# ysymyth/3D-SDN

Measured on AMD Instinct MI355X. Metric: rendered-objects/sec (FFD decode + transform + silhouette/normal/depth @384, fwd+bwd), higher is better.
Workload: dtype f32

## Files before the change

### 3d-sdn_amd/csrc/raster_bwd.hip

```cpp
#include "raster_math.h"
#include "sdn_common.h"

namespace sdn {

#ifndef SDN_EDGE_CHUNK
#define SDN_EDGE_CHUNK 8
#endif
constexpr int CHUNK = SDN_EDGE_CHUNK;
static_assert(CHUNK == 4 || CHUNK == 8, "k_edge_scan_sil / k_chunk_sum are written for 4 or 8");

struct BwdParams {
    const float* faces;
    const float* textures;
    const float* face_inv;
    const int32_t* face_index_map;
    const float* weight_map;
    const float* depth_map;
    const float* rgb_map;
    const float* g_rgb_out;
    const float* g_alpha_out;
    const float* g_depth_out;
    float* grad_faces;
    float* grad_textures;
    uint32_t* visible;
// ... 102 lines not shown
    w.pi0 = pi[0];
    w.pi1 = pi[1];
    if (axis == 0)
        w.direction = (w.p[0][0] < w.p[1][0]) ? -1 : 1;
    else
        w.direction = (w.p[0][0] < w.p[1][0]) ? 1 : -1;
    w.d0_from = cvt_i32(fmaxf(ceilf(fminf(w.p[0][0], w.p[1][0])), 0.0f));
    w.d0_to = cvt_i32(fminf(fmaxf(w.p[0][0], w.p[1][0]), is_f - 1.0f));
    return w;
}

__device__ __forceinline__ void edge_pixel(const BwdParams& P, const MapReader& M, const EdgeWalk& w, int fn, int axis,
                                           int d0, bool use_alpha, bool use_rgb, int lane, int nlanes, float& acc0,
                                           float& acc1)
{
    const int S = P.S;
    const float is_f = (float)S;
    const float fd0 = (float)d0;
    float d1_cross = (w.p[1][1] - w.p[0][1]) / (w.p[1][0] - w.p[0][0]);
    d1_cross = d1_cross * (fd0 - w.p[0][0]);
    d1_cross = d1_cross + w.p[0][1];
    const int d1_in = (0 < w.direction) ? cvt_i32(floorf(d1_cross)) : cvt_i32(ceilf(d1_cross));
    const int d1_out = d1_in + w.direction;
    if (d1_in < 0 || S <= d1_in) return;
    if (d1_out < 0 || S <= d1_out) return;

    const int xin = axis == 0 ? d0 : d1_in, yin = axis == 0 ? d1_in : d0;
    const int xout = axis == 0 ? d0 : d1_out, yout = axis == 0 ? d1_out : d0;
    float alpha_in = 0.f, alpha_out = 0.f, rgb_in[3] = {0, 0, 0}, rgb_out[3] = {0, 0, 0};
    const int f_in = M.fidx(xin, yin);
    if (use_alpha) {
        alpha_in = f_in >= 0 ? 1.0f : 0.0f;
        alpha_out = M.alpha(xout, yout);
    }
    if (use_rgb) {
#pragma unroll
        for (int k = 0; k < 3; k++) {
            rgb_in[k] = M.rgb(xin, yin, k);
            rgb_out[k] = M.rgb(xout, yout, k);
        }
    }
    const bool nz1 = w.p[1][0] != fd0, nz0 = w.p[0][0] != fd0;
    const float den1 = w.p[1][0] - fd0, den0 = fd0 - w.p[0][0];
    const bool sparse_rows = P.nz_cnt && use_alpha && !use_rgb;

    if (f_in == fn && sparse_rows) {
        const int d1_limit = (0 < w.direction) ? S - 1 : 0;
        const int d1_from = max(min(d1_out, d1_limit), 0);
        const int d1_to = min(max(d1_out, d1_limit), S - 1);
        const size_t row = (size_t)(axis == 0 ? P.bs : 0) * S + (size_t)M.b * S + d0;
        const uint16_t* cnt = P.nz_cnt + row * (S + 1);
        const int k1 = cnt[d1_to + 1];
        for (int k = cnt[d1_from] + lane; k < k1; k += nlanes) {
            const int d1 = P.nz_pos[row * S + k];
            const float diff_grad = P.nz_val[row * S + k];
            if (nz1) acc0 -= diff_grad / edge_dist(w.p[0][0], w.p[1][0], den1, d1, d1_cross, is_f, P.eps);
            if (nz0) acc1 -= diff_grad / edge_dist(w.p[0][0], w.p[1][0], den0, d1, d1_cross, is_f, P.eps);
        }
    } else if (f_in == fn) {
        const int d1_limit = (0 < w.direction) ? S - 1 : 0;
        const int d1_from = max(min(d1_out, d1_limit), 0);
        const int d1_to = min(max(d1_out, d1_limit), S - 1);
        for (int d1 = d1_from + lane; d1 <= d1_to; d1 += nlanes) {
            const int x = axis == 0 ? d0 : d1, y = axis == 0 ? d1 : d0;
            float diff_grad = 0.0f;
            if (use_alpha) diff_grad = diff_grad + (M.alpha(x, y) - alpha_in) * M.g_alpha(x, y);
            if (use_rgb) {
#pragma unroll
                for (int k = 0; k < 3; k++) diff_grad = diff_grad + (M.rgb(x, y, k) - rgb_in[k]) * M.g_rgb(x, y, k);
            }
            if (diff_grad <= 0) continue;
            if (nz1) acc0 -= diff_grad / edge_dist(w.p[0][0], w.p[1][0], den1, d1, d1_cross, is_f, P.eps);
            if (nz0) acc1 -= diff_grad / edge_dist(w.p[0][0], w.p[1][0], den0, d1, d1_cross, is_f, P.eps);
        }
    }
    {
        float d0_cross2;
        if ((fd0 - w.p[0][0]) * (fd0 - w.p[2][0]) < 0) {
            d0_cross2 = (w.p[2][1] - w.p[0][1]) / (w.p[2][0] - w.p[0][0]);
            d0_cross2 = d0_cross2 * (fd0 - w.p[0][0]);
            d0_cross2 = d0_cross2 + w.p[0][1];
        } else {
            d0_cross2 = (w.p[1][1] - w.p[2][1]) / (w.p[1][0] - w.p[2][0]);
            d0_cross2 = d0_cross2 * (fd0 - w.p[2][0]);
            d0_cross2 = d0_cross2 + w.p[2][1];
        }
        const int d1_limit = (0 < w.direction) ? cvt_i32(ceilf(d0_cross2)) : cvt_i32(floorf(d0_cross2));
        const int d1_from = max(min(d1_in, d1_limit), 0);
        const int d1_to = min(max(d1_in, d1_limit), S - 1);
        for (int d1 = d1_from + lane; d1 <= d1_to; d1 += nlanes) {
            const int x = axis == 0 ? d0 : d1, y = axis == 0 ? d1 : d0;
            if (M.fidx(x, y) != fn) continue;
            float diff_grad = 0.0f;
            if (use_alpha) diff_grad = diff_grad + (1.0f - alpha_out) * M.g_alpha(x, y);
            if (use_rgb) {
#pragma unroll
                for (int k = 0; k < 3; k++) diff_grad = diff_grad + (M.rgb(x, y, k) - rgb_out[k]) * M.g_rgb(x, y, k);
            }
            if (diff_grad <= 0) continue;
            if (nz1) acc0 -= diff_grad / edge_dist(w.p[0][0], w.p[1][0], den1, d1, d1_cross, is_f, P.eps);
            if (nz0) acc1 -= diff_grad / edge_dist(w.p[0][0], w.p[1][0], den0, d1, d1_cross, is_f, P.eps);
        }
    }
}

__global__ __launch_bounds__(256) void k_mark_visible(const int32_t* __restrict__ face_index_map, long npx, int S,
                                                       int nf, uint32_t* __restrict__ visible)
{
    const long i = (long)blockIdx.x * 256 + threadIdx.x;
    if (i >= npx) return;
    const int fn = face_index_map[i];
    if (fn >= 0) visible[(i / ((long)S * S)) * nf + fn] = 1u;
}

__global__ __launch_bounds__(256) void k_cover_bits(const BwdParams P, uint32_t* __restrict__ cov, uint32_t* __restrict__ covT,
                                                    float* __restrict__ gT)
{
    __shared__ uint32_t flag[32][33];
    __shared__ float gt[32][33];
    const int S = P.S, b = blockIdx.z, W = (S + 31) >> 5;
    const bool aa = (P.flags & SDN_AA) != 0;
    const int R = aa ? S / 2 : S, n = aa ? 16 : 32;
    const int lx = threadIdx.x & 31, l8 = threadIdx.x >> 5;
    const unsigned half = threadIdx.x & 32;
    const int x = blockIdx.x * 32 + lx;
    int fn[4];
    float gv[4];
#pragma unroll
    for (int r = 0; r < 4; r++) {
        const int ly = l8 + 8 * r, y = blockIdx.y * 32 + ly;
        const int xo = blockIdx.x * n + lx, yo = blockIdx.y * n + ly;
        fn[r] = (x < S && y < S) ? P.face_index_map[((size_t)b * S + y) * S + x] : -1;
        gv[r] = (lx < n && ly < n && xo < R && yo < R) ? P.g_alpha_out[((size_t)b * R + yo) * R + xo] : 0.0f;
    }
#pragma unroll
    for (int r = 0; r < 4; r++) {
        const int ly = l8 + 8 * r, y = blockIdx.y * 32 + ly;
        const bool covered = fn[r] >= 0;
        const int left = __shfl_up(fn[r], 1);
        if (covered && ((threadIdx.x & 63) == 0 || left != fn[r])) P.visible[(size_t)b * P.nf + fn[r]] = 1u;
        flag[ly][lx] = covered ? 1u : 0u;
        gt[ly][lx] = gv[r];
        const unsigned long long m = __ballot(covered);
        if (lx == 0 && y < S) cov[((size_t)b * S + y) * W + blockIdx.x] = (uint32_t)(m >> half);
    }
    __syncthreads();
#pragma unroll
    for (int r = 0; r < 4; r++) {
        const int lc = l8 + 8 * r, xt = blockIdx.x * 32 + lc;
        const unsigned long long m = __ballot(flag[lx][lc] != 0u);
        if (lx == 0 && xt < S) covT[((size_t)b * S + xt) * W + blockIdx.y] = (uint32_t)(m >> half);
        const int xo = blockIdx.x * n + lc, yo = blockIdx.y * n + lx;
        if (lx < n && lc < n && xo < R && yo < R) gT[((size_t)b * R + xo) * R + yo] = gt[lx][lc];
    }
}

constexpr int CR = 6;
template <bool AA>
__global__ __launch_bounds__(256) void k_compact_rows(const BwdParams P, const uint32_t* __restrict__ cov,
                                                      const uint32_t* __restrict__ covT, const float* __restrict__ gT,
                                                      size_t rows_per_map, int S, uint16_t* __restrict__ cnt,
                                                      uint16_t* __restrict__ pos, float* __restrict__ val)
{
    const int lane = threadIdx.x & 63;
    const size_t row = (size_t)blockIdx.x * 4 + (threadIdx.x >> 6);
    if (row >= 2 * rows_per_map) return;
    const bool image_row = row < rows_per_map;
    const size_t line = image_row ? row : row - rows_per_map;
    const int b = (int)(line / (size_t)S), d0 = (int)(line % (size_t)S);
    const int R = AA ? S / 2 : S, W = (S + 31) >> 5;
    const uint32_t* cw = (image_row ? cov : covT) + line * W;
    const float* gl = image_row ? P.g_alpha_out + ((size_t)b * R + (R - 1 - (AA ? d0 >> 1 : d0))) * R
                                : gT + ((size_t)b * R + (AA ? d0 >> 1 : d0)) * R;
    uint16_t* c = cnt + row * (S + 1);
    const bool odd = ((row * (size_t)(S + 1)) & 1) != 0;
    const unsigned long long below = (1ull << lane) - 1ull;
    int base = 0;
    if (AA && odd && lane == 0) c[0] = 0;
    for (int e0 = 0; e0 < R; e0 += 64 * CR) {
        float g[CR];
        uint32_t w[CR];
#pragma unroll
        for (int j = 0; j < CR; j++) {
            const int e = e0 + 64 * j + lane;
            g[j] = 0.0f;
            w[j] = 0u;
            if (e < R) {
                g[j] = gl[image_row ? e : R - 1 - e];
                w[j] = cw[AA ? e >> 4 : e >> 5];
            }
        }
#pragma unroll
        for (int j = 0; j < CR; j++) {
            const int e = e0 + 64 * j + lane;
            if (e0 + 64 * j >= R) break;
            const float t = (0.0f - 1.0f) * (AA ? g[j] * 0.25f : g[j]);
            const float h = t > 0.0f ? t : 0.0f;
            const bool in = e < R && h > 0.0f;
            if (AA) {
                const uint32_t two = w[j] >> (2 * (e & 15));
                const bool nz0 = in && !(two & 1u), nz1 = in && !(two & 2u);
                const unsigned long long m0 = __ballot(nz0), m1 = __ballot(nz1);
                const int i0 = base + __popcll(m0 & below) + __popcll(m1 & below);
                const int i1 = i0 + (nz0 ? 1 : 0), i2 = i1 + (nz1 ? 1 : 0);
                if (e < R) {
                    const int x = 2 * e;
                    if (odd)
                        *reinterpret_cast<uint32_t*>(c + x + 1) = (uint32_t)i1 | (uint32_t)i2 << 16;
                    else
                        *reinterpret_cast<uint32_t*>(c + x) = (uint32_t)i0 | (uint32_t)i1 << 16;
                    if (nz0) {
                        pos[row * S + i0] = (uint16_t)x;
                        val[row * S + i0] = h;
                    }
                    if (nz1) {
                        pos[row * S + i1] = (uint16_t)(x + 1);
                        val[row * S + i1] = h;
                    }
                }
                base += __popcll(m0) + __popcll(m1);
            } else {
                const bool nz = in && !((w[j] >> (e & 31)) & 1u);
                const unsigned long long m = __ballot(nz);
                const int i0 = base + __popcll(m & below);
                if (e < R) {
                    c[e] = (uint16_t)i0;
                    if (nz) {
                        pos[row * S + i0] = (uint16_t)e;
                        val[row * S + i0] = h;
                    }
                }
                base += __popcll(m);
            }
        }
    }
    if (lane == 0 && !(AA && odd)) c[S] = (uint16_t)base;
}

constexpr int PLAN_THREADS = 1024;
__global__ __launch_bounds__(PLAN_THREADS) void k_edge_plan(const BwdParams P)
{
    const long i = (long)blockIdx.x * PLAN_THREADS + threadIdx.x;
    const long total = (long)P.bs * P.nf;
    if (P.sink.grad_verts) {
        const long n = (long)P.bs * P.sink.nv * 3;
        for (long k = i; k < n; k += (long)gridDim.x * PLAN_THREADS) P.sink.grad_verts[k] = 0.0f;
    }
    const int lane = threadIdx.x & 63;
    int from[6], cnt[6];
    uint32_t nchunks = 0;
    bool contributes = false;
    if (i < total) {
        const bool active = (P.flags & (SDN_ALPHA | SDN_RGB)) != 0;
        if (active && P.visible[i] != 0u) {
            float face[9];
#pragma unroll
            for (int k = 0; k < 9; k++) face[k] = P.faces[i * 9 + k];
            if (!is_backface(face)) {
                const float is_f = (float)P.S;
#pragma unroll
                for (int e = 0; e < 6; e++) {
                    const EdgeWalk w = edge_walk(face, e >> 1, e & 1, is_f);
                    from[e] = w.d0_from;
                    cnt[e] = max(w.d0_to - w.d0_from + 1, 0);
                    nchunks += (uint32_t)((cnt[e] + CHUNK - 1) / CHUNK);
                }
                contributes = nchunks != 0;
            }
        }
    }
    __shared__ uint32_t wave_sum[PLAN_THREADS / 64];
    __shared__ uint32_t block_base;
    uint32_t incl = nchunks;
#pragma unroll
    for (int d = 1; d < 64; d <<= 1) {
        const uint32_t o = __shfl_up(incl, d, 64);
        if (lane >= d) incl += o;
    }
    const int wave = threadIdx.x >> 6;
    if (lane == 63) wave_sum[wave] = incl;
    __syncthreads();
    if (threadIdx.x == 0) {
        uint32_t tot = 0;
        for (int w = 0; w < PLAN_THREADS / 64; w++) tot += wave_sum[w];
        block_base = tot ? atomicAdd(P.counter, tot) : 0u;
    }
    __syncthreads();
    uint32_t wave_base = block_base;
    for (int w = 0; w < wave; w++) wave_base += wave_sum[w];
    if (i >= total) return;
    const bool per_face = !segment_path(P);
    if (!contributes) {
        if (per_face) P.chunk_base[i] = -2;
        return;
    }
    const uint32_t base = wave_base + incl - nchunks;
    if (base + nchunks > P.cap) {
        if (per_face)
            P.chunk_base[i] = -1;
        else
            P.chunk_base[atomicAdd(P.counter + 1, 1u)] = (int32_t)i;
        for (uint32_t c = base; c < P.cap; c++) P.chunk_desc[c] = make_uint4(0xffffffffu, 0xffffffffu, 0u, 0u);
        return;
    }
    if (per_face) P.chunk_base[i] = (int32_t)base;
    uint32_t c = base;
// ... 495 lines not shown
    const bool head = valid && (px != d.x || py != d.y);
    const unsigned long long bounds = __ballot(head || !valid);
    const unsigned long long above = lane == 63 ? 0ull : bounds >> (lane + 1);
    const int len = head ? (above ? __ffsll((long long)above) : 64 - lane) : 0;
    float a0 = 0.f, a1 = 0.f;
    for (int k = 0; __ballot(k < len) != 0ull; k++) {
        const float tx = __shfl(v.x, lane + k, 64), ty = __shfl(v.y, lane + k, 64);
        if (k < len) {
            a0 += tx;
            a1 += ty;
        }
    }
    const unsigned long long runs_on = __ballot(head && !above && after.x == d.x && after.y == d.y);
    if (runs_on) {
        const int hl = __ffsll((long long)runs_on) - 1;
        const uint32_t kx = (uint32_t)__builtin_amdgcn_readlane((int)d.x, hl), ky = (uint32_t)__builtin_amdgcn_readlane((int)d.y, hl);
        for (uint32_t s0 = c_wave + 64u; s0 < nchunks; s0 += 64u) {
            const uint32_t s = s0 + (uint32_t)lane;
            uint2 ds = make_uint2(0xffffffffu, 0xffffffffu);
            float2 vs = make_float2(0.f, 0.f);
            uint32_t ms = 0u;
            if (s < nchunks) {
                ds = key_at(s);
                vs = P.chunk_out[s];
                ms = P.chunk_mask[s];
            }
            const bool mine = ds.x == kx && ds.y == ky;
            if (mine && ms) vs = chunk_add_owners(P, s, ms, vs);
            const unsigned long long others = ~__ballot(mine);
            const int n = others ? __ffsll((long long)others) - 1 : 64;
            for (int k = 0; k < n; k++) {
                const float tx = __shfl(vs.x, k, 64), ty = __shfl(vs.y, k, 64);
                if (lane == hl) {
                    a0 += tx;
                    a1 += ty;
                }
            }
            if (n < 64) break;
        }
    }
    if (!head) return;
    segment_add(P, (long)d.x, (int)d.y, a0, a1);
}

__global__ __launch_bounds__(256) void k_bwd_pixels(const BwdParams P)
{
    const long i = (long)blockIdx.x * 256 + threadIdx.x;
    const long npx = (long)P.bs * P.S * P.S;
    if (i >= npx) return;
    const int fn = P.face_index_map[i];
    if (fn < 0) return;
    const int S = P.S;
    const int bn = (int)(i / ((long)S * S));
    const int pn = (int)(i % ((long)S * S));
    const int yi = pn / S, xi = pn % S;
    const MapReader M(P, bn);
    const size_t fidx = (size_t)bn * P.nf + fn;
    float face[9];
#pragma unroll
    for (int k = 0; k < 9; k++) face[k] = P.faces[fidx * 9 + k];
    const float depth = P.depth_map[i];
    const float w[3] = {P.weight_map[i * 3 + 0], P.weight_map[i * 3 + 1], P.weight_map[i * 3 + 2]};

    if ((P.flags & SDN_DEPTH) && P.g_depth_out) {
        float inv[9];
#pragma unroll
        for (int k = 0; k < 9; k++) inv[k] = P.face_inv[fidx * 9 + k];
        const float g = M.g_depth(xi, yi);
        const float depth2 = depth * depth;
        float* gf = P.grad_faces + fidx * 9;
#pragma unroll
        for (int k = 0; k < 3; k++) {
            const float zk = face[3 * k + 2];
            float t = g * w[k];
            t = t * depth2;
            t = t / (zk * zk);
            unsafeAtomicAdd(&gf[3 * k + 2], t);
        }
        float tmp[2] = {0.f, 0.f};
#pragma unroll
        for (int k = 0; k < 2; k++)
#pragma unroll
            for (int l = 0; l < 3; l++) tmp[k] = tmp[k] + (-inv[3 * l + k] / face[3 * l + 2]);
#pragma unroll
        for (int k = 0; k < 3; k++)
#pragma unroll
            for (int l = 0; l < 2; l++) {
                float t = -g * tmp[l];
                t = t * w[k];
                t = t * depth2;
                t = t * (float)S;
                t = t / 2.0f;
                unsafeAtomicAdd(&gf[3 * k + l], t);
            }
    }
    if ((P.flags & SDN_RGB) && P.g_rgb_out && P.grad_textures) {
        const bool face_color = (P.flags & SDN_FACE_COLOR) != 0;
        const int ts = face_color ? 2 : P.ts;
        const TexCoord tc = texture_coord(w, depth, face[2], face[5], face[8], ts, P.eps);
        const float g[3] = {M.g_rgb(xi, yi, 0), M.g_rgb(xi, yi, 1), M.g_rgb(xi, yi, 2)};
        if (face_color) {
            float acc[3] = {0.f, 0.f, 0.f};
#pragma unroll
            for (int c = 0; c < 8; c++) {
                int isc;
                float wgt;
                texture_corner(tc, c, ts, isc, wgt);
#pragma unroll
                for (int k = 0; k < 3; k++) acc[k] = acc[k] + wgt * g[k];
            }
#pragma unroll
            for (int k = 0; k < 3; k++) unsafeAtomicAdd(&P.grad_textures[fidx * 3 + k], acc[k]);
        } else {
            float* gt = P.grad_textures + fidx * (size_t)ts * ts * ts * 3;
#pragma unroll
            for (int c = 0; c < 8; c++) {
                int isc;
                float wgt;
                texture_corner(tc, c, ts, isc, wgt);
#pragma unroll
                for (int k = 0; k < 3; k++) unsafeAtomicAdd(&gt[(long)isc * 3 + k], wgt * g[k]);
            }
        }
    }
}

}

using namespace sdn;

static size_t align256(size_t n) { return (n + 255) & ~(size_t)255; }

static void bwd_layout(int bs, int nf, int S, size_t off[14], uint32_t& cap, size_t& total)
{
    const size_t n = (size_t)bs * nf;
    cap = (uint32_t)(4 * n + 65536);
    off[0] = 0;
    off[1] = 256;
    off[10] = off[1] + align256(n * sizeof(uint32_t));
    off[2] = off[10] + align256((size_t)4 * bs * S * sizeof(uint32_t));
    off[3] = off[2] + align256(n * sizeof(int32_t));
    off[4] = off[3] + align256((size_t)cap * sizeof(uint4));
    off[5] = off[4] + align256((size_t)cap * sizeof(float2));
    off[6] = off[5];
    off[7] = off[6] + align256((size_t)bs * S * S * sizeof(float));
    off[8] = off[7] + align256((size_t)2 * bs * S * (S + 1) * sizeof(uint16_t));
    off[9] = off[8] + align256((size_t)2 * bs * S * S * sizeof(uint16_t));
    off[11] = off[9] + align256((size_t)2 * bs * S * S * sizeof(float));
    off[12] = off[11] + align256((size_t)2 * bs * S * 3 * S * sizeof(OwnerRec));
    off[13] = off[12] + align256((size_t)cap * 8 * sizeof(float2));
    total = off[13] + align256((size_t)cap);
}

namespace sdn {
const uint32_t* raster_bwd_visible_flags(const void* workspace) { return (const uint32_t*)((const char*)workspace + 256); }
}

SDN_API int sdn_raster_bwd_workspace_bytes(int bs, int nf, int S, size_t* out)
{
    if (bs <= 0 || nf <= 0 || S <= 0 || !out) return fail(SDN_EINVAL, "sdn_raster_bwd_workspace_bytes: bad sizes");
    size_t off[14], total;
    uint32_t cap;
    bwd_layout(bs, nf, S, off, cap, total);
    *out = total;
    return SDN_OK;
}

SDN_API int sdn_rasterize_bwd(const float* faces, const float* textures, int ts, int bs, int nf, int S, double eps,
                              int flags, const float* face_inv, const int32_t* face_index_map,
                              const float* weight_map, const float* depth_map, const float* rgb_map,
                              const float* g_rgb_out, const float* g_alpha_out, const float* g_depth_out,
                              float* grad_faces, float* grad_textures, void* workspace, size_t workspace_bytes,
                              sdnStream stream)
{
    return rasterize_bwd_core(nullptr, faces, textures, ts, bs, nf, S, eps, flags, face_inv, face_index_map, weight_map, depth_map,
                              rgb_map, g_rgb_out, g_alpha_out, g_depth_out, grad_faces, grad_textures, workspace, workspace_bytes,
                              stream);
}

int sdn::rasterize_bwd_core(const VertexSink* sink, const float* faces, const float* textures, int ts, int bs, int nf, int S,
                            double eps, int flags, const float* face_inv, const int32_t* face_index_map, const float* weight_map,
                            const float* depth_map, const float* rgb_map, const float* g_rgb_out, const float* g_alpha_out,
                            const float* g_depth_out, float* grad_faces, float* grad_textures, void* workspace,
                            size_t workspace_bytes, sdnStream stream)
{
    if (!faces || !face_inv || !face_index_map || !weight_map || !depth_map || (!grad_faces && !sink) || bs <= 0 || nf <= 0 ||
        S <= 0)
        return fail(SDN_EINVAL, "sdn_rasterize_bwd: missing state (was the forward run with SDN_SAVE_MAPS?)");
    if (sink && ((flags & (SDN_RGB | SDN_DEPTH | SDN_ACCUMULATE)) || !(flags & SDN_ALPHA) || !g_alpha_out || !sink->faces_idx ||
                 !sink->grad_verts || nf != (sink->fill_back ? 2 : 1) * sink->nf0))
        return fail(SDN_EINVAL, "rasterize_bwd_core: the vertex sink takes a silhouette-only pass");
    if ((flags & SDN_RGB) && (!rgb_map || !textures))
        return fail(SDN_EINVAL, "sdn_rasterize_bwd: rgb gradients need rgb_map and textures");
    if ((flags & SDN_AA) && (S & 1)) return fail(SDN_EINVAL, "sdn_rasterize_bwd: SDN_AA needs an even internal size");
    size_t off[14], need;
    uint32_t cap;
    bwd_layout(bs, nf, S, off, cap, need);
    if (!workspace || workspace_bytes < need)
        return fail(SDN_ENOMEM, "sdn_rasterize_bwd: workspace %zu < %zu bytes", workspace_bytes, need);
    hipStream_t st = (hipStream_t)stream;
    BwdParams P;
    P.faces = faces;
    P.textures = textures;
    P.face_inv = face_inv;
    P.face_index_map = face_index_map;
    P.weight_map = weight_map;
    P.depth_map = depth_map;
    P.rgb_map = rgb_map;
    P.g_rgb_out = (flags & SDN_RGB) ? g_rgb_out : nullptr;
    P.g_alpha_out = (flags & SDN_ALPHA) ? g_alpha_out : nullptr;
    P.g_depth_out = (flags & SDN_DEPTH) ? g_depth_out : nullptr;
    P.grad_faces = grad_faces;
    P.grad_textures = grad_textures;
    char* ws = (char*)workspace;
    P.counter = (uint32_t*)(ws + off[0]);
    P.visible = (uint32_t*)(ws + off[1]);
    P.chunk_base = (int32_t*)(ws + off[2]);
    P.chunk_desc = (uint4*)(ws + off[3]);
    P.chunk_out = (float2*)(ws + off[4]);
    P.nz_cnt = nullptr;
    P.nz_pos = nullptr;
    P.nz_val = nullptr;
    P.row_cnt = nullptr;
    P.own_rec = nullptr;
    P.own_out = nullptr;
    P.chunk_mask = nullptr;
    P.cap = (flags & SDN_SERIAL_EDGES) ? 0u : cap;
    P.eps = eps;
    P.ts = ts;
    P.bs = bs;
    P.nf = nf;
    P.S = S;
    P.flags = flags;
    P.sink = sink ? *sink : VertexSink{nullptr, 0, 0, 0, 0, nullptr};
    if (!P.g_rgb_out) P.flags &= ~SDN_RGB;
    if (!P.g_alpha_out) P.flags &= ~SDN_ALPHA;
    const long total = (long)bs * nf;
    const long npx = (long)bs * S * S;
    const bool edges = (P.flags & (SDN_ALPHA | SDN_RGB)) != 0;
    if (!edges) P.flags &= ~SDN_SPARSE_GRAD;
    int rc;
    if (edges) {
        hipError_t e = hipMemsetAsync(ws, 0, off[2], st);
        if (e != hipSuccess) return fail(SDN_ELAUNCH, "hipMemsetAsync(plan): %s", hipGetErrorString(e));
        const size_t cov_words = (size_t)(S + 31) / 32;
        const bool setup_fits = 2 * (size_t)bs * S * cov_words * sizeof(uint32_t) <= off[7] - off[6] &&
                                (size_t)bs * S * S * sizeof(float) <= off[12] - off[11];
        const bool sil_path = (P.flags & SDN_ALPHA) && !(P.flags & SDN_RGB) && !(flags & SDN_SERIAL_EDGES) && setup_fits;
        if (!sil_path) {
            hipLaunchKernelGGL(k_mark_visible, dim3(cdiv(npx, 256)), dim3(256), 0, st, face_index_map, npx, S, nf,
                               P.visible);
            if ((rc = check_launch("k_mark_visible"))) return rc;
        }
        if (sil_path) {
            if (S > 65535) return fail(SDN_EINVAL, "sdn_rasterize_bwd: internal size %d exceeds the 16-bit row index", S);
            const bool aa = (P.flags & SDN_AA) != 0;
            const size_t rows = (size_t)bs * S;
            uint32_t* cov = (uint32_t*)(ws + off[6]);
            uint32_t* covT = cov + rows * cov_words;
            float* gT = (float*)(ws + off[11]);
            uint16_t* cnt = (uint16_t*)(ws + off[7]);
            uint16_t* pos = (uint16_t*)(ws + off[8]);
            float* val = (float*)(ws + off[9]);
            hipLaunchKernelGGL(k_cover_bits, dim3(cdiv(S, 32), cdiv(S, 32), bs), dim3(256), 0, st, P, cov, covT, gT);
            if ((rc = check_launch("k_cover_bits"))) return rc;
            const dim3 grid((unsigned)cdiv((long)(2 * rows), 4));
            if (aa)
                hipLaunchKernelGGL(k_compact_rows<true>, grid, dim3(256), 0, st, P, cov, covT, gT, rows, S, cnt, pos, val);
            else
                hipLaunchKernelGGL(k_compact_rows<false>, grid, dim3(256), 0, st, P, cov, covT, gT, rows, S, cnt, pos, val);
            if ((rc = check_launch("k_compact_rows"))) return rc;
            P.nz_cnt = cnt;
            P.nz_pos = pos;
            P.nz_val = val;
            if ((size_t)cap * 8 >= (1u << 30)) return fail(SDN_EINVAL, "sdn_rasterize_bwd: %u chunks exceed the 30-bit slot index", cap);
            P.row_cnt = (uint32_t*)(ws + off[10]);
            P.own_rec = (OwnerRec*)(ws + off[11]);
            P.own_out = (float2*)(ws + off[12]);
            P.chunk_mask = (uint8_t*)(ws + off[13]);
        }
    }
    hipLaunchKernelGGL(k_edge_plan, dim3(cdiv(total, PLAN_THREADS)), dim3(PLAN_THREADS), 0, st, P);
    if ((rc = check_launch("k_edge_plan"))) return rc;
    if (edges) {
        {
            TimedLaunch timed(TIME_EDGE_SCAN, st, 0.0);
            if (P.nz_cnt) {
                hipLaunchKernelGGL(k_edge_scan_sil, dim3(256 * 8), dim3(256), 0, st, P);
                const int nrows = 2 * bs * S;
                hipLaunchKernelGGL(k_edge_rows, dim3((unsigned)nrows), dim3(256), (size_t)S * sizeof(float2), st, P, nrows);
                if (!segment_path(P)) hipLaunchKernelGGL(k_chunk_sum, dim3(cdiv((long)cap, 256)), dim3(256), 0, st, P);
            } else
                hipLaunchKernelGGL(k_edge_scan, dim3(256 * 8), dim3(256), 0, st, P);
        }
        if ((rc = check_launch("k_edge_scan"))) return rc;
    }
    if (segment_path(P)) {
        hipLaunchKernelGGL(k_edge_segments, dim3((unsigned)(cdiv((long)cap, 256) + SEG_SERIAL_BLOCKS)), dim3(256), 0, st, P);
        if ((rc = check_launch("k_edge_segments"))) return rc;
    } else {
        hipLaunchKernelGGL(k_edge_reduce, dim3(cdiv(total, 256)), dim3(256), 0, st, P);
        if ((rc = check_launch("k_edge_reduce"))) return rc;
    }

    const bool need_tex = (P.flags & SDN_RGB) && grad_textures;
    if (need_tex && !(flags & SDN_ACCUMULATE)) {
        const size_t n = (flags & SDN_FACE_COLOR) ? (size_t)total * 3 : (size_t)total * ts * ts * ts * 3;
        hipError_t e = hipMemsetAsync(grad_textures, 0, n * sizeof(float), st);
        if (e != hipSuccess) return fail(SDN_ELAUNCH, "hipMemsetAsync(grad_textures): %s", hipGetErrorString(e));
    }
    if (((P.flags & SDN_DEPTH) && P.g_depth_out) || need_tex) {
        hipLaunchKernelGGL(k_bwd_pixels, dim3(cdiv(npx, 256)), dim3(256), 0, st, P);
        if ((rc = check_launch("k_bwd_pixels"))) return rc;
    }
    return SDN_OK;
}
```

### 3d-sdn_amd/csrc/raster_fwd.hip

```cpp
#include <mutex>
#include <type_traits>
#include <vector>

#include "camera_math.h"
#include "raster_math.h"
#include "sdn_common.h"

namespace sdn {

constexpr int TS = 32;
constexpr int NTHR = (TS / 2) * (TS / 2);
constexpr int NWAVE = NTHR / 64;
static_assert(NTHR % 64 == 0 && NTHR >= 2 * TS && TS <= 32, "tile / workgroup geometry (hit queue packs px, py in 5 bits)");
constexpr int QCAP = 512;
constexpr int FREC = 13;
#ifndef SDN_LAB_FLAT_MAX
#define SDN_LAB_FLAT_MAX 256
#endif
constexpr int FLAT_MAX = SDN_LAB_FLAT_MAX;
static_assert(FLAT_MAX >= 1 && FLAT_MAX <= 256, "a batch's stream holds at most 64 * 256 candidates: 14 bits of start, at most 256 passes (the marks are u16, 0xffff = none)");
#ifndef SDN_LAB_HIZ_MIN_LIST
#define SDN_LAB_HIZ_MIN_LIST 257
#endif
constexpr int HIZ_MIN_LIST = SDN_LAB_HIZ_MIN_LIST;
#ifndef SDN_K1_HIZ
#define SDN_K1_HIZ 1
#endif
constexpr uint32_t TB_CULLED = 0x000000FFu;

struct FwdParams {
    const float* faces;
    const float* textures;
    const float* bg;
    float* face_inv;
    int32_t* face_index_map;
    float* weight_map;
    float* depth_map;
    float* rgb_map;
    float* rgb_out;
    float* alpha_out;
    float* depth_out;
    const uint32_t* tilebox;
    const uint4* pixbox;
    const uint32_t* tile_off;
    const uint32_t* tile_list;
    const uint32_t* overflow;
    const uint32_t* tile_order;
    const uint32_t* thin_count;
    const float4* thin_list;
    unsigned long long* counters;
    uint32_t list_cap;
    double eps;
    int ts, bs, nf, S, ntx, flags, bg_per_batch;
    int hiz;
    float near_le, far_f;
};

constexpr float THIN_MARGIN = 4.0f;

__device__ __forceinline__ float face_margin_px(const float f[9], int S)
{
    const float ex0 = f[3] - f[0], ey0 = f[4] - f[1];
    const float ex1 = f[6] - f[0], ey1 = f[7] - f[1];
    const float ex2 = f[6] - f[3], ey2 = f[7] - f[4];
    const float l0 = sqrtf(ex0 * ex0 + ey0 * ey0);
    const float l1 = sqrtf(ex1 * ex1 + ey1 * ey1);
    const float l2 = sqrtf(ex2 * ex2 + ey2 * ey2);
    const float lmax = fmaxf(l0, fmaxf(l1, l2));
    const float perim = l0 + l1 + l2;
    float cmax = fmaxf(fmaxf(fabsf(f[0]), fabsf(f[1])), fmaxf(fabsf(f[3]), fabsf(f[4])));
    cmax = fmaxf(cmax, fmaxf(fabsf(f[6]), fabsf(f[7])));
    const float area2 = fabsf(ex0 * ey1 - ex1 * ey0) - 9.5367432e-7f * lmax * lmax;
    if (!(area2 > 0.0f)) return -1.0f;
    const float delta = 9.5367432e-7f * (1.0f + cmax);
    const float base = 0.004f * fmaxf(1.0f, (float)S * (1.0f / 1024.0f)) + 0.5f * (float)S * delta;
    const float m = base + 0.5f * (float)S * (delta * perim * lmax / area2);
    if (!(m < (float)S)) return -1.0f;
    return m;
}

constexpr int HIST_MAX = 4096;

template <bool K1, bool GATHER>
__global__ __launch_bounds__(256) void k_face_setup(const float* __restrict__ faces, int nf, int S, int ntx,
                                                     float* __restrict__ face_inv, uint32_t* __restrict__ tilebox,
                                                     uint4* __restrict__ pixbox, uint32_t* __restrict__ tile_count,
                                                     uint32_t* __restrict__ thin_count, float4* __restrict__ thin_list,
                                                     const FaceSource G)
{
    __shared__ uint32_t hist[HIST_MAX];
    const int ntiles = ntx * ntx;
    const bool use_lds = ntiles <= HIST_MAX;
    if (use_lds)
        for (int t = threadIdx.x; t < ntiles; t += 256) hist[t] = 0u;
    __syncthreads();
    const int b = blockIdx.y;
    const int t_local = blockIdx.x * 256 + threadIdx.x;
    uint32_t* gcount = tile_count + (size_t)b * ntiles;
    const bool pairs = GATHER && G.fill_back != 0;
    const int nthr = pairs ? G.nf0 : nf;
    float v[3][3], pf[9];
    if constexpr (GATHER) {
        if (t_local < nthr) {
            const int32_t* idx = G.faces_idx + (size_t)b * G.fstride + (size_t)t_local * 3;
#pragma unroll
            for (int k = 0; k < 3; k++) {
                const float* p = G.verts + ((size_t)b * G.nv + idx[k]) * 3;
                v[k][0] = G.flip_x ? p[0] * -1.0f : p[0];
                v[k][1] = p[1];
                v[k][2] = p[2];
            }
            Basis B;
            if (G.mode != 0) B = camera_basis(G.mode, G.eye, G.dir, G.up, b);
            const float wv = G.width ? G.width[b] : 1.0f;
#pragma unroll
            for (int k = 0; k < 3; k++) {
                float o[3];
                project_vertex(v[k], G.mode, B, G.width != nullptr, wv, o);
                pf[3 * k + 0] = o[0];
                pf[3 * k + 1] = o[1];
                pf[3 * k + 2] = o[2];
            }
        }
    }
    if (t_local < nthr)
    for (int rep = 0; rep < (pairs ? 2 : 1); rep++) {
    const int fn_local = t_local + (rep ? G.nf0 : 0);
    const long i = (long)b * nf + fn_local;
    float f[9];
    float nrm[3] = {0.f, 0.f, 0.f};
    if constexpr (GATHER) {
        if (G.normals_out) {
            if (rep)
                face_normal(v[2], v[1], v[0], G.sx, nrm);
            else
                face_normal(v[0], v[1], v[2], G.sx, nrm);
        }
#pragma unroll
        for (int k = 0; k < 3; k++)
#pragma unroll
            for (int d = 0; d < 3; d++) f[3 * k + d] = rep ? pf[3 * (2 - k) + d] : pf[3 * k + d];
    } else {
#pragma unroll
        for (int k = 0; k < 9; k++) f[k] = faces[i * 9 + k];
    }
    float inv[9] = {0, 0, 0, 0, 0, 0, 0, 0, 0};
    uint32_t tb = TB_CULLED;
    uint4 pb = make_uint4(0, 0, 0, 0);
    bool thin = false;
    if constexpr (K1) {
      if (!is_backface(f)) {
        bool finite = true;
#pragma unroll
        for (int k = 0; k < 9; k++) finite = finite && (f[k] - f[k] == 0.0f);
        const K1Face K = k1_setup(f, S);
        if (finite && !K.dead && K.xi_min <= K.xi_max) {
            float inv_s[9];
            face_inverse(K.px, K.py, inv_s);
#pragma unroll
            for (int l = 0; l < 3; l++)
#pragma unroll
                for (int k = 0; k < 3; k++) {
                    const float v = inv_s[3 * l + k];
                    if (K.pi[l] == 0) inv[k] = v;
                    if (K.pi[l] == 1) inv[3 + k] = v;
                    if (K.pi[l] == 2) inv[6 + k] = v;
                }
            const float ymin = fminf(K.py[0], fminf(K.py[1], K.py[2])), ymax = fmaxf(K.py[0], fmaxf(K.py[1], K.py[2]));
            int y0 = 0, y1 = S - 1;
            if (!(K.px[2] < 0.0f)) {
                y0 = (int)fmaxf(floorf(ymin) - 1.0f, 0.0f);
                y1 = (int)fminf(ceilf(ymax) + 1.0f, (float)(S - 1));
            }
            if (y0 <= y1 && ymax + 1.0f >= 0.0f && ymin - 1.0f <= (float)(S - 1)) {
                const int x0 = K.xi_min, x1 = K.xi_max;
                tb = (uint32_t)(x0 / TS) | ((uint32_t)(x1 / TS) << 8) | ((uint32_t)(y0 / TS) << 16) | ((uint32_t)(y1 / TS) << 24);
                pb = make_uint4((uint32_t)x0 | ((uint32_t)x1 << 16), (uint32_t)y0 | ((uint32_t)y1 << 16), 0u, 0u);
                for (int ty = y0 / TS; ty <= y1 / TS; ty++)
                    for (int tx = x0 / TS; tx <= x1 / TS; tx++) {
                        if (use_lds)
                            atomicAdd(&hist[ty * ntx + tx], 1u);
                        else
                            atomicAdd(&gcount[ty * ntx + tx], 1u);
                    }
            }
        }
      }
    } else if (!is_backface(f)) {
        const float is_f = (float)S;
        float px[3], py[3];
#pragma unroll
        for (int k = 0; k < 3; k++) {
            px[k] = ndc_to_pixel(f[3 * k + 0], is_f);
            py[k] = ndc_to_pixel(f[3 * k + 1], is_f);
        }
        face_inverse(px, py, inv);
        int x0 = 0, x1 = S - 1, y0 = 0, y1 = S - 1;
        const float m = face_margin_px(f, S);
        const float xmin = fminf(px[0], fminf(px[1], px[2])), xmax = fmaxf(px[0], fmaxf(px[1], px[2]));
        const float ymin = fminf(py[0], fminf(py[1], py[2])), ymax = fmaxf(py[0], fmaxf(py[1], py[2]));
        const bool finite = (xmin - xmin == 0.0f) && (xmax - xmax == 0.0f) && (ymin - ymin == 0.0f) &&
                            (ymax - ymax == 0.0f) && (px[0] == px[0]) && (px[1] == px[1]) && (px[2] == px[2]) &&
                            (py[0] == py[0]) && (py[1] == py[1]) && (py[2] == py[2]);
        bool visible = true;
        if (!finite) {
            visible = false;
        } else if (!(m > 0.0f) || m > THIN_MARGIN) {
            visible = false;
            int ia = 0, ib = 1;
            float l2 = (px[1] - px[0]) * (px[1] - px[0]) + (py[1] - py[0]) * (py[1] - py[0]);
            const float l2b = (px[2] - px[0]) * (px[2] - px[0]) + (py[2] - py[0]) * (py[2] - py[0]);
            const float l2c = (px[2] - px[1]) * (px[2] - px[1]) + (py[2] - py[1]) * (py[2] - py[1]);
            if (l2b > l2) { l2 = l2b; ia = 0; ib = 2; }
            if (l2c > l2) { l2 = l2c; ia = 1; ib = 2; }
            if (l2 > 0.0f) {
                const float L = sqrtf(l2);
                const float nx = -(py[ib] - py[ia]) / L, ny = (px[ib] - px[ia]) / L;
                const int ic = 3 - ia - ib;
                const float h = fabsf((px[ic] - px[ia]) * nx + (py[ic] - py[ia]) * ny);
                const float pmax = fmaxf(fmaxf(fabsf(xmin), fabsf(xmax)), fmaxf(fabsf(ymin), fabsf(ymax)));
                float cmax = fmaxf(fmaxf(fabsf(f[0]), fabsf(f[1])), fmaxf(fabsf(f[3]), fabsf(f[4])));
                cmax = fmaxf(cmax, fmaxf(fabsf(f[6]), fabsf(f[7])));
                const float delta_px = 9.5367432e-7f * (1.0f + cmax) * 0.5f * (float)S;
                const float band = h + 0.05f + 2.5f * delta_px + 4e-6f * (pmax + (float)S);
                const bool repeated = (__float_as_uint(f[0]) == __float_as_uint(f[3]) && __float_as_uint(f[1]) == __float_as_uint(f[4])) ||
                                      (__float_as_uint(f[0]) == __float_as_uint(f[6]) && __float_as_uint(f[1]) == __float_as_uint(f[7])) ||
                                      (__float_as_uint(f[3]) == __float_as_uint(f[6]) && __float_as_uint(f[4]) == __float_as_uint(f[7]));
                int bx0 = 0, bx1 = S - 1, by0 = 0, by1 = S - 1;
                bool boxed_out = false;
                if (m > 0.0f) {
                    const float fx0 = ceilf(xmin - m), fx1 = floorf(xmax + m);
                    const float fy0 = ceilf(ymin - m), fy1 = floorf(ymax + m);
                    if (fx1 < 0.0f || fy1 < 0.0f || fx0 > (float)(S - 1) || fy0 > (float)(S - 1) || fx0 > fx1 || fy0 > fy1) {
                        boxed_out = true;
                    } else {
                        bx0 = (int)fmaxf(fx0, 0.0f);
                        by0 = (int)fmaxf(fy0, 0.0f);
                        bx1 = (int)fminf(fx1, (float)(S - 1));
                        by1 = (int)fminf(fy1, (float)(S - 1));
                    }
                }
                if (!(repeated && band < 0.5f) && !boxed_out) {
                    const uint32_t trange = (uint32_t)(bx0 / TS) | ((uint32_t)(bx1 / TS) << 8) | ((uint32_t)(by0 / TS) << 16) |
                                            ((uint32_t)(by1 / TS) << 24);
                    pb = make_uint4((uint32_t)bx0 | ((uint32_t)bx1 << 16), (uint32_t)by0 | ((uint32_t)by1 << 16), __float_as_uint(m), 0u);
                    const uint32_t slot = atomicAdd(&thin_count[b], 1u);
                    float4* e = thin_list + (size_t)b * nf * 2;
                    e[slot] = make_float4(nx, ny, px[ia] * nx + py[ia] * ny, band);
                    e[nf + slot] = make_float4(px[ia], py[ia], __uint_as_float((uint32_t)fn_local), __uint_as_float(trange));
                    thin = true;
                }
            }
        } else {
            const float fx0 = ceilf(xmin - m), fx1 = floorf(xmax + m);
            const float fy0 = ceilf(ymin - m), fy1 = floorf(ymax + m);
            if (fx1 < 0.0f || fy1 < 0.0f || fx0 > (float)(S - 1) || fy0 > (float)(S - 1) || fx0 > fx1 || fy0 > fy1) {
                visible = false;
            } else {
                x0 = (int)fmaxf(fx0, 0.0f);
                y0 = (int)fmaxf(fy0, 0.0f);
                x1 = (int)fminf(fx1, (float)(S - 1));
                y1 = (int)fminf(fy1, (float)(S - 1));
            }
        }
        if (visible) {
            tb = (uint32_t)(x0 / TS) | ((uint32_t)(x1 / TS) << 8) | ((uint32_t)(y0 / TS) << 16) |
                 ((uint32_t)(y1 / TS) << 24);
            pb = make_uint4((uint32_t)x0 | ((uint32_t)x1 << 16), (uint32_t)y0 | ((uint32_t)y1 << 16), __float_as_uint(m), 0u);
            for (int ty = y0 / TS; ty <= y1 / TS; ty++)
                for (int tx = x0 / TS; tx <= x1 / TS; tx++) {
                    if (use_lds)
                        atomicAdd(&hist[ty * ntx + tx], 1u);
                    else
                        atomicAdd(&gcount[ty * ntx + tx], 1u);
                }
        }
    }
    tilebox[i] = tb;
    if (!GATHER || tb != TB_CULLED || thin) {
#pragma unroll
        for (int k = 0; k < 9; k++) face_inv[i * 9 + k] = inv[k];
        pixbox[i] = pb;
        if constexpr (GATHER) {
            float* fo = G.faces_out + i * 9;
#pragma unroll
            for (int k = 0; k < 9; k++) fo[k] = f[k];
            if (G.normals_out) {
                float* o = G.normals_out + i * 3;
                o[0] = nrm[0];
                o[1] = nrm[1];
                o[2] = nrm[2];
            }
        }
    }
    }
    __syncthreads();
    if (use_lds)
        for (int t = threadIdx.x; t < ntiles; t += 256) {
            const uint32_t c = hist[t];
            if (c) atomicAdd(&gcount[t], c);
        }
}

constexpr int ORDER_CLASSES = 64;
__device__ __forceinline__ int order_class(uint32_t entries, bool streams_all_faces)
{
    if (streams_all_faces) return 0;
    const int c = (int)(4.0f * __log2f((float)entries + 1.0f));
    return ORDER_CLASSES - 1 - min(ORDER_CLASSES - 1, c);
}

__global__ __launch_bounds__(256) void k_tile_offsets(const uint32_t* __restrict__ tile_count, int ntiles,
                                                       uint32_t list_cap, uint32_t* __restrict__ tile_off,
                                                       uint32_t* __restrict__ overflow, uint32_t* __restrict__ order_hist)
{
    __shared__ uint32_t wave_tot[4];
    __shared__ uint32_t carry_s;
    __shared__ uint32_t hist[ORDER_CLASSES];
    const int b = blockIdx.x, tid = threadIdx.x;
    if (tid < ORDER_CLASSES) hist[tid] = 0u;
    const uint32_t* cnt = tile_count + (size_t)b * ntiles;
    uint32_t* off = tile_off + (size_t)b * (ntiles + 1);
    if (tid == 0) carry_s = 0u;
    __syncthreads();
    for (int base = 0; base < ntiles; base += 256) {
        const int t = base + tid;
        const uint32_t v = t < ntiles ? cnt[t] : 0u;
        uint32_t incl = v;
#pragma unroll
        for (int d = 1; d < 64; d <<= 1) {
            const uint32_t o = __shfl_up(incl, d, 64);
            if ((tid & 63) >= d) incl += o;
        }
        if ((tid & 63) == 63) wave_tot[tid >> 6] = incl;
        __syncthreads();
        uint32_t wave_off = 0, total = 0;
#pragma unroll
        for (int w = 0; w < 4; w++) {
            const uint32_t x = wave_tot[w];
            if (w < (tid >> 6)) wave_off += x;
            total += x;
        }
        const uint32_t carry = carry_s;
        if (t < ntiles) off[t] = carry + wave_off + incl - v;
        __syncthreads();
        if (tid == 0) carry_s = carry + total;
        __syncthreads();
    }
    if (tid == 0) {
        off[ntiles] = carry_s;
        overflow[b] = carry_s > list_cap ? 1u : 0u;
    }
    const bool streams = carry_s > list_cap;
    for (int t = tid; t < ntiles; t += 256) atomicAdd(&hist[order_class(cnt[t], streams)], 1u);
    __syncthreads();
    if (tid < ORDER_CLASSES && hist[tid]) atomicAdd(&order_hist[tid], hist[tid]);
}

__global__ __launch_bounds__(256) void k_tile_order(const uint32_t* __restrict__ tile_count, int ntiles, int total,
                                                     const uint32_t* __restrict__ overflow,
                                                     const uint32_t* __restrict__ order_hist,
                                                     uint32_t* __restrict__ order_cursor, uint32_t* __restrict__ tile_order)
{
    __shared__ uint32_t base[ORDER_CLASSES];
    const int tid = threadIdx.x;
    if (tid < 64) {
        const uint32_t v = order_hist[tid];
        uint32_t incl = v;
#pragma unroll
        for (int d = 1; d < 64; d <<= 1) {
            const uint32_t o = __shfl_up(incl, d, 64);
            if (tid >= d) incl += o;
        }
        base[tid] = incl - v;
    }
    __shared__ uint32_t lcnt[ORDER_CLASSES], lbase[ORDER_CLASSES];
    if (tid < ORDER_CLASSES) lcnt[tid] = 0u;
    __syncthreads();
    const int g = blockIdx.x * 256 + tid;
    int c = 0;
    uint32_t local = 0;
    if (g < total) {
        c = order_class(tile_count[g], overflow[g / ntiles] != 0u);
        local = atomicAdd(&lcnt[c], 1u);
    }
    __syncthreads();
    if (tid < ORDER_CLASSES && lcnt[tid]) lbase[tid] = base[tid] + atomicAdd(&order_cursor[tid], lcnt[tid]);
    __syncthreads();
    if (g < total) tile_order[lbase[c] + local] = (uint32_t)g;
}

__global__ __launch_bounds__(256) void k_tile_fill(const uint32_t* __restrict__ tilebox, int nf, int ntx,
                                                    const uint32_t* __restrict__ tile_off,
                                                    const uint32_t* __restrict__ overflow, uint32_t list_cap,
                                                    uint32_t* __restrict__ tile_cursor, uint32_t* __restrict__ tile_list)
{
    __shared__ uint32_t cnt[HIST_MAX];
    __shared__ uint32_t base[HIST_MAX];
    const int b = blockIdx.y;
    if (overflow[b]) return;
    const int fn = blockIdx.x * 256 + threadIdx.x;
    const uint32_t v = fn < nf ? tilebox[(size_t)b * nf + fn] : TB_CULLED;
    const int tx0 = (int)(v & 255u), tx1 = (int)((v >> 8) & 255u), ty0 = (int)((v >> 16) & 255u), ty1 = (int)(v >> 24);
    const bool active = tx0 <= tx1;
    const int ntiles = ntx * ntx;
    const uint32_t* off = tile_off + (size_t)b * (ntiles + 1);
    uint32_t* cur = tile_cursor + (size_t)b * ntiles;
    uint32_t* lst = tile_list + (size_t)b * list_cap;
    if (ntiles > HIST_MAX) {
        if (active)
            for (int ty = ty0; ty <= ty1; ty++)
                for (int tx = tx0; tx <= tx1; tx++) {
                    const int tt = ty * ntx + tx;
                    lst[off[tt] + atomicAdd(&cur[tt], 1u)] = (uint32_t)fn;
                }
        return;
    }
    for (int t = threadIdx.x; t < ntiles; t += 256) cnt[t] = 0u;
    __syncthreads();
    if (active)
        for (int ty = ty0; ty <= ty1; ty++)
            for (int tx = tx0; tx <= tx1; tx++) atomicAdd(&cnt[ty * ntx + tx], 1u);
    __syncthreads();
    for (int t = threadIdx.x; t < ntiles; t += 256) {
        const uint32_t c = cnt[t];
        if (c) {
            base[t] = off[t] + atomicAdd(&cur[t], c);
            cnt[t] = 0u;
        }
    }
    __syncthreads();
    if (active)
        for (int ty = ty0; ty <= ty1; ty++)
            for (int tx = tx0; tx <= tx1; tx++) {
                const int tt = ty * ntx + tx;
                lst[base[tt] + atomicAdd(&cnt[tt], 1u)] = (uint32_t)fn;
            }
}

struct PixelResult {
    int fn;
    float w[3];
    float zp;
    float rgb[3];
    float alpha;
};

__device__ __forceinline__ PixelResult shade_pixel(const FwdParams& P, int b, unsigned long long key, int gx, int gy)
{
    PixelResult r;
    const bool want_rgb = (P.flags & SDN_RGB) != 0;
    float bgc[3] = {0.f, 0.f, 0.f};
    if (want_rgb) {
        const float* c = P.bg + (P.bg_per_batch ? 3 * b : 0);
        bgc[0] = c[0];
        bgc[1] = c[1];
        bgc[2] = c[2];
    }
    if (key == ~0ull) {
        r.fn = -1;
        r.w[0] = r.w[1] = r.w[2] = 0.0f;
        r.zp = P.far_f;
        r.alpha = 0.0f;
#pragma unroll
        for (int k = 0; k < 3; k++) r.rgb[k] = 0.0f * 0.0f + (1.0f - 0.0f) * bgc[k];
        return r;
    }
    const int fn = (int)(uint32_t)(key & 0xffffffffull);
    const size_t fidx = (size_t)b * P.nf + fn;
    float inv[9], f[9];
#pragma unroll
    for (int k = 0; k < 9; k++) inv[k] = P.face_inv[fidx * 9 + k];
#pragma unroll
    for (int k = 0; k < 9; k++) f[k] = P.faces[fidx * 9 + k];
    r.fn = fn;
    if (P.flags & SDN_K1_COVERAGE) {
        int pi[3];
        k1_order(f, pi);
        float inv_s[9], ws[3];
#pragma unroll
        for (int l = 0; l < 3; l++)
#pragma unroll
            for (int k = 0; k < 3; k++) inv_s[3 * l + k] = pi[l] == 0 ? inv[k] : (pi[l] == 1 ? inv[3 + k] : inv[6 + k]);
        bary_weights(inv_s, gx, gy, ws);
#pragma unroll
        for (int l = 0; l < 3; l++) {
            if (pi[l] == 0) r.w[0] = ws[l];
            if (pi[l] == 1) r.w[1] = ws[l];
            if (pi[l] == 2) r.w[2] = ws[l];
        }
    } else {
        bary_weights(inv, gx, gy, r.w);
    }
    r.zp = ord_unbits((uint32_t)(key >> 32));
    r.alpha = 1.0f;
    r.rgb[0] = r.rgb[1] = r.rgb[2] = 0.0f;
    if (want_rgb) {
        const bool face_color = (P.flags & SDN_FACE_COLOR) != 0;
        const int ts = face_color ? 2 : P.ts;
        const TexCoord tc = texture_coord(r.w, r.zp, f[2], f[5], f[8], ts, P.eps);
        const float* tex = face_color ? (P.textures + fidx * 3) : (P.textures + fidx * (size_t)ts * ts * ts * 3);
        float acc[3] = {0.f, 0.f, 0.f};
#pragma unroll
        for (int pn = 0; pn < 8; pn++) {
            int isc;
            float wgt;
            texture_corner(tc, pn, ts, isc, wgt);
            const float* t = face_color ? tex : (tex + (long)isc * 3);
#pragma unroll
            for (int k = 0; k < 3; k++) acc[k] = acc[k] + wgt * t[k];
        }
#pragma unroll
        for (int k = 0; k < 3; k++) r.rgb[k] = acc[k] * 1.0f + (1.0f - 1.0f) * bgc[k];
    }
    return r;
}

__device__ __forceinline__ void tile_epilogue(const FwdParams& P, const int b, const int X0, const int Y0,
                                              const unsigned long long* zbuf, const int tid)
{
    const int S = P.S;
    const bool aa = (P.flags & SDN_AA) != 0;
    const bool save = (P.flags & SDN_SAVE_MAPS) != 0;
    const bool lazy = (P.flags & SDN_LAZY_MAPS) != 0;
    const bool want_rgb = (P.flags & SDN_RGB) != 0;
    const bool want_alpha = (P.flags & SDN_ALPHA) != 0;
    const bool want_depth = (P.flags & SDN_DEPTH) != 0;
    const int qx = tid % (TS / 2), qy = tid / (TS / 2);
    const int R = aa ? S / 2 : S;
    float s_alpha = 0.f, s_depth = 0.f, s_rgb[3] = {0.f, 0.f, 0.f};
    bool any_valid = false;
#pragma unroll
    for (int dyi = 0; dyi < 2; dyi++) {
#pragma unroll
        for (int dx = 0; dx < 2; dx++) {
            const int dy = 1 - dyi;
            const int px = 2 * qx + dx, py = 2 * qy + dy;
            const int gx = X0 + px, gy = Y0 + py;
            if (gx >= S || gy >= S) continue;
            any_valid = true;
            const PixelResult r = shade_pixel(P, b, zbuf[py * TS + px], gx, gy);
            const size_t q = ((size_t)b * S + gy) * S + gx;
            if (save) {
                P.face_index_map[q] = r.fn;
                P.depth_map[q] = r.zp;
            }
            if (save && !lazy) {
                P.weight_map[q * 3 + 0] = r.w[0];
                P.weight_map[q * 3 + 1] = r.w[1];
                P.weight_map[q * 3 + 2] = r.w[2];
                if (want_rgb) {
                    P.rgb_map[q * 3 + 0] = r.rgb[0];
                    P.rgb_map[q * 3 + 1] = r.rgb[1];
                    P.rgb_map[q * 3 + 2] = r.rgb[2];
                }
            }
            if (aa) {
                s_alpha = s_alpha + r.alpha;
                s_depth = s_depth + r.zp;
#pragma unroll
                for (int k = 0; k < 3; k++) s_rgb[k] = s_rgb[k] + r.rgb[k];
            } else {
                const size_t o = ((size_t)b * S + (S - 1 - gy)) * S + gx;
                if (want_alpha) P.alpha_out[o] = r.alpha;
                if (want_depth) P.depth_out[o] = r.zp;
                if (want_rgb) {
#pragma unroll
                    for (int k = 0; k < 3; k++)
                        P.rgb_out[(((size_t)b * 3 + k) * S + (S - 1 - gy)) * S + gx] = r.rgb[k];
                }
            }
        }
    }
    if (aa && any_valid) {
        const int oc = X0 / 2 + qx;
        const int orow = R - 1 - (Y0 / 2 + qy);
        const size_t o = ((size_t)b * R + orow) * R + oc;
        if (want_alpha) P.alpha_out[o] = s_alpha * 0.25f;
        if (want_depth) P.depth_out[o] = s_depth * 0.25f;
        if (want_rgb) {
#pragma unroll
            for (int k = 0; k < 3; k++) P.rgb_out[(((size_t)b * 3 + k) * R + orow) * R + oc] = s_rgb[k] * 0.25f;
        }
    }
}

__device__ __forceinline__ void hiz_refresh(const uint32_t* zhi, uint32_t* blockmax, const int lane)
{
    uint32_t m[4] = {0u, 0u, 0u, 0u};
#pragma unroll
    for (int i = 0; i < 16; i++) m[i >> 2] = max(m[i >> 2], zhi[2 * (i * 64 + lane) + 1]);
#pragma unroll
    for (int rb = 0; rb < 4; rb++) {
        uint32_t v = m[rb];
        v = max(v, (uint32_t)__shfl_xor((int)v, 1, 64));
        v = max(v, (uint32_t)__shfl_xor((int)v, 2, 64));
        v = max(v, (uint32_t)__shfl_xor((int)v, 4, 64));
        v = max(v, (uint32_t)__shfl_xor((int)v, 32, 64));
        m[rb] = v;
    }
    if ((lane & 39) == 0) {
#pragma unroll
        for (int rb = 0; rb < 4; rb++) blockmax[rb * 4 + (lane >> 3)] = m[rb];
    }
    __builtin_amdgcn_wave_barrier();
}
__device__ __forceinline__ bool hiz_hidden(const uint32_t* blockmax, const uint32_t zc, const int x0, const int x1, const int y0,
                                           const int y1)
{
    uint32_t zb = 0u;
    for (int by = y0 >> 3; by <= (y1 >> 3); by++)
        for (int bx = x0 >> 3; bx <= (x1 >> 3); bx++) zb = max(zb, blockmax[by * (TS / 8) + bx]);
    return zc > zb;
}

template <bool COUNT, int HIZ>
__global__ __launch_bounds__(NTHR, 6) void k_raster_tiles(const FwdParams P)
{
    unsigned n_cand = 0, n_in = 0, n_key = 0;
    unsigned long long c_fetch = 0, c_small = 0, c_large = 0, c_thin = 0, c_epi = 0, t_mark = 0, t_begin = 0;
    auto tick = [&](unsigned long long& acc) {
        if constexpr (COUNT) {
            const unsigned long long now = wall_clock64();
            acc += now - t_mark;
            t_mark = now;
        }
    };
    if constexpr (COUNT) t_begin = t_mark = wall_clock64();
    __shared__ unsigned long long zbuf[TS * TS];
    __shared__ uint32_t q_fn[QCAP];
    __shared__ float xtab[TS], ytab[TS];
    __shared__ uint32_t q_count, next_batch, next_thin;
    __shared__ uint32_t hit_queue[NWAVE][128];
    __shared__ float face_rec[NWAVE][64 * FREC];
    __shared__ uint32_t blockmax[(TS / 8) * (TS / 8)];
    __shared__ uint32_t own_strip[NWAVE][32];
    static_assert(TS == 32, "the hi-z refresh maps 64 lanes x 16 reads onto a 32 x 32 tile");

    const int tid = threadIdx.x;
    const int lane = tid & 63, wave = tid >> 6;
    const int ntiles_all = P.ntx * P.ntx;
    const uint32_t gid = P.tile_order[blockIdx.x];
    const int b = (int)(gid / (uint32_t)ntiles_all), tile = (int)(gid % (uint32_t)ntiles_all);
    const int tx = tile % P.ntx, ty = tile / P.ntx;
    const int X0 = tx * TS, Y0 = ty * TS;
    const int S = P.S, nf = P.nf;

    for (int i = tid; i < TS * TS; i += NTHR) zbuf[i] = ~0ull;
    if (tid < TS)
        xtab[tid] = pixel_to_ndc(X0 + tid, S);
    else if (tid < 2 * TS)
        ytab[tid - TS] = pixel_to_ndc(Y0 + tid - TS, S);
    if (tid == 0) q_count = next_batch = next_thin = 0;
    if (tid < (TS / 8) * (TS / 8)) blockmax[tid] = 0xffffffffu;
    __syncthreads();

    const float4* thin_cull = P.thin_list + (size_t)b * nf * 2;
    const uint32_t n_thin = P.thin_count[b];
    const float4 thin_c0 = thin_cull[min(tid, 2 * nf - 1)];
    const uint32_t thin_r0 = reinterpret_cast<const uint32_t*>(thin_cull + nf + min(tid, nf - 1))[3];
    const uint32_t* tb = P.tilebox + (size_t)b * nf;
    const uint4* pbx = P.pixbox + (size_t)b * nf;
    const float* faces_b = P.faces + (size_t)b * nf * 9;
    const float* finv_b = P.face_inv + (size_t)b * nf * 9;

    auto shade_hit = [&](const float z0, const float z1, const float z2, const float (&inv)[9], const uint32_t qf,
                         const int px, const int py) {
        float bw[3];
        bary_weights(inv, X0 + px, Y0 + py, bw);
        const float zp = persp_depth(bw, z0, z1, z2);
        if (zp > P.near_le && zp < P.far_f) {
            if constexpr (COUNT) n_key++;
            const unsigned long long key = ((unsigned long long)ord_bits(zp) << 32) | qf;
            atomicMin(&zbuf[py * TS + px], key);
        }
    };
    uint32_t* hq = hit_queue[wave];
    float* frec = face_rec[wave];
    int hq_n = 0;
    auto drain = [&](const int count) {
        if (lane < count) {
            const uint32_t e = hq[lane];
            const int slot = (int)(e & 63u), px = (int)((e >> 6) & 31u), py = (int)((e >> 11) & 31u);
            const float* r = frec + slot * FREC;
            float inv[9];
#pragma unroll
            for (int k = 0; k < 9; k++) inv[k] = r[3 + k];
            shade_hit(r[0], r[1], r[2], inv, __float_as_uint(r[12]), px, py);
        }
    };
    const uint32_t* zhi = reinterpret_cast<const uint32_t*>(zbuf);
    auto behind = [&](const uint32_t zc, const int px, const int py) -> bool { return zc > zhi[2 * (py * TS + px) + 1]; };
    bool hiz_on = false;
    auto refresh_hiz = [&]() { hiz_refresh(zhi, blockmax, lane); };
    auto push_hits = [&](const bool hit, const uint32_t entry) {
        const unsigned long long hm = __ballot(hit);
        if (hm) {
            if (hit) hq[hq_n + (int)__popcll(hm & ((1ull << lane) - 1ull))] = entry;
            hq_n += (int)__popcll(hm);
            __builtin_amdgcn_wave_barrier();
            if (hq_n >= 64) {
                drain(64);
                __builtin_amdgcn_wave_barrier();
                const uint32_t rest = (lane < hq_n - 64) ? hq[64 + lane] : 0u;
                __builtin_amdgcn_wave_barrier();
                hq[lane] = rest;
                hq_n -= 64;
                __builtin_amdgcn_wave_barrier();
            }
        }
    };
    auto raster_batch = [&](const uint32_t* ids, const int n) {
        if constexpr (HIZ > 0) {
            if (HIZ == 1 || hiz_on) refresh_hiz();
        }
        const bool mine = lane < n;
        const uint32_t qf_l = mine ? ids[lane] : 0u;
        uint4 pb_l = make_uint4(0u, 0u, 0u, 0u);
        float f_l[9], inv_l[9];
#pragma unroll
        for (int kk = 0; kk < 9; kk++) f_l[kk] = inv_l[kk] = 0.0f;
        if (mine) {
            pb_l = pbx[qf_l];
#pragma unroll
            for (int kk = 0; kk < 9; kk++) f_l[kk] = faces_b[(size_t)qf_l * 9 + kk];
#pragma unroll
            for (int kk = 0; kk < 9; kk++) inv_l[kk] = finv_b[(size_t)qf_l * 9 + kk];
        }
        const int lx0 = max((int)(pb_l.x & 0xffffu), X0), lx1 = min((int)(pb_l.x >> 16), X0 + TS - 1);
        const int ly0 = max((int)(pb_l.y & 0xffffu), Y0), ly1 = min((int)(pb_l.y >> 16), Y0 + TS - 1);
        const int lw = lx1 - lx0 + 1, lh = ly1 - ly0 + 1;
        int area_l = (mine && lw > 0 && lh > 0) ? lw * lh : 0;
        const float zmin_l = fminf(f_l[2], fminf(f_l[5], f_l[8]));
        const uint32_t zc_l = (zmin_l > 0.0f) ? ord_bits(zmin_l * 0.99999f) : 0u;
        if constexpr (HIZ > 0) {
            if ((HIZ == 1 || hiz_on) && area_l > 0 && zc_l != 0u && hiz_hidden(blockmax, zc_l, lx0 - X0, lx1 - X0, ly0 - Y0, ly1 - Y0))
// ... 119 lines not shown
                    hit = inside_ndc(f, xtab[px], yp);
                    if constexpr (COUNT) n_in += hit ? 1u : 0u;
                    if (hit) hit = !behind(zc, px, py);
                }
                push_hits(hit, slot | ((uint32_t)px << 6) | ((uint32_t)py << 11));
            }
        }
        if (hq_n) {
            drain(hq_n);
            hq_n = 0;
            __builtin_amdgcn_wave_barrier();
        }
        tick(c_large);
    };

    const float4* thin_recs = thin_cull + nf;
    auto thin_cull_pass = [&]() {
        const float cx = (float)X0 + 0.5f * (float)(TS - 1), cy = (float)Y0 + 0.5f * (float)(TS - 1);
        const float reach = 0.7072f * (float)TS + 0.4f;
#ifndef SDN_LAB_NO_THIN_CULL
        for (uint32_t t = tid; t < n_thin; t += NTHR) {
            const float4 c = t < (uint32_t)NTHR ? thin_c0 : thin_cull[t];
            if (fabsf(cx * c.x + cy * c.y - c.z) > c.w + reach) continue;
            const uint32_t v = t < (uint32_t)NTHR ? thin_r0 : reinterpret_cast<const uint32_t*>(thin_recs + t)[3];
            if ((uint32_t)tx < (v & 255u) || (uint32_t)tx > ((v >> 8) & 255u) || (uint32_t)ty < ((v >> 16) & 255u) || (uint32_t)ty > (v >> 24)) continue;
            const uint32_t slot = atomicAdd(&q_count, 1u);
            if (slot < (uint32_t)QCAP) q_fn[slot] = t;
        }
#endif
    };
    auto thin_items = [&]() {
#ifndef SDN_LAB_NO_THIN
        const uint32_t queued = q_count;
        const bool all = queued > (uint32_t)QCAP;
        const uint32_t n_loop = all ? n_thin : queued;
        constexpr int ROWS_PER_ITEM = 8, GROUPS = TS / ROWS_PER_ITEM;
        for (;;) {
            uint32_t first = 0;
            if (lane == 0) first = atomicAdd(&next_thin, 64u);
            first = (uint32_t)__builtin_amdgcn_readfirstlane((int)first);
            if (first >= n_loop * GROUPS) break;
            const uint32_t item = first + (uint32_t)lane;
            if (item >= n_loop * GROUPS) continue;
            const uint32_t c = item / GROUPS;
            const int g = (int)(item % GROUPS);
            const uint32_t t = all ? c : q_fn[c];
            const float4 e0 = thin_cull[t], e1 = thin_recs[t];
            const float nx = e0.x, ny = e0.y, band = e0.w, ax = e1.x, ay = e1.y;
            const uint32_t qf = __float_as_uint(e1.z);
            const uint4 pbq = pbx[qf];
            const int cx0 = max((int)(pbq.x & 0xffffu) - X0, 0), cx1 = min((int)(pbq.x >> 16) - X0, TS - 1);
            const int cy0 = max((int)(pbq.y & 0xffffu) - Y0, g * ROWS_PER_ITEM), cy1 = min((int)(pbq.y >> 16) - Y0, (g + 1) * ROWS_PER_ITEM - 1);
            if (cx0 > cx1) continue;
            float f[9];
            bool loaded = false;
            for (int py = cy0; py <= cy1; py++) {
                const float off = ((float)(Y0 + py) - ay) * ny;
                int lo = cx0, hi = cx1;
                if (fabsf(nx) > 1e-3f) {
                    const float r = 1.0f / nx;
                    const float xa = ax + (-band - off) * r, xb = ax + (band - off) * r;
                    const float x_lo = fminf(xa, xb) - (float)X0 - 1.0f, x_hi = fmaxf(xa, xb) - (float)X0 + 1.0f;
                    if (!(x_lo <= (float)(TS - 1)) || !(x_hi >= 0.0f)) continue;
                    lo = max(cx0, (int)fmaxf(x_lo, 0.0f));
                    hi = min(cx1, (int)fminf(x_hi, (float)(TS - 1)));
                } else if (fabsf(off + ((float)X0 + 0.5f * (float)(TS - 1) - ax) * nx) > band + 0.5f * (float)TS * fabsf(nx) + 1.0f) {
                    continue;
                }
                for (int px = lo; px <= hi; px++) {
                    const float dist = fabsf(((float)(X0 + px) - ax) * nx + ((float)(Y0 + py) - ay) * ny);
                    if (!(dist <= band)) continue;
                    if (!loaded) {
#pragma unroll
                        for (int k = 0; k < 9; k++) f[k] = faces_b[(size_t)qf * 9 + k];
                        loaded = true;
                    }
                    if (inside_ndc(f, xtab[px], ytab[py])) {
                        float inv[9];
#pragma unroll
                        for (int k = 0; k < 9; k++) inv[k] = finv_b[(size_t)qf * 9 + k];
                        float w[3];
                        bary_weights(inv, X0 + px, Y0 + py, w);
                        const float zp = persp_depth(w, f[2], f[5], f[8]);
                        if (zp > P.near_le && zp < P.far_f) {
                            const unsigned long long key = ((unsigned long long)ord_bits(zp) << 32) | qf;
                            atomicMin(&zbuf[py * TS + px], key);
                        }
                    }
                }
            }
        }
#endif
    };

    if (P.overflow[b] == 0u) {
        const int ntiles = P.ntx * P.ntx;
        const uint32_t* off = P.tile_off + (size_t)b * (ntiles + 1);
        const uint32_t lo = off[tile], hi = off[tile + 1];
        tick(c_fetch);
        thin_cull_pass();
        __syncthreads();
        tick(c_thin);
        const uint32_t* lst = P.tile_list + (size_t)b * P.list_cap + lo;
        const int n_list = (int)(hi - lo);
        hiz_on = n_list >= HIZ_MIN_LIST;
        if (n_list <= 64 * NWAVE) {
            const int per_wave = (n_list + NWAVE - 1) / NWAVE;
            const int run_lo = wave * per_wave, run_hi = min(n_list, run_lo + per_wave);
            if (run_lo < run_hi) raster_batch(lst + run_lo, run_hi - run_lo);
        } else {
            for (;;) {
                int base = 0;
                if (lane == 0) base = (int)atomicAdd(&next_batch, 64u);
                base = __builtin_amdgcn_readfirstlane(base);
                if (base >= n_list) break;
                raster_batch(lst + base, min(64, n_list - base));
            }
        }
        thin_items();
        tick(c_thin);
    } else {
        for (int base = 0; base < nf; base += NTHR) {
            const int fn = base + tid;
            if (fn < nf) {
                const uint32_t v = tb[fn];
                const bool hit = (uint32_t)tx >= (v & 255u) && (uint32_t)tx <= ((v >> 8) & 255u) &&
                                 (uint32_t)ty >= ((v >> 16) & 255u) && (uint32_t)ty <= (v >> 24);
                if (hit) {
                    const uint32_t slot = atomicAdd(&q_count, 1u);
                    q_fn[slot] = (uint32_t)fn;
                }
            }
            __syncthreads();
            const int cnt = (int)q_count;
            __syncthreads();
            const bool last = base + NTHR >= nf;
            if (cnt >= NTHR || (last && cnt > 0)) {
                const int per_wave = (cnt + NWAVE - 1) / NWAVE;
                const int run_lo = wave * per_wave, run_hi = min(cnt, run_lo + per_wave);
                for (int qb = run_lo; qb < run_hi; qb += 64) raster_batch(q_fn + qb, min(64, run_hi - qb));
                __syncthreads();
                if (tid == 0) q_count = 0;
                __syncthreads();
            }
        }
        thin_cull_pass();
        __syncthreads();
        thin_items();
    }
    __syncthreads();
    tick(c_fetch);


    tile_epilogue(P, b, X0, Y0, zbuf, tid);
    if constexpr (COUNT) {
        tick(c_epi);
        __shared__ unsigned long long cnt[3];
        if (tid < 3) cnt[tid] = 0ull;
        __syncthreads();
        unsigned long long c[3] = {n_cand, n_in, n_key};
#pragma unroll
        for (int k = 0; k < 3; k++) {
#pragma unroll
            for (int o = 32; o > 0; o >>= 1) c[k] += __shfl_xor(c[k], o, 64);
            if (lane == 0 && c[k]) atomicAdd(&cnt[k], c[k]);
        }
        __syncthreads();
        if (tid < 3 && cnt[tid]) atomicAdd(P.counters + tid, cnt[tid]);
        if (lane == 0 && (gid & 15u) == 0u) {
            atomicAdd(P.counters + 3, c_fetch);
            atomicAdd(P.counters + 4, c_small);
            atomicAdd(P.counters + 5, c_large);
            atomicAdd(P.counters + 6, c_thin);
            atomicAdd(P.counters + 7, c_epi);
            atomicAdd(P.counters + 8, t_mark - t_begin);
            atomicMax(P.counters + 9, t_mark - t_begin);
            atomicAdd(P.counters + 10, 1ull);
        }
    }
}

__global__ __launch_bounds__(NTHR) void k_raster_tiles_k1(const FwdParams P)
{
    __shared__ unsigned long long zbuf[TS * TS];
    __shared__ uint32_t next_batch;
    __shared__ uint32_t hit_queue[NWAVE][128];
    __shared__ float face_rec[NWAVE][64 * FREC];
    __shared__ uint32_t blockmax[(TS / 8) * (TS / 8)];
    bool hiz_on = false;
    const int tid = threadIdx.x;
    const int lane = tid & 63, wave = tid >> 6;
    const int ntiles = P.ntx * P.ntx;
    const uint32_t gid = P.tile_order[blockIdx.x];
    const int b = (int)(gid / (uint32_t)ntiles), tile = (int)(gid % (uint32_t)ntiles);
    const int tx = tile % P.ntx, ty = tile / P.ntx;
    const int X0 = tx * TS, Y0 = ty * TS;
    const int S = P.S, nf = P.nf;
    for (int i = tid; i < TS * TS; i += NTHR) zbuf[i] = ~0ull;
    if (tid == 0) next_batch = 0;
    if (tid < (TS / 8) * (TS / 8)) blockmax[tid] = 0xffffffffu;
    __syncthreads();
    const uint4* pbx = P.pixbox + (size_t)b * nf;
    const uint32_t* tb = P.tilebox + (size_t)b * nf;
    const float* faces_b = P.faces + (size_t)b * nf * 9;
    const float* finv_b = P.face_inv + (size_t)b * nf * 9;
    const uint32_t* zhi = reinterpret_cast<const uint32_t*>(zbuf);
    uint32_t* hq = hit_queue[wave];
    float* frec = face_rec[wave];
    int hq_n = 0;
    auto drain = [&](const int count) {
        if (lane < count) {
            const uint32_t e = hq[lane];
            const int slot = (int)(e & 63u), px = (int)((e >> 6) & 31u), py = (int)((e >> 11) & 31u);
            const float* r = frec + slot * FREC;
            float inv_s[9], w[3];
#pragma unroll
            for (int k = 0; k < 9; k++) inv_s[k] = r[3 + k];
            bary_weights(inv_s, X0 + px, Y0 + py, w);
            const float zp = persp_depth(w, r[0], r[1], r[2]);
            if (zp > P.near_le && zp < P.far_f) {
                const unsigned long long key = ((unsigned long long)ord_bits(zp) << 32) | __float_as_uint(r[12]);
                atomicMin(&zbuf[py * TS + px], key);
            }
        }
    };
    auto behind = [&](const uint32_t zc, const int px, const int py) -> bool { return zc > zhi[2 * (py * TS + px) + 1]; };
    auto push_hits = [&](const bool hit, const uint32_t entry) {
        const unsigned long long hm = __ballot(hit);
        if (hm) {
            if (hit) hq[hq_n + (int)__popcll(hm & ((1ull << lane) - 1ull))] = entry;
            hq_n += (int)__popcll(hm);
            __builtin_amdgcn_wave_barrier();
            if (hq_n >= 64) {
                drain(64);
                __builtin_amdgcn_wave_barrier();
                const uint32_t rest = (lane < hq_n - 64) ? hq[64 + lane] : 0u;
                __builtin_amdgcn_wave_barrier();
                hq[lane] = rest;
                hq_n -= 64;
                __builtin_amdgcn_wave_barrier();
            }
        }
    };
    constexpr int K1_SMALL = 32;
    auto raster_batch = [&](const bool have, const uint32_t fn) {
        if (hiz_on && SDN_K1_HIZ) hiz_refresh(zhi, blockmax, lane);
        float f[9], inv[9];
#pragma unroll
        for (int k = 0; k < 9; k++) f[k] = inv[k] = 0.0f;
        uint4 pb = make_uint4(0u, 0u, 0u, 0u);
        if (have) {
#pragma unroll
            for (int k = 0; k < 9; k++) f[k] = faces_b[(size_t)fn * 9 + k];
#pragma unroll
            for (int k = 0; k < 9; k++) inv[k] = finv_b[(size_t)fn * 9 + k];
            pb = pbx[fn];
        }
        const int lx0 = max((int)(pb.x & 0xffffu), X0), lx1 = min((int)(pb.x >> 16), X0 + TS - 1);
        const int ly0 = max((int)(pb.y & 0xffffu), Y0), ly1 = min((int)(pb.y >> 16), Y0 + TS - 1);
        const int lw = lx1 - lx0 + 1, lh = ly1 - ly0 + 1;
        int area = (have && lw > 0 && lh > 0) ? lw * lh : 0;
        const K1Face K = k1_setup(f, S);
        const float zmin = fminf(f[2], fminf(f[5], f[8]));
        const uint32_t zc_l = (zmin > 0.0f) ? ord_bits(zmin * 0.99999f) : 0u;
        if (hiz_on && SDN_K1_HIZ && area > 0 && zc_l != 0u && hiz_hidden(blockmax, zc_l, lx0 - X0, lx1 - X0, ly0 - Y0, ly1 - Y0)) area = 0;
        if (area > 0) {
            float* r = frec + lane * FREC;
#pragma unroll
            for (int l = 0; l < 3; l++) {
                const int k = K.pi[l];
                r[l] = k == 0 ? f[2] : (k == 1 ? f[5] : f[8]);
#pragma unroll
                for (int c = 0; c < 3; c++) r[3 + 3 * l + c] = k == 0 ? inv[c] : (k == 1 ? inv[3 + c] : inv[6 + c]);
            }
            r[12] = __uint_as_float(fn);
        }
        __builtin_amdgcn_wave_barrier();
        {
            bool act = area > 0 && area <= K1_SMALL;
            int xi = lx0 - 1, yi = 0, ye = -1;
            while (__ballot(act) != 0ull) {
                bool hit = false;
                uint32_t entry = 0u;
                if (act) {
                    if (yi > ye) {
                        xi++;
                        if (xi > lx1) {
                            act = false;
                        } else {
                            int ya, yb;
                            k1_column(K, xi, S, ya, yb);
                            yi = max(ya, ly0);
                            ye = min(yb, ly1);
                        }
                    }
                    if (act && yi <= ye) {
                        const int px = xi - X0, py = yi - Y0;
                        hit = !behind(zc_l, px, py);
                        entry = (uint32_t)lane | ((uint32_t)px << 6) | ((uint32_t)py << 11);
                        yi++;
                    }
                }
                push_hits(hit, entry);
            }
        }
        unsigned long long big = __ballot(area > K1_SMALL);
        while (big) {
            const int j = __builtin_amdgcn_readfirstlane(__ffsll((long long)big) - 1);
            big &= big - 1ull;
            const int x0 = __builtin_amdgcn_readlane(lx0, j), y0 = __builtin_amdgcn_readlane(ly0, j);
            const int w = __builtin_amdgcn_readlane(lw, j), h = __builtin_amdgcn_readlane(lh, j);
            const uint32_t zc = (uint32_t)__builtin_amdgcn_readlane((int)zc_l, j);
            K1Face Kj;
#pragma unroll
            for (int l = 0; l < 3; l++) {
                Kj.px[l] = __int_as_float(__builtin_amdgcn_readlane(__float_as_int(K.px[l]), j));
                Kj.py[l] = __int_as_float(__builtin_amdgcn_readlane(__float_as_int(K.py[l]), j));
                Kj.pi[l] = 0;
            }
            Kj.sa = __int_as_float(__builtin_amdgcn_readlane(__float_as_int(K.sa), j));
            Kj.sb = __int_as_float(__builtin_amdgcn_readlane(__float_as_int(K.sb), j));
            Kj.sc = __int_as_float(__builtin_amdgcn_readlane(__float_as_int(K.sc), j));
            Kj.xi_min = __builtin_amdgcn_readlane(K.xi_min, j);
            Kj.xi_max = __builtin_amdgcn_readlane(K.xi_max, j);
            Kj.a_ok = __builtin_amdgcn_readlane((int)K.a_ok, j) != 0;
            Kj.b_ok = __builtin_amdgcn_readlane((int)K.b_ok, j) != 0;
            Kj.dead = false;
            const int col = lane >> 1;
            int ya = 0, yb = -1;
            if (col < w) {
                k1_column(Kj, x0 + col, S, ya, yb);
                ya = max(ya, y0);
                yb = min(yb, y0 + h - 1);
            }
            const int px = x0 + col - X0;
            for (int yi = ya + (lane & 1); __ballot(yi <= yb) != 0ull; yi += 2) {
                const bool in = yi <= yb;
                const int py = in ? yi - Y0 : 0;
                const bool hit = in && !behind(zc, in ? px : 0, py);
                push_hits(hit, (uint32_t)j | ((uint32_t)px << 6) | ((uint32_t)py << 11));
            }
        }
        if (hq_n) {
            drain(hq_n);
            hq_n = 0;
            __builtin_amdgcn_wave_barrier();
        }
    };
    if (P.overflow[b] == 0u) {
        const uint32_t* off = P.tile_off + (size_t)b * (ntiles + 1);
        const uint32_t lo = off[tile], hi = off[tile + 1];
        const uint32_t* lst = P.tile_list + (size_t)b * P.list_cap + lo;
        const int n_list = (int)(hi - lo);
        hiz_on = P.hiz != 0 && n_list >= HIZ_MIN_LIST;
        for (;;) {
            int base = 0;
            if (lane == 0) base = (int)atomicAdd(&next_batch, 64u);
            base = __builtin_amdgcn_readfirstlane(base);
            if (base >= n_list) break;
            const bool have = base + lane < n_list;
            raster_batch(have, have ? lst[base + lane] : 0u);
        }
    } else {
        for (int base = 0; base < nf; base += NTHR) {
            const int fn = base + tid;
            bool have = false;
            if (fn < nf) {
                const uint32_t v = tb[fn];
                have = (uint32_t)tx >= (v & 255u) && (uint32_t)tx <= ((v >> 8) & 255u) && (uint32_t)ty >= ((v >> 16) & 255u) &&
                       (uint32_t)ty <= (v >> 24);
            }
            raster_batch(have, (uint32_t)fn);
        }
    }
    __syncthreads();
    tile_epilogue(P, b, X0, Y0, zbuf, tid);
}

__global__ __launch_bounds__(NTHR) void k_raster_tiles_k1_plain(const FwdParams P)
{
    __shared__ unsigned long long zbuf[TS * TS];
    __shared__ uint32_t next_batch;
    const int tid = threadIdx.x;
    const int lane = tid & 63;
    const int ntiles = P.ntx * P.ntx;
    const uint32_t gid = P.tile_order[blockIdx.x];
    const int b = (int)(gid / (uint32_t)ntiles), tile = (int)(gid % (uint32_t)ntiles);
    const int tx = tile % P.ntx, ty = tile / P.ntx;
    const int X0 = tx * TS, Y0 = ty * TS;
    const int S = P.S, nf = P.nf;
    for (int i = tid; i < TS * TS; i += NTHR) zbuf[i] = ~0ull;
    if (tid == 0) next_batch = 0;
    __syncthreads();
    const uint4* pbx = P.pixbox + (size_t)b * nf;
    const uint32_t* tb = P.tilebox + (size_t)b * nf;
    const float* faces_b = P.faces + (size_t)b * nf * 9;
    const float* finv_b = P.face_inv + (size_t)b * nf * 9;
    const uint32_t* zhi = reinterpret_cast<const uint32_t*>(zbuf);
    auto k1_pixel = [&](const float (&inv_s)[9], const float (&zs)[3], const uint32_t fn, const int xi, const int yi) {
        const float zmin = fminf(zs[0], fminf(zs[1], zs[2]));
        if (zmin > 0.0f && ord_bits(zmin * 0.99999f) > zhi[2 * ((yi - Y0) * TS + (xi - X0)) + 1]) return;
        float w[3];
        bary_weights(inv_s, xi, yi, w);
        const float zp = persp_depth(w, zs[0], zs[1], zs[2]);
        if (zp > P.near_le && zp < P.far_f) {
            const unsigned long long key = ((unsigned long long)ord_bits(zp) << 32) | fn;
            atomicMin(&zbuf[(yi - Y0) * TS + (xi - X0)], key);
        }
    };
    auto sorted_rows = [&](const K1Face& K, const float (&f)[9], const float (&inv)[9], float (&inv_s)[9], float (&zs)[3]) {
#pragma unroll
        for (int l = 0; l < 3; l++) {
            const int k = K.pi[l];
            zs[l] = k == 0 ? f[2] : (k == 1 ? f[5] : f[8]);
#pragma unroll
            for (int c = 0; c < 3; c++) inv_s[3 * l + c] = k == 0 ? inv[c] : (k == 1 ? inv[3 + c] : inv[6 + c]);
        }
    };
    constexpr int K1_SMALL = 32;
    auto raster_batch = [&](const bool have, const uint32_t fn) {
        float f[9], inv[9];
#pragma unroll
        for (int k = 0; k < 9; k++) f[k] = inv[k] = 0.0f;
        uint4 pb = make_uint4(0u, 0u, 0u, 0u);
        if (have) {
#pragma unroll
            for (int k = 0; k < 9; k++) f[k] = faces_b[(size_t)fn * 9 + k];
#pragma unroll
            for (int k = 0; k < 9; k++) inv[k] = finv_b[(size_t)fn * 9 + k];
            pb = pbx[fn];
        }
        const int lx0 = max((int)(pb.x & 0xffffu), X0), lx1 = min((int)(pb.x >> 16), X0 + TS - 1);
        const int ly0 = max((int)(pb.y & 0xffffu), Y0), ly1 = min((int)(pb.y >> 16), Y0 + TS - 1);
        const int lw = lx1 - lx0 + 1, lh = ly1 - ly0 + 1;
        const int area = (have && lw > 0 && lh > 0) ? lw * lh : 0;
        if (area > 0 && area <= K1_SMALL) {
            const K1Face K = k1_setup(f, S);
            float inv_s[9], zs[3];
            sorted_rows(K, f, inv, inv_s, zs);
            for (int xi = lx0; xi <= lx1; xi++) {
                int ya, yb;
                k1_column(K, xi, S, ya, yb);
                for (int yi = max(ya, ly0); yi <= min(yb, ly1); yi++) k1_pixel(inv_s, zs, fn, xi, yi);
            }
        }
        unsigned long long big = __ballot(area > K1_SMALL);
        while (big) {
            const int j = __builtin_amdgcn_readfirstlane(__ffsll((long long)big) - 1);
            big &= big - 1ull;
            float g[9], ginv[9];
#pragma unroll
            for (int k = 0; k < 9; k++) {
                g[k] = __int_as_float(__builtin_amdgcn_readlane(__float_as_int(f[k]), j));
                ginv[k] = __int_as_float(__builtin_amdgcn_readlane(__float_as_int(inv[k]), j));
            }
            const int x0 = __builtin_amdgcn_readlane(lx0, j), y0 = __builtin_amdgcn_readlane(ly0, j);
            const int w = __builtin_amdgcn_readlane(lw, j), h = __builtin_amdgcn_readlane(lh, j);
            const uint32_t gfn = (uint32_t)__builtin_amdgcn_readlane((int)fn, j);
            const K1Face K = k1_setup(g, S);
            float inv_s[9], zs[3];
            sorted_rows(K, g, ginv, inv_s, zs);
            const int col = lane >> 1;
            if (col < w) {
                int ya, yb;
                k1_column(K, x0 + col, S, ya, yb);
                ya = max(ya, y0);
                yb = min(yb, y0 + h - 1);
                for (int yi = ya + (lane & 1); yi <= yb; yi += 2) k1_pixel(inv_s, zs, gfn, x0 + col, yi);
            }
        }
    };
    if (P.overflow[b] == 0u) {
        const uint32_t* off = P.tile_off + (size_t)b * (ntiles + 1);
        const uint32_t lo = off[tile], hi = off[tile + 1];
        const uint32_t* lst = P.tile_list + (size_t)b * P.list_cap + lo;
        const int n_list = (int)(hi - lo);
        for (;;) {
            int base = 0;
            if (lane == 0) base = (int)atomicAdd(&next_batch, 64u);
            base = __builtin_amdgcn_readfirstlane(base);
            if (base >= n_list) break;
            const bool have = base + lane < n_list;
            raster_batch(have, have ? lst[base + lane] : 0u);
        }
    } else {
        for (int base = 0; base < nf; base += NTHR) {
            const int fn = base + tid;
            bool have = false;
            if (fn < nf) {
                const uint32_t v = tb[fn];
                have = (uint32_t)tx >= (v & 255u) && (uint32_t)tx <= ((v >> 8) & 255u) && (uint32_t)ty >= ((v >> 16) & 255u) &&
                       (uint32_t)ty <= (v >> 24);
            }
            raster_batch(have, (uint32_t)fn);
        }
    }
    __syncthreads();
    tile_epilogue(P, b, X0, Y0, zbuf, tid);
}

}

using namespace sdn;

struct FwdWorkspace {
    size_t tilebox, pixbox, zeroed, tile_count, tile_cursor, overflow, thin_count, counters, order_hist, zeroed_bytes,
        tile_order, tile_off, tile_list, thin_list, total;
    uint32_t list_cap;
    int ntx, ntiles;
};

static size_t align256(size_t n) { return (n + 255) & ~(size_t)255; }

static FwdWorkspace workspace_layout(int bs, int nf, int S)
{
    FwdWorkspace w;
    const size_t n = (size_t)bs * nf;
    w.ntx = (S + TS - 1) / TS;
    w.ntiles = w.ntx * w.ntx;
    w.list_cap = (uint32_t)(8 * (size_t)nf + 4 * (size_t)w.ntiles);
    size_t o = 0;
    w.tilebox = o;
    o += align256(n * sizeof(uint32_t));
    w.pixbox = o;
    o += align256(n * sizeof(uint4));
    w.zeroed = o;
    w.tile_count = o;
    o += align256((size_t)bs * w.ntiles * sizeof(uint32_t));
    w.tile_cursor = o;
    o += align256((size_t)bs * w.ntiles * sizeof(uint32_t));
    w.overflow = o;
    o += align256((size_t)bs * sizeof(uint32_t));
    w.thin_count = o;
    o += align256((size_t)bs * sizeof(uint32_t));
    w.counters = o;
    o += align256(16 * sizeof(unsigned long long));
    w.order_hist = o;
    o += align256(2 * ORDER_CLASSES * sizeof(uint32_t));
    w.zeroed_bytes = o - w.zeroed;
    w.tile_order = o;
    o += align256((size_t)bs * w.ntiles * sizeof(uint32_t));
    w.tile_off = o;
    o += align256((size_t)bs * (w.ntiles + 1) * sizeof(uint32_t));
    w.tile_list = o;
    o += align256((size_t)bs * w.list_cap * sizeof(uint32_t));
    w.thin_list = o;
    o += align256(n * 2 * sizeof(float4));
    w.total = o;
    return w;
}

SDN_API int sdn_raster_workspace_bytes(int bs, int nf, int S, size_t* out)
{
    if (bs <= 0 || nf <= 0 || S <= 0 || !out) return fail(SDN_EINVAL, "sdn_raster_workspace_bytes: bad sizes");
    *out = workspace_layout(bs, nf, S).total;
    return SDN_OK;
}

namespace sdn {
int rasterize_fwd_core(const FaceSource* src, const float* faces, const float* textures, int ts, int bs, int nf, int S, double near,
                       double far, double eps, const float* bg, int bg_per_batch, int flags, float* face_inv,
                       int32_t* face_index_map, float* weight_map, float* depth_map, float* rgb_map,
                       float* rgb_out, float* alpha_out, float* depth_out, void* workspace,
                       size_t workspace_bytes, sdnStream stream)
{
    if (!(flags & (SDN_RGB | SDN_ALPHA | SDN_DEPTH)))
        return fail(SDN_EINVAL, "sdn_rasterize_fwd: nothing to draw (rasterize.py:25-27)");
    if (!faces || !face_inv || bs <= 0 || nf <= 0 || S <= 0) return fail(SDN_EINVAL, "sdn_rasterize_fwd: bad faces/sizes");
    if (S > TS * 256) return fail(SDN_EINVAL, "sdn_rasterize_fwd: internal size %d > %d", S, TS * 256);
    if ((flags & SDN_AA) && (S & 1)) return fail(SDN_EINVAL, "sdn_rasterize_fwd: SDN_AA needs an even internal size");
    if (flags & SDN_RGB) {
        if (!textures || !bg || !rgb_out) return fail(SDN_EINVAL, "sdn_rasterize_fwd: rgb needs textures, bg, rgb_out");
        if (!(flags & SDN_FACE_COLOR) && ts < 2) return fail(SDN_EINVAL, "sdn_rasterize_fwd: texture size < 2");
    }
    if ((flags & SDN_ALPHA) && !alpha_out) return fail(SDN_EINVAL, "sdn_rasterize_fwd: alpha_out is NULL");
    if ((flags & SDN_DEPTH) && !depth_out) return fail(SDN_EINVAL, "sdn_rasterize_fwd: depth_out is NULL");
    if ((flags & SDN_SAVE_MAPS) && (!face_index_map || !depth_map))
        return fail(SDN_EINVAL, "sdn_rasterize_fwd: SDN_SAVE_MAPS needs the state maps");
    if ((flags & SDN_SAVE_MAPS) && !(flags & SDN_LAZY_MAPS) && (!weight_map || ((flags & SDN_RGB) && !rgb_map)))
        return fail(SDN_EINVAL, "sdn_rasterize_fwd: SDN_SAVE_MAPS needs the state maps");
    const FwdWorkspace W = workspace_layout(bs, nf, S);
    if (!workspace || workspace_bytes < W.total)
        return fail(SDN_ENOMEM, "sdn_rasterize_fwd: workspace %zu < %zu bytes", workspace_bytes, W.total);

    hipStream_t st = (hipStream_t)stream;
    char* ws = (char*)workspace;
    uint32_t* tilebox = (uint32_t*)(ws + W.tilebox);
    uint4* pixbox = (uint4*)(ws + W.pixbox);
    uint32_t* tile_count = (uint32_t*)(ws + W.tile_count);
    uint32_t* tile_cursor = (uint32_t*)(ws + W.tile_cursor);
    uint32_t* overflow = (uint32_t*)(ws + W.overflow);
    uint32_t* tile_off = (uint32_t*)(ws + W.tile_off);
    uint32_t* tile_list = (uint32_t*)(ws + W.tile_list);
    uint32_t* thin_count = (uint32_t*)(ws + W.thin_count);
    float4* thin_list = (float4*)(ws + W.thin_list);
    const int ntx = W.ntx;
    hipError_t me = hipMemsetAsync(ws + W.zeroed, 0, W.zeroed_bytes, st);
    if (me != hipSuccess) return fail(SDN_ELAUNCH, "hipMemsetAsync(tile counters): %s", hipGetErrorString(me));
    const dim3 face_grid(cdiv(nf, 256), bs);
    if (src && nf != (src->fill_back ? 2 : 1) * src->nf0) return fail(SDN_EINVAL, "rasterize_fwd_core: nf %d does not match the face source (%d faces, fill_back %d)", nf, src->nf0, src->fill_back);
    const dim3 setup_grid(cdiv((src && src->fill_back) ? src->nf0 : nf, 256), bs);
    const int k1 = (flags & SDN_K1_COVERAGE) ? 1 : 0;
    FaceSource G = FaceSource();
    if (src) G = *src;
#define SDN_FACE_SETUP(K1_, GATHER_)                                                                                          \
    hipLaunchKernelGGL((k_face_setup<K1_, GATHER_>), setup_grid, dim3(256), 0, st, faces, nf, S, ntx, face_inv, tilebox, pixbox, \
                       tile_count, thin_count, thin_list, G)
    if (k1 && src) SDN_FACE_SETUP(true, true);
    else if (k1) SDN_FACE_SETUP(true, false);
    else if (src) SDN_FACE_SETUP(false, true);
    else SDN_FACE_SETUP(false, false);
#undef SDN_FACE_SETUP
    int rc = check_launch("k_face_setup");
    if (rc) return rc;
    const uint32_t list_cap = (flags & SDN_STREAM_FACES) ? 0u : W.list_cap;
    uint32_t* order_hist = (uint32_t*)(ws + W.order_hist);
    uint32_t* tile_order = (uint32_t*)(ws + W.tile_order);
    hipLaunchKernelGGL(k_tile_offsets, dim3(bs), dim3(256), 0, st, tile_count, W.ntiles, list_cap, tile_off, overflow,
                       order_hist);
    if ((rc = check_launch("k_tile_offsets"))) return rc;
    hipLaunchKernelGGL(k_tile_order, dim3(cdiv(bs * W.ntiles, 256)), dim3(256), 0, st, tile_count, W.ntiles, bs * W.ntiles,
                       overflow, order_hist, order_hist + ORDER_CLASSES, tile_order);
    if ((rc = check_launch("k_tile_order"))) return rc;
    hipLaunchKernelGGL(k_tile_fill, face_grid, dim3(256), 0, st, tilebox, nf, ntx, tile_off, overflow, W.list_cap,
                       tile_cursor, tile_list);
    if ((rc = check_launch("k_tile_fill"))) return rc;

    FwdParams P;
    P.faces = faces;
    P.textures = textures;
    P.bg = bg;
    P.face_inv = face_inv;
    P.face_index_map = face_index_map;
    P.weight_map = weight_map;
    P.depth_map = depth_map;
    P.rgb_map = rgb_map;
    P.rgb_out = rgb_out;
    P.alpha_out = alpha_out;
    P.depth_out = depth_out;
    P.tilebox = tilebox;
    P.pixbox = pixbox;
    P.tile_off = tile_off;
    P.tile_list = tile_list;
    P.overflow = overflow;
    P.tile_order = tile_order;
    P.thin_count = thin_count;
    P.thin_list = thin_list;
    P.counters = (unsigned long long*)(ws + W.counters);
    P.list_cap = W.list_cap;
    P.eps = eps;
    P.ts = ts;
    P.bs = bs;
    P.nf = nf;
    P.S = S;
    P.ntx = ntx;
    P.flags = flags;
    P.bg_per_batch = bg_per_batch;
    float near_le = (float)near;
    if ((double)near_le > near) near_le = nextafterf(near_le, -INFINITY);
    P.near_le = near_le;
    P.far_f = (float)far;
    static const int hiz = [] { const char* e = getenv("SDN_RASTER_HIZ"); return e && e[0] >= '0' && e[0] <= '2' ? e[0] - '0' : 2; }();
    P.hiz = hiz;
    if (k1) {
        if (flags & SDN_COUNT_WORK) return fail(SDN_EINVAL, "sdn_rasterize_fwd: SDN_COUNT_WORK is not built for SDN_K1_COVERAGE");
        TimedLaunch timed(TIME_RASTER_TILES_K1, st, 0.0);
        static const bool plain = [] { const char* e = getenv("SDN_K1_PLAIN"); return e && e[0] == '1'; }();
        if (plain)
            hipLaunchKernelGGL(k_raster_tiles_k1_plain, dim3(ntx * ntx * bs), dim3(NTHR), 0, st, P);
        else
            hipLaunchKernelGGL(k_raster_tiles_k1, dim3(ntx * ntx * bs), dim3(NTHR), 0, st, P);
        return check_launch("k_raster_tiles_k1");
    }
    const dim3 grid(ntx * ntx * bs);
    if (flags & SDN_COUNT_WORK) {
        if (hiz == 0)
            hipLaunchKernelGGL((k_raster_tiles<true, 0>), grid, dim3(NTHR), 0, st, P);
        else if (hiz == 1)
            hipLaunchKernelGGL((k_raster_tiles<true, 1>), grid, dim3(NTHR), 0, st, P);
        else
            hipLaunchKernelGGL((k_raster_tiles<true, 2>), grid, dim3(NTHR), 0, st, P);
    } else {
        TimedLaunch timed(TIME_RASTER_TILES, st, 0.0);
        if (hiz == 0)
            hipLaunchKernelGGL((k_raster_tiles<false, 0>), grid, dim3(NTHR), 0, st, P);
        else if (hiz == 1)
            hipLaunchKernelGGL((k_raster_tiles<false, 1>), grid, dim3(NTHR), 0, st, P);
        else
            hipLaunchKernelGGL((k_raster_tiles<false, 2>), grid, dim3(NTHR), 0, st, P);
    }
    return check_launch("k_raster_tiles");
}
}

SDN_API int sdn_rasterize_fwd(const float* faces, const float* textures, int ts, int bs, int nf, int S, double near,
                              double far, double eps, const float* bg, int bg_per_batch, int flags, float* face_inv,
                              int32_t* face_index_map, float* weight_map, float* depth_map, float* rgb_map,
                              float* rgb_out, float* alpha_out, float* depth_out, void* workspace,
                              size_t workspace_bytes, sdnStream stream)
{
    return rasterize_fwd_core(nullptr, faces, textures, ts, bs, nf, S, near, far, eps, bg, bg_per_batch, flags, face_inv,
                              face_index_map, weight_map, depth_map, rgb_map, rgb_out, alpha_out, depth_out, workspace,
                              workspace_bytes, stream);
}

__global__ __launch_bounds__(256) void k_reshade_maps(const FwdParams P, long npx)
{
    const long q = (long)blockIdx.x * 256 + threadIdx.x;
    if (q >= npx) return;
    const int S = P.S;
    const int gx = (int)(q % S), gy = (int)((q / S) % S), b = (int)(q / ((long)S * S));
    const int fn = P.face_index_map[q];
    const unsigned long long key = fn < 0 ? ~0ull : (((unsigned long long)ord_bits(P.depth_map[q]) << 32) | (uint32_t)fn);
    const PixelResult r = shade_pixel(P, b, key, gx, gy);
    P.weight_map[q * 3 + 0] = r.w[0];
    P.weight_map[q * 3 + 1] = r.w[1];
    P.weight_map[q * 3 + 2] = r.w[2];
    if ((P.flags & SDN_RGB) && P.rgb_map) {
        P.rgb_map[q * 3 + 0] = r.rgb[0];
        P.rgb_map[q * 3 + 1] = r.rgb[1];
        P.rgb_map[q * 3 + 2] = r.rgb[2];
    }
}

namespace sdn {
int launch_reshade_maps(const float* faces, const float* textures, int ts, int bs, int nf, int S, double far, double eps,
                        const float* bg, int bg_per_batch, int flags, const float* face_inv, const int32_t* face_index_map,
                        const float* depth_map, float* weight_map, float* rgb_map, hipStream_t st)
{
    if (!faces || !face_inv || !face_index_map || !depth_map || !weight_map) return fail(SDN_EINVAL, "reshade: null pointer");
    if ((flags & SDN_RGB) && (!textures || !bg || !rgb_map)) return fail(SDN_EINVAL, "reshade: colour maps need textures, bg, rgb_map");
    FwdParams P = {};
    P.faces = faces;
    P.textures = textures;
    P.bg = bg;
    P.face_inv = const_cast<float*>(face_inv);
    P.face_index_map = const_cast<int32_t*>(face_index_map);
    P.depth_map = const_cast<float*>(depth_map);
    P.weight_map = weight_map;
    P.rgb_map = rgb_map;
    P.eps = eps;
    P.ts = ts;
    P.bs = bs;
    P.nf = nf;
    P.S = S;
    P.flags = flags;
    P.bg_per_batch = bg_per_batch;
    P.far_f = (float)far;
    const long npx = (long)bs * S * S;
    hipLaunchKernelGGL(k_reshade_maps, dim3(cdiv(npx, 256)), dim3(256), 0, st, P, npx);
    return check_launch("k_reshade_maps");
}
}

SDN_API int sdn_raster_work_counters(const void* workspace, int bs, int nf, int S, unsigned long long* out3, sdnStream stream)
{
    if (!workspace || !out3 || bs <= 0 || nf <= 0 || S <= 0) return fail(SDN_EINVAL, "sdn_raster_work_counters: bad arguments");
    const FwdWorkspace W = workspace_layout(bs, nf, S);
    hipStream_t st = (hipStream_t)stream;
    if (hipMemcpyAsync(out3, (const char*)workspace + W.counters, 3 * sizeof(unsigned long long), hipMemcpyDeviceToHost, st) !=
            hipSuccess ||
        hipStreamSynchronize(st) != hipSuccess)
        return fail(SDN_ELAUNCH, "sdn_raster_work_counters: copy failed");
    return SDN_OK;
}

SDN_API int sdn_raster_phase_clocks(const void* workspace, int bs, int nf, int S, unsigned long long* out8, sdnStream stream)
{
    if (!workspace || !out8 || bs <= 0 || nf <= 0 || S <= 0) return fail(SDN_EINVAL, "sdn_raster_phase_clocks: bad arguments");
    const FwdWorkspace W = workspace_layout(bs, nf, S);
    hipStream_t st = (hipStream_t)stream;
    if (hipMemcpyAsync(out8, (const char*)workspace + W.counters + 3 * sizeof(unsigned long long), 8 * sizeof(unsigned long long),
                       hipMemcpyDeviceToHost, st) != hipSuccess ||
        hipStreamSynchronize(st) != hipSuccess)
        return fail(SDN_ELAUNCH, "sdn_raster_phase_clocks: copy failed");
    return SDN_OK;
}
```

### 3d-sdn_amd/csrc/raster_maps.hip

```cpp
#include <cstdlib>

#include "camera_math.h"
#include "sdn_common.h"

using namespace sdn;

namespace {

size_t a256(size_t n) { return (n + 255) & ~(size_t)255; }

struct MapsLayout {
    size_t pv, faces9, face_inv, faces_n, colors, fim, wmap, dmap, rgbmap, bgcopy, raster_ws, raster_ws_bytes, total;
    size_t b_raster, b_raster_bytes, g_faces9, g_colors, g_pv, g_faces_n, g_v2, b_total;
    int nf, S;
};

int maps_layout(int bs, int nv, int nf0, int fill_back, int image_size, int flags, MapsLayout& L)
{
    if (bs < 1 || nv < 1 || nf0 < 1 || image_size < 1) return fail(SDN_EINVAL, "sdn_render_maps: bad sizes");
    L.nf = fill_back ? 2 * nf0 : nf0;
    L.S = (flags & SDN_AA) ? 2 * image_size : image_size;
    const size_t n = (size_t)bs * L.nf, px = (size_t)bs * L.S * L.S, v = (size_t)bs * nv;
    const bool normal = (flags & SDN_RGB) != 0;
    size_t o = 0;
    auto take = [&](size_t bytes) {
        const size_t at = o;
        o += a256(bytes);
        return at;
    };
    L.pv = take(v * 12);
    L.faces9 = take(n * 36);
    L.face_inv = take(n * 36);
    L.colors = take(normal ? n * 12 : 0);
    L.fim = take(px * 4);
    L.wmap = take(px * 12);
    L.dmap = take(px * 4);
    L.rgbmap = take(normal ? px * 12 : 0);
    L.bgcopy = take(0);
    int rc = sdn_raster_workspace_bytes(bs, L.nf, L.S, &L.raster_ws_bytes);
    if (rc) return rc;
    L.raster_ws = 0;
    L.total = o;
    o = 0;
    rc = sdn_raster_bwd_workspace_bytes(bs, L.nf, L.S, &L.b_raster_bytes);
    if (rc) return rc;
    L.b_raster = take(L.b_raster_bytes);
    L.g_faces9 = take(n * 36);
    L.g_colors = take(normal ? n * 12 : 0);
    L.g_pv = take(v * 12);
    L.g_faces_n = take(normal ? n * 36 : 0);
    L.faces_n = take(normal ? n * 36 : 0);
    L.g_v2 = take(normal ? v * 12 : 0);
    L.b_total = o;
    return SDN_OK;
}

__global__ __launch_bounds__(256) void k_add_inplace(float* __restrict__ a, const float* __restrict__ b, long n)
{
    const long i = (long)blockIdx.x * 256 + threadIdx.x;
    if (i < n) a[i] = a[i] + b[i];
}

bool sink_enabled()
{
    static const bool on = [] { const char* e = getenv("SDN_VERTEX_SINK"); return !(e && e[0] == '0'); }();
    return on;
}

}

SDN_API int sdn_render_maps_bytes(int bs, int nv, int nf0, int fill_back, int image_size, int flags, size_t* state_bytes,
                                  size_t* bwd_bytes, size_t* fwd_scratch_bytes)
{
    MapsLayout L;
    int rc = maps_layout(bs, nv, nf0, fill_back, image_size, flags, L);
    if (rc) return rc;
    if (state_bytes) *state_bytes = L.total;
    if (bwd_bytes) *bwd_bytes = L.b_total;
    if (fwd_scratch_bytes) *fwd_scratch_bytes = L.raster_ws_bytes;
    return SDN_OK;
}

SDN_API int sdn_render_maps_fwd(const float* verts, int bs, int nv, const int32_t* faces_idx, int nf0,
                                long faces_batch_stride, int fill_back, int camera_mode, const float* eye, const float* dir,
                                const float* up, const float* width, int flip_x, int image_size, int flags, double near,
                                double far, double eps, const float* bg, float* alpha_out, float* normal_out,
                                float* depth_out, void* state, size_t state_bytes, void* scratch, size_t scratch_bytes,
                                sdnStream stream)
{
    if (!verts || !faces_idx || !alpha_out || !state || !scratch) return fail(SDN_EINVAL, "sdn_render_maps_fwd: null pointer");
    MapsLayout L;
    int rc = maps_layout(bs, nv, nf0, fill_back, image_size, flags, L);
    if (rc) return rc;
    if (state_bytes < L.total) return fail(SDN_ENOMEM, "sdn_render_maps_fwd: state %zu < %zu bytes", state_bytes, L.total);
    if (scratch_bytes < L.raster_ws_bytes)
        return fail(SDN_ENOMEM, "sdn_render_maps_fwd: scratch %zu < %zu bytes", scratch_bytes, L.raster_ws_bytes);
    const bool normal = (flags & SDN_RGB) != 0;
    if (normal && (!normal_out || !bg)) return fail(SDN_EINVAL, "sdn_render_maps_fwd: the normal map needs normal_out and bg");
    if ((flags & SDN_DEPTH) && !depth_out) return fail(SDN_EINVAL, "sdn_render_maps_fwd: depth_out is NULL");
    hipStream_t st = (hipStream_t)stream;
    char* s = (char*)state;
    float* colors = normal ? (float*)(s + L.colors) : nullptr;
    static const bool fused_setup = [] { const char* e = getenv("SDN_MAPS_FUSED_SETUP"); return !(e && e[0] == '0'); }();
    FaceSource G = FaceSource();
    if (fused_setup) {
        G.verts = verts; G.faces_idx = faces_idx; G.fstride = faces_batch_stride; G.nv = nv; G.nf0 = nf0;
        G.fill_back = fill_back; G.flip_x = flip_x; G.mode = camera_mode; G.eye = eye; G.dir = dir; G.up = up; G.width = width;
        G.faces_out = (float*)(s + L.faces9); G.normals_out = colors; G.sx = flip_x ? -1.0f : 1.0f;
        if (camera_mode < 0 || camera_mode > 2 || (camera_mode != 0 && (!eye || !dir || !up)))
            return fail(SDN_EINVAL, "sdn_render_maps_fwd: camera mode %d needs eye / direction / up", camera_mode);
    } else {
        if (normal) {
            if ((rc = launch_face_normals_gather(verts, faces_idx, bs, nv, nf0, faces_batch_stride, fill_back, flip_x,
                                                 flip_x ? -1.0f : 1.0f, colors, st)))
                return rc;
        }
        if ((rc = sdn_project_vertices(verts, bs, nv, camera_mode, eye, dir, up, width, flip_x, (float*)(s + L.pv), stream)))
            return rc;
        if ((rc = launch_gather_faces((const float*)(s + L.pv), faces_idx, bs, nv, nf0, faces_batch_stride, fill_back, 0,
                                      (float*)(s + L.faces9), st)))
            return rc;
    }
    const int rflags = (flags & (SDN_RGB | SDN_DEPTH | SDN_AA | SDN_SAVE_MAPS | SDN_STREAM_FACES | SDN_COUNT_WORK | SDN_K1_COVERAGE)) | SDN_ALPHA |
                       (normal ? SDN_FACE_COLOR : 0) | SDN_LAZY_MAPS;
    return rasterize_fwd_core(fused_setup ? &G : nullptr, (const float*)(s + L.faces9), colors, normal ? 2 : 0, bs, L.nf, L.S, near,
                              far, eps, bg, 0, rflags, (float*)(s + L.face_inv), (int32_t*)(s + L.fim), (float*)(s + L.wmap),
                              (float*)(s + L.dmap), normal ? (float*)(s + L.rgbmap) : nullptr, normal_out, alpha_out, depth_out,
                              scratch, L.raster_ws_bytes, stream);
}

SDN_API int sdn_render_maps_bwd(const float* verts, int bs, int nv, const int32_t* faces_idx, int nf0,
                                long faces_batch_stride, int fill_back, int camera_mode, const float* eye, const float* dir,
                                const float* up, const float* width, int flip_x, int image_size, int flags, double eps,
                                double eps_alpha, const float* bg, const float* g_alpha, const float* g_normal, const float* g_depth,
                                float* grad_verts, const void* state, size_t state_bytes, void* workspace,
                                size_t workspace_bytes, sdnStream stream)
{
    if (!verts || !faces_idx || !grad_verts || !state || !workspace) return fail(SDN_EINVAL, "sdn_render_maps_bwd: null pointer");
    if (!(flags & SDN_SAVE_MAPS)) return fail(SDN_EINVAL, "sdn_render_maps_bwd: the forward call did not save its maps");
    MapsLayout L;
    int rc = maps_layout(bs, nv, nf0, fill_back, image_size, flags, L);
    if (rc) return rc;
    if (state_bytes < L.total || workspace_bytes < L.b_total)
        return fail(SDN_ENOMEM, "sdn_render_maps_bwd: state %zu / workspace %zu bytes, need %zu / %zu", state_bytes,
                    workspace_bytes, L.total, L.b_total);
    const bool normal = (flags & SDN_RGB) != 0;
    if (!normal) g_normal = nullptr;
    if (!(flags & SDN_DEPTH)) g_depth = nullptr;
    if (normal && (g_normal || g_depth) && !bg)
        return fail(SDN_EINVAL, "sdn_render_maps_bwd: the colour map is re-derived for this gradient: pass the forward call's bg");
    hipStream_t st = (hipStream_t)stream;
    const char* s = (const char*)state;
    char* w = (char*)workspace;
    const float* faces9 = (const float*)(s + L.faces9);
    const float* colors = normal ? (const float*)(s + L.colors) : nullptr;
    float* g_faces9 = (float*)(w + L.g_faces9);
    float* g_colors = g_normal ? (float*)(w + L.g_colors) : nullptr;
    const int base = (flags & (SDN_AA | SDN_SERIAL_EDGES)) | (normal ? SDN_FACE_COLOR : 0) | SDN_SPARSE_GRAD;
    const uint32_t* visible = (g_alpha || g_normal) ? raster_bwd_visible_flags(w + L.b_raster) : nullptr;
    auto raster_bwd = [&](int fl, double e, const float* gr, const float* ga, const float* gd, float* gt) {
        return sdn_rasterize_bwd(faces9, colors, normal ? 2 : 0, bs, L.nf, L.S, e, fl, (const float*)(s + L.face_inv),
                                 (const int32_t*)(s + L.fim), (const float*)(s + L.wmap), (const float*)(s + L.dmap),
                                 normal ? (const float*)(s + L.rgbmap) : nullptr, gr, ga, gd, g_faces9, gt, w + L.b_raster,
                                 L.b_raster_bytes, stream);
    };
    if ((normal && (g_normal || g_depth)) || (!normal && g_depth)) {
        char* sw = const_cast<char*>(s);
        if ((rc = launch_reshade_maps(faces9, colors, normal ? 2 : 0, bs, L.nf, L.S, 0.0, eps,
                                      normal ? bg : nullptr, 0,
                                      (flags & (SDN_AA | SDN_K1_COVERAGE)) | (normal ? (SDN_RGB | SDN_FACE_COLOR) : 0), (const float*)(s + L.face_inv),
                                      (const int32_t*)(s + L.fim), (const float*)(s + L.dmap), (float*)(sw + L.wmap),
                                      normal ? (float*)(sw + L.rgbmap) : nullptr, st)))
            return rc;
    }
    float* g_pv = (float*)(w + L.g_pv);
    if (g_alpha && !g_depth && !g_colors && sink_enabled()) {
        const VertexSink sink = {faces_idx, faces_batch_stride, nv, nf0, fill_back, g_pv};
        if ((rc = rasterize_bwd_core(&sink, faces9, colors, normal ? 2 : 0, bs, L.nf, L.S, eps_alpha, base | SDN_ALPHA,
                                     (const float*)(s + L.face_inv), (const int32_t*)(s + L.fim), (const float*)(s + L.wmap),
                                     (const float*)(s + L.dmap), nullptr, nullptr, g_alpha, nullptr, nullptr, nullptr,
                                     w + L.b_raster, L.b_raster_bytes, stream)))
            return rc;
        return sdn_project_vertices_bwd(verts, bs, nv, camera_mode, eye, dir, up, width, flip_x, g_pv, grad_verts, stream);
    }
    if (!normal) {
        if ((rc = raster_bwd(base | SDN_ALPHA | (g_depth ? SDN_DEPTH : 0), eps_alpha, nullptr, g_alpha, g_depth, nullptr))) return rc;
    } else if ((rc = raster_bwd(base | SDN_ALPHA, eps_alpha, nullptr, g_alpha, nullptr, nullptr))) {
        return rc;
    }
    if (normal && (g_normal || g_depth)) {
        if (g_colors) {
            hipError_t e = hipMemsetAsync(g_colors, 0, (size_t)bs * L.nf * 12, st);
            if (e != hipSuccess) return fail(SDN_ELAUNCH, "sdn_render_maps_bwd: memset: %s", hipGetErrorString(e));
        }
        if ((rc = raster_bwd(base | (g_normal ? SDN_RGB : 0) | (g_depth ? SDN_DEPTH : 0) | SDN_ACCUMULATE, eps, g_normal, nullptr,
                             g_depth, g_colors)))
            return rc;
    }
    if ((rc = launch_gather_faces_bwd(g_faces9, faces_idx, bs, nv, nf0, faces_batch_stride, fill_back, 0, 1, g_pv, st, visible)))
        return rc;
    if ((rc = sdn_project_vertices_bwd(verts, bs, nv, camera_mode, eye, dir, up, width, flip_x, g_pv, grad_verts, stream)))
        return rc;
    if (g_colors) {
        float* g_faces_n = (float*)(w + L.g_faces_n);
        float* g_v2 = (float*)(w + L.g_v2);
        float* faces_n = (float*)(w + L.faces_n);
        if ((rc = launch_gather_faces(verts, faces_idx, bs, nv, nf0, faces_batch_stride, fill_back, flip_x, faces_n, st))) return rc;
        if ((rc = launch_face_normals_bwd(faces_n, g_colors, (long)bs * L.nf, flip_x ? -1.0f : 1.0f,
                                          g_faces_n, st)))
            return rc;
        if ((rc = launch_gather_faces_bwd(g_faces_n, faces_idx, bs, nv, nf0, faces_batch_stride, fill_back, flip_x, 1, g_v2, st, visible)))
            return rc;
        const long n = (long)bs * nv * 3;
        hipLaunchKernelGGL(k_add_inplace, dim3(cdiv(n, 256)), dim3(256), 0, st, grad_verts, (const float*)g_v2, n);
        if ((rc = check_launch("k_add_inplace"))) return rc;
    }
    return SDN_OK;
}
```

### 3d-sdn_amd/csrc/sdn_common.h

```cpp
#pragma once
#include <hip/hip_runtime.h>

#include <cstdarg>
#include <cstdio>
#include <cstdlib>
#include <cstring>

#include "../../include/sdn_hip.h"

#define SDN_API extern "C" __attribute__((visibility("default")))

namespace sdn {

char* error_slot();

inline int fail(int code, const char* fmt, ...)
{
    va_list ap;
    va_start(ap, fmt);
    vsnprintf(error_slot(), 512, fmt, ap);
    va_end(ap);
    return code;
}

inline int check_launch(const char* what)
{
    hipError_t e = hipGetLastError();
    if (e != hipSuccess) return fail(SDN_ELAUNCH, "%s: %s", what, hipGetErrorString(e));
    return SDN_OK;
}

inline unsigned cdiv(long a, long b) { return (unsigned)((a + b - 1) / b); }

inline bool debug_checks()
{
    const char* e = getenv("SDN_DEBUG_CHECKS");
    return e && !strcmp(e, "1");
}

template <class Launch>
inline int debug_count(const char* who, hipStream_t st, int* bad, Launch launch)
{
    int* flag = nullptr;
    if (hipMalloc(&flag, sizeof(int)) != hipSuccess || hipMemsetAsync(flag, 0, sizeof(int), st) != hipSuccess)
        return fail(SDN_ELAUNCH, "%s: no memory for the debug check", who);
    launch(flag);
    hipError_t e = hipMemcpyAsync(bad, flag, sizeof(int), hipMemcpyDeviceToHost, st);
    if (e == hipSuccess) e = hipStreamSynchronize(st);
    (void)hipFree(flag);
    if (e != hipSuccess) return fail(SDN_ELAUNCH, "%s: debug check: %s", who, hipGetErrorString(e));
    return SDN_OK;
}

enum TimingSlot { TIME_RASTER_TILES = 0, TIME_EDGE_SCAN = 1, TIME_CONV_GEMM = 2, TIME_CONV_WGRAD = 3, TIME_CONV_NARROW = 4,
                  TIME_RASTER_TILES_K1 = 5, TIME_SCENE_MASKS = 6, TIME_SLOTS = 7 };
void timing_declare_work(double work);
struct TimedLaunch {
    TimedLaunch(int slot, hipStream_t st, double work);
    ~TimedLaunch();
    int slot_;
    hipStream_t st_;
    double work_;
    hipEvent_t e0_ = nullptr, e1_ = nullptr;
};

int launch_gather_faces(const float* verts, const int32_t* faces_idx, int bs, int nv, int nf0, long fstride, int fill_back,
                        int flip_x, float* faces_out, hipStream_t st);
int launch_gather_faces_bwd(const float* grad_faces, const int32_t* faces_idx, int bs, int nv, int nf0, long fstride,
                            int fill_back, int flip_x, int zero_first, float* grad_verts, hipStream_t st,
                            const uint32_t* visible = nullptr);
const uint32_t* raster_bwd_visible_flags(const void* raster_bwd_workspace);
int launch_face_normals_gather(const float* verts, const int32_t* faces_idx, int bs, int nv, int nf0, long fstride,
                               int fill_back, int flip_x, float sx, float* normals, hipStream_t st);
int launch_face_normals(const float* faces, long total, float sx, float* normals, hipStream_t st);
int launch_reshade_maps(const float* faces, const float* textures, int ts, int bs, int nf, int S, double far, double eps,
                        const float* bg, int bg_per_batch, int flags, const float* face_inv, const int32_t* face_index_map,
                        const float* depth_map, float* weight_map, float* rgb_map, hipStream_t st);
int launch_face_normals_bwd(const float* faces, const float* grad_normals, long total, float sx, float* grad_faces,
                            hipStream_t st);
struct FaceSource;
int rasterize_fwd_core(const FaceSource* src, const float* faces, const float* textures, int ts, int bs, int nf, int S, double near,
                       double far, double eps, const float* bg, int bg_per_batch, int flags, float* face_inv,
                       int32_t* face_index_map, float* weight_map, float* depth_map, float* rgb_map, float* rgb_out,
                       float* alpha_out, float* depth_out, void* workspace, size_t workspace_bytes, sdnStream stream);

struct VertexSink {
    const int32_t* faces_idx;
    long fstride;
    int nv, nf0, fill_back;
    float* grad_verts;
};
int rasterize_bwd_core(const VertexSink* sink, const float* faces, const float* textures, int ts, int bs, int nf, int S, double eps,
                       int flags, const float* face_inv, const int32_t* face_index_map, const float* weight_map,
                       const float* depth_map, const float* rgb_map, const float* g_rgb_out, const float* g_alpha_out,
                       const float* g_depth_out, float* grad_faces, float* grad_textures, void* workspace, size_t workspace_bytes,
                       sdnStream stream);

}
```

### 3d-sdn_amd/sdn_hip/__init__.py

```python
import ctypes
import os
import threading

import torch

_HERE = os.path.dirname(os.path.abspath(__file__))
LIB_PATH = os.path.normpath(os.path.join(_HERE, '..', 'lib', 'libsdn_hip.so'))

RGB, ALPHA, DEPTH, AA, FACE_COLOR, SAVE_MAPS, ACCUMULATE, SERIAL_EDGES, STREAM_FACES, COUNT_WORK = 1, 2, 4, 8, 16, 32, 64, 128, 256, 512
K1_COVERAGE = 4096

ABI_VERSION = 20

_lib = None
_lock = threading.Lock()
_vp = ctypes.c_void_p
_ci = ctypes.c_int
_cl = ctypes.c_long
_cd = ctypes.c_double
_sz = ctypes.c_size_t


class SdnHipError(RuntimeError):
    pass


def _signatures():
    sig = {
        'sdn_project_vertices': [_vp, _ci, _ci, _ci, _vp, _vp, _vp, _vp, _ci, _vp, _vp],
        'sdn_project_vertices_bwd': [_vp, _ci, _ci, _ci, _vp, _vp, _vp, _vp, _ci, _vp, _vp, _vp],
        'sdn_gather_faces': [_vp, _vp, _ci, _ci, _ci, _cl, _ci, _vp, _vp],
        'sdn_gather_faces_bwd': [_vp, _vp, _ci, _ci, _ci, _cl, _ci, _vp, _vp],
        'sdn_face_normals': [_vp, _cl, _vp, _vp],
        'sdn_face_normals_bwd': [_vp, _vp, _cl, _vp, _vp],
        'sdn_raster_workspace_bytes': [_ci, _ci, _ci, ctypes.POINTER(_sz)],
        'sdn_rasterize_fwd': [_vp, _vp, _ci, _ci, _ci, _ci, _cd, _cd, _cd, _vp, _ci, _ci, _vp, _vp, _vp, _vp, _vp,
                              _vp, _vp, _vp, _vp, _sz, _vp],
        'sdn_raster_bwd_workspace_bytes': [_ci, _ci, _ci, ctypes.POINTER(_sz)],
        'sdn_rasterize_bwd': [_vp, _vp, _ci, _ci, _ci, _ci, _cd, _ci, _vp, _vp, _vp, _vp, _vp, _vp, _vp, _vp, _vp,
                              _vp, _vp, _sz, _vp],
    }
    sig['sdn_raster_work_counters'] = [_vp, _ci, _ci, _ci, ctypes.POINTER(ctypes.c_ulonglong), _vp]
    sig['sdn_ffd_decode'] = [_vp, _vp, _vp, _ci, _ci, _ci, _vp, _vp]
    sig['sdn_ffd_decode_bwd'] = [_vp, _vp, _vp, _ci, _ci, _ci, _vp, _vp]
    _i8p = ctypes.POINTER(ctypes.c_int8)
    _cf = ctypes.c_float
    sig['sdn_conv_gemm_workspace_bytes'] = [_ci, _ci, _ci, _ci, ctypes.POINTER(_sz)]
    sig['sdn_conv_gemm'] = [_vp, _ci, _ci, _ci, _ci, _vp, _ci, _ci, _ci, _ci, _ci, _ci, _ci, _ci, _ci, _ci, _i8p, _i8p,
                            _ci, _ci, _vp, _ci, _ci, _vp, _ci, _vp, _ci, _ci, _vp, _sz, _vp]
    _i32p = ctypes.POINTER(ctypes.c_int32)
    sig['sdn_conv_gemm_phases'] = [_vp, _ci, _ci, _ci, _ci, _vp, _ci, _ci, _ci, _ci, _ci, _ci, _i32p, _i32p, _i32p, _i32p, _i32p, _i8p,
                                   _ci, _ci, ctypes.POINTER(_vp), _i32p, _ci, _vp, _ci, _vp, _ci, _ci, _vp]
    sig['sdn_conv_wgrad'] = [_vp, _vp, _vp, _ci, _ci, _ci, _ci, _ci, _ci, _ci, _ci, _ci, _i8p, _i8p, _ci, _ci, _ci, _ci,
                             _ci, _vp, _sz, _vp]
    sig['sdn_conv_wgrad_narrow'] = [_vp, _vp, _vp, _ci, _ci, _ci, _ci, _ci, _ci, _ci, _ci, _ci, _i8p, _i8p, _ci, _ci, _ci,
                                    _vp]
    sig['sdn_conv_wgrad_head_mfma'] = [_vp, _vp, _vp, _ci, _ci, _ci, _ci, _ci, _ci, _ci, _ci, _ci, _i8p, _i8p, _ci, _ci, _ci,
                                    _vp]
    sig['sdn_conv_narrow_fwd'] = [_vp, _ci, _ci, _ci, _ci, _vp, _ci, _ci, _ci, _ci, _vp, _ci, _ci, _ci, _ci, _ci, _ci,
                                  _vp, _ci, _vp]
    sig['sdn_conv_head_steps'] = [_ci, _ci, _ci, ctypes.POINTER(_ci)]
    sig['sdn_conv_head_mfma'] = [_vp, _ci, _ci, _ci, _ci, _vp, _ci, _ci, _ci, _ci, _vp, _ci, _ci, _ci, _ci, _ci, _ci, _vp, _ci, _vp, _vp]
    sig['sdn_in_apply'] = [_vp, _vp, _vp, _vp, _vp, _ci, _ci, _ci, _ci, _cf, _ci, _ci, _cf, _vp, _vp, _vp, _cl, _ci, _vp]
    sig['sdn_in_bwd'] = [_vp, _vp, _vp, _vp, _ci, _ci, _ci, _ci, _vp, _cl, _vp]
    sig['sdn_act_bwd'] = [_vp, _vp, _vp, _cl, _ci, _ci, _vp, _cl, _vp]
    sig['sdn_reflect_fold'] = [_vp, _vp, _ci, _ci, _ci, _ci, _ci, _ci, _vp]
    sig['sdn_conv_pack_weights'] = [_vp, _ci, _ci, _cl, _cl, _vp, _ci, _ci, _ci, _ci, _vp, _vp]
    sig['sdn_conv_unpack_grad'] = [_vp, _ci, _ci, _cl, _cl, _vp, _ci, _ci, _vp, _ci, _vp]
    sig['sdn_split_planes'] = [_vp, _cl, _ci, _vp, _cl, _vp]
    sig['sdn_assemble_nhwc'] = [_vp, _vp, _ci, _ci, _ci, _ci, _ci, _vp, _vp]
    sig['sdn_conv_pack_weights_kmajor'] = [_vp, _ci, _ci, _cl, _cl, _vp, _ci, _ci, _ci, _vp, _vp]
    sig['sdn_conv_tile'] = [_vp, _cl, _ci, _ci, _ci, _ci, _vp, _vp, _cl, _ci, _ci, _ci, _ci, _ci, _ci, _ci, _ci, _ci, _ci, _ci,
                            _i8p, _i8p, _ci, _vp, _ci, _vp, _ci, _vp, _ci, _ci, _vp]
    sig['sdn_conv_halo_blocks'] = [_ci, _ci, _ci, _ci, _ci, _ci, ctypes.POINTER(_ci), ctypes.POINTER(_ci), ctypes.POINTER(_cl)]
    sig['sdn_conv_halo'] = [_vp, _cl, _ci, _ci, _ci, _ci, _vp, _ci, _ci, _ci, _ci, _i8p, _i8p, _ci, _vp, _ci, _vp, _ci, _vp, _ci, _vp]
    sig['sdn_conv_wgrad_tile'] = [_vp, _cl, _vp, _cl, _vp, _ci, _ci, _ci, _ci, _ci, _ci, _ci, _ci, _ci, _i8p, _i8p, _ci, _vp]
    sig['sdn_segment_mean'] = [_vp, _vp, _ci, _ci, _ci, _ci, _vp, _vp, _vp, _vp]
    sig['sdn_l1_loss_fwd'] = [_vp, _vp, _cl, _vp, _vp, _vp]
    sig['sdn_l1_loss_bwd'] = [_vp, _vp, _cl, _vp, _vp, _vp, _vp]
    sig['sdn_silhouette_loss_fwd'] = [_vp, _vp, _vp, _cl, _vp, _cl, _vp, _vp, _vp]
    sig['sdn_silhouette_loss_bwd'] = [_vp, _vp, _vp, _cl, _vp, _cl, _vp, _vp, _vp, _vp, _vp]
    sig['sdn_pose_params'] = [_vp, _vp, _ci, _vp, _vp, _vp]
    sig['sdn_pose_params_bwd'] = [_vp, _vp, _vp, _vp, _ci, _vp, _vp, _vp]
    sig['sdn_pose_algebra'] = [_vp] * 7 + [_ci, _ci, ctypes.c_float, ctypes.c_float] + [_vp] * 9 + [_vp]
    sig['sdn_pose_algebra_bwd'] = [_vp] * 8 + [_ci, _ci] + [_vp] * 8 + [_vp] * 4 + [_vp]
    sig['sdn_composite_frame'] = [_vp, _vp, _vp, _vp, _ci, _ci, _vp, _ci, _vp, _vp, _vp, _ci, _ci, _vp, _vp, _vp, _vp]
    sig['sdn_edit_assemble'] = [_vp, _cl, _vp, _vp, _vp, _vp, _vp, _ci, _ci, _ci, _ci, _ci, _vp, _vp, _vp, _vp, _vp, _vp]
    sig['sdn_scene_cover'] = [_vp, _ci, _ci, _ci, _vp, _vp]
    sig['sdn_scene_crops'] = [_vp] * 8 + [_ci] * 6 + [_cf] * 6 + [_vp] * 4
    sig['sdn_scene_edit'] = [_vp] * 7 + [_ci, _ci, _ci] + [_vp] * 5
    sig['sdn_unmold_masks'] = [_vp, _ci, _ci, _ci, _ci, _vp, _vp, _ci, _vp, _ci, _vp, _ci, _ci, _ci, _vp, _vp, _vp]
    sig['sdn_scene_gt_masks'] = [_vp, _vp, _ci, _ci, _ci, _vp, _vp, _vp, _vp]
    sig['sdn_scene_paint2d'] = [_vp, _vp, _vp, _ci, _ci, _vp, _ci, _vp, _ci, _ci, _ci, _vp, _vp]
    sig['sdn_scene_id_workspace_bytes'] = [ctypes.POINTER(_sz)]
    sig['sdn_scene_id_stats'] = [_vp, _vp, _ci, _ci, _ci, _vp, _vp, _vp]
    sig['sdn_scene_id_planes'] = [_vp, _vp, _vp, _vp, _ci, _ci, _ci, _vp, _vp, _vp, _vp]
    sig['sdn_assemble_planes'] = [_vp] * 5 + [_ci, _vp, _vp, _ci, _vp] + [_ci] * 9 + [_cf, _cf, _ci, _cf, _vp, _vp]
    sig['sdn_assemble_maps'] = [_vp] * 10 + [_ci] * 9 + [_vp] * 4 + [_ci, _ci] + [_vp] * 4
    sig['sdn_train_rois'] = [_vp, _vp, _ci, _ci, _ci, _ci, _vp, _vp]
    sig['sdn_train_crops'] = [_vp, _vp, _ci, _ci, _ci] + [_vp] * 5 + [_ci, _vp, _ci, _vp, _ci, _vp, _ci, _ci, _ci] + [_cf] * 6 + [_vp] * 5
    sig['sdn_train_id_stats_workspace_bytes'] = [_ci, ctypes.POINTER(_sz)]
    sig['sdn_train_id_stats'] = [_vp, _ci, _cl, _vp, _vp, _vp]
    sig['sdn_train_crops_mixed'] = [_vp] * 5 + [_ci, _vp, _ci, _vp, _ci, _vp, _ci, _ci, _ci] + [_vp] * 5
    sig['sdn_segm_fuse'] = [_vp, _ci, _ci, _ci, _ci, _ci, _vp, _vp, _vp]
    sig['sdn_segm_labels_from_colors'] = [_vp, _ci, _ci, _ci, _vp, _vp, _ci, _vp, _vp, _vp]
    sig['sdn_segm_confusion'] = [_vp, _vp, _ci, _ci, _ci, _ci, _vp, _vp]
    sig['sdn_segm_train_batch'] = [_vp, _vp, _ci, _ci, _ci, _vp, _vp, _cl, _ci, _ci, _ci] + [_cf] * 6 + [_vp, _cl, _vp, _vp, _vp, _vp]
    sig['sdn_segm_loss_fwd'] = [_vp, _vp, _vp, _ci, _ci, _ci, _ci, _cf, _vp, _sz, _vp, _vp, _vp, _vp]
    sig['sdn_segm_loss_bwd'] = [_vp, _vp, _vp, _ci, _ci, _ci, _ci, _cf, _vp, _vp, _vp, _vp, _vp, _vp]
    sig['sdn_segm_ppm_pool'] = [_vp, _ci, _ci, _ci, _ci, _vp, _vp, _ci, _vp, _vp, _vp]
    sig['sdn_segm_ppm_fill'] = [_vp, _ci, _ci, _ci, _ci, _vp, _vp, _ci, _vp, _vp]
    sig['sdn_segm_ppm_fill_bwd'] = [_vp, _ci, _ci, _ci, _ci, _vp, _vp, _ci, _vp, _vp]
    sig['sdn_segm_ppm_pool_bwd'] = [_vp, _vp, _ci, _ci, _ci, _ci, _vp, _vp, _ci, _vp, _vp]
    sig['sdn_encode_maps'] = [_vp, _ci, _vp, _ci, _vp, _ci, _ci, _ci, _ci, _ci, _ci, _vp, _vp, _vp, _vp]
    sig['sdn_inst_index_workspace_bytes'] = [ctypes.POINTER(_sz)]
    sig['sdn_inst_index_build'] = [_vp, _ci, _ci, _ci, _ci, _vp, _sz, _vp, _vp, _cl, _vp]
    sig['sdn_inst_index_rank'] = [_vp, _ci, _ci, _ci, _ci, _vp, _sz, _vp, _vp, _vp]
    sig['sdn_mrcnn_loss_workspace_bytes'] = [_ci, _ci, ctypes.POINTER(_sz), ctypes.POINTER(_sz)]
    _mrl_inputs = [_vp, _ci, _vp, _vp, _vp, _ci, _ci, _ci, _vp, _ci, _vp, _vp, _vp, _vp, _vp, _ci, _ci, _ci, _ci]
    sig['sdn_mrcnn_loss_fwd'] = _mrl_inputs + [_vp, _sz, _vp, _sz, _vp, _vp, _vp]
    sig['sdn_mrcnn_loss_bwd'] = _mrl_inputs + [_vp, _sz, _vp] + [_vp] * 5 + [_vp]
    _ip = ctypes.POINTER(_ci)
    sig['sdn_pyramid_roi_align_grad_floats'] = [_ci, _ip, _ip, ctypes.POINTER(_sz), ctypes.POINTER(_sz)]
    sig['sdn_pyramid_roi_align_fwd'] = [_vp, _ci, ctypes.POINTER(_vp), _ip, _ip, _ci, _ci, _cf, _cf, _vp, _vp, _vp]
    sig['sdn_pyramid_roi_align_bwd'] = [_vp, _vp, _ci, _ip, _ip, _ci, _ci, _cf, _vp, _vp]
    sig['sdn_pyramid_roi_align_bwd_ordered_workspace_bytes'] = [_ci, ctypes.POINTER(_sz)]
    sig['sdn_pyramid_roi_align_bwd_ordered'] = [_vp, _vp, _ci, _ip, _ip, _ci, _ci, _cf, _vp, _vp, _sz, _vp]
    sig['sdn_proposal_layer_workspace_bytes'] = [_ci, _ci, _ci, ctypes.POINTER(_sz)]
    sig['sdn_proposal_layer'] = [_vp, _vp, _vp, _ci, ctypes.POINTER(_cf), _ci, _ci, _ci, _ci, _cf, _ci, _vp, _vp, _vp, _vp, _vp, _vp, _sz, _vp]
    sig['sdn_detection_layer_workspace_bytes'] = [_ci, _ci, _ci, ctypes.POINTER(_sz)]
    sig['sdn_detection_layer'] = [_vp, _vp, _vp, _ci, _ci, ctypes.POINTER(_cf), ctypes.POINTER(_cf), _ci, _ci, _cf, _cf, _ci, _ci, _vp, _vp, _vp,
                                  _vp, _vp, _vp, _vp, _vp, _vp, _sz, _vp]
    sig['sdn_detection_targets_workspace_bytes'] = [_ci] * 7 + [ctypes.POINTER(_sz)]
    sig['sdn_detection_targets'] = [_vp] * 5 + [_ci] * 5 + [_vp, _ci, _cd, ctypes.POINTER(_cf), _ci, _ci, _ci] + [_vp] * 9 + [_sz, _vp]
    sig['sdn_rpn_targets_workspace_bytes'] = [_ci] * 3 + [ctypes.POINTER(_sz)]
    sig['sdn_rpn_targets'] = [_vp] * 4 + [_ci] * 4 + [_vp, _ci, ctypes.POINTER(_cd)] + [_vp] * 5 + [_sz, _vp]
    sig['sdn_training_item_workspace_bytes'] = [_ci] * 4 + [ctypes.POINTER(_sz)]
    sig['sdn_training_item_image'] = [_vp, _ci, _ci, _ci, _vp, _vp, _cl, _vp, _sz, _vp, _vp]
    sig['sdn_training_item'] = [_vp, _vp, _ci, _vp, _ci, _ci, _ci, _vp, _vp, _cl, _ci, _ci, _ci, _vp, _sz] + [_vp] * 7 + [_vp]
    _pp = ctypes.POINTER(_vp)
    sig['sdn_rpn_outputs_fwd'] = [_pp, _pp, _ip, _ip, _ci, _ci, _ci, _vp, _vp, _vp, _vp]
    sig['sdn_rpn_outputs_bwd'] = [_vp, _vp, _vp, _vp, _ip, _ip, _ci, _ci, _ci, _pp, _pp, _vp]
    sig['sdn_derender_heads_workspace_bytes'] = [_ci] * 5 + [ctypes.POINTER(_sz)]
    sig['sdn_derender_heads_fwd'] = [_vp] * 12 + [_ci] * 5 + [_vp] * 5 + [_vp]
    sig['sdn_derender_heads_bwd'] = [_vp] * 15 + [_ci] * 5 + [_vp] * 9 + [_vp, _sz, _vp]
    sig['sdn_train_losses_scratch'] = [_ci, _ci, _cl, ctypes.POINTER(_sz)]
    sig['sdn_train_losses_fwd'] = [_vp] * 7 + [_cl] + [_vp] * 7 + [_ci, _ci, _ci, _ci, _cd, _cd, _vp, _vp, _vp]
    sig['sdn_train_losses_bwd'] = [_vp] * 6 + [_cl] + [_vp] * 7 + [_ci, _ci, _ci, _ci, _cd, _cd] + [_vp] * 9 + [_vp]
    sig['sdn_perspective_transform_scratch'] = [_ci, _ci, ctypes.POINTER(_sz), ctypes.POINTER(_sz)]
    sig['sdn_perspective_transform'] = [_vp, _vp, _vp, _vp, _vp, _vp, _vp, _ci, _ci, _vp, _vp, _vp, _vp]
    sig['sdn_perspective_transform_bwd'] = [_vp, _vp, _vp, _vp, _vp, _vp, _ci, _ci, _vp, _vp, _vp, _vp, _vp, _vp, _vp, _vp,
                                            _vp, _vp, _vp, _vp]
    sig['sdn_bn_forward'] = [_vp, _cl, _ci, _vp, _vp, _vp, _vp, _cf, _cf, _ci, _vp, _ci, _vp, _vp, _vp, _vp, _vp]
    sig['sdn_bn_backward'] = [_vp, _vp, _vp, _vp, _vp, _cl, _ci, _ci, _ci, _vp, _vp, _vp, _vp]
    sig['sdn_maxpool3x3s2_fwd'] = [_vp, _ci, _ci, _ci, _ci, _vp, _vp, _vp]
    sig['sdn_maxpool3x3s2_bwd'] = [_vp, _vp, _ci, _ci, _ci, _ci, _vp, _vp]
    sig['sdn_avgpool_global'] = [_vp, _ci, _ci, _ci, _vp, _ci, _vp]
    sig['sdn_nms_workspace_bytes'] = [_ci, ctypes.POINTER(_sz)]
    sig['sdn_nms'] = [_vp, _vp, _ci, _cf, _ci, _vp, _vp, _vp, _sz, _vp]
    sig['sdn_crop_and_resize_fwd'] = [_vp, _ci, _ci, _ci, _ci, _vp, _vp, _ci, _ci, _ci, _cf, _vp, _vp]
    sig['sdn_crop_and_resize_bwd'] = [_vp, _vp, _vp, _ci, _ci, _ci, _vp, _ci, _ci, _ci, _ci, _vp]
    sig['sdn_timing_enable'] = [_ci]
    sig['sdn_timing_declare_work'] = [_cd]
    sig['sdn_timing_read'] = [ctypes.POINTER(_cd), ctypes.POINTER(_cl)]
    sig['sdn_timing_read_slot'] = [_ci, ctypes.POINTER(_cd), ctypes.POINTER(_cl), ctypes.POINTER(_cd)]
    sig['sdn_ffd_coefficients'] = [_vp, _vp, _vp, _ci, _ci, _ci, _vp, _vp]
    sig['sdn_raster_phase_clocks'] = [_vp, _ci, _ci, _ci, ctypes.POINTER(ctypes.c_ulonglong), _vp]
    sig['sdn_render_maps_bytes'] = [_ci, _ci, _ci, _ci, _ci, _ci, ctypes.POINTER(_sz), ctypes.POINTER(_sz), ctypes.POINTER(_sz)]
    sig['sdn_render_maps_fwd'] = [_vp, _ci, _ci, _vp, _ci, _cl, _ci, _ci, _vp, _vp, _vp, _vp, _ci, _ci, _ci, _cd, _cd, _cd, _vp,
                                  _vp, _vp, _vp, _vp, _sz, _vp, _sz, _vp]
    sig['sdn_render_maps_bwd'] = [_vp, _ci, _ci, _vp, _ci, _cl, _ci, _ci, _vp, _vp, _vp, _vp, _ci, _ci, _ci, _cd, _cd, _vp, _vp, _vp,
                                  _vp, _vp, _vp, _sz, _vp, _sz, _vp]
    _lp = ctypes.POINTER(_cl)
    sig['sdn_avgpool3x3s2_fwd'] = [_vp, _ci, _ci, _ci, _ci, _lp, _vp, _lp, _ci, _vp]
    sig['sdn_avgpool3x3s2_bwd'] = [_vp, _ci, _ci, _ci, _ci, _lp, _vp, _lp, _ci, _vp]
    sig['sdn_program_create'] = [_vp, _ci, _vp, _sz, _ci, ctypes.POINTER(_vp)]
    sig['sdn_program_run'] = [_vp, ctypes.POINTER(_vp), _ci, _vp, _vp, ctypes.POINTER(_cf), ctypes.POINTER(_ci)]
    sig['sdn_program_destroy'] = [_vp]
    return sig


_SIG = _signatures()


def _declare(L):
    L.sdn_last_error.restype = ctypes.c_char_p
    L.sdn_version.restype = _ci
    for name, argtypes in _SIG.items():
        try:
            fn = getattr(L, name)
        except AttributeError:
            raise SdnHipError('%s does not export %s -- rebuild it (`python __graft_entry__.py build`)' % (LIB_PATH, name))
        fn.argtypes = argtypes
        fn.restype = _ci
    return _SIG


def lib():
    global _lib
    if _lib is None:
        with _lock:
            if _lib is None:
                if not os.path.exists(LIB_PATH):
                    raise SdnHipError(
                        'libsdn_hip.so not found at %s -- run `python __graft_entry__.py build` (hipcc, gfx950); '
                        'there is no CPU or PyTorch fallback for this path' % LIB_PATH)
                L = ctypes.CDLL(LIB_PATH)
                L.sdn_version.restype = _ci
                have = L.sdn_version()
                if have != ABI_VERSION:
                    raise SdnHipError('%s reports ABI version %d, this binding needs %d -- rebuild it '
                                      '(`python __graft_entry__.py build`)' % (LIB_PATH, have, ABI_VERSION))
                _declare(L)
                _lib = L
    return _lib


def exported_symbols():
    return ['sdn_last_error', 'sdn_version'] + list(_SIG)


def deterministic():
    return torch.are_deterministic_algorithms_enabled() or os.environ.get('SDN_DETERMINISTIC') == '1'


def check(rc):
    if rc != 0:
        raise SdnHipError('libsdn_hip error %d: %s' % (rc, lib().sdn_last_error().decode()))


def ptr(t):
    return None if t is None else t.data_ptr()


def stream():
    return _vp(torch.cuda.current_stream().cuda_stream)


def want(t, dtype, name):
    if t is None:
        return None
    if not isinstance(t, torch.Tensor):
        raise TypeError('%s must be a torch.Tensor, got %r' % (name, type(t)))
    if not t.is_cuda:
        raise NotImplementedError('%s is on %s; this renderer only runs on the GPU' % (name, t.device))
    if t.dtype != dtype:
        raise TypeError('%s must be %s, got %s' % (name, dtype, t.dtype))
    return t.contiguous()


_const_cache = {}


def const_f32(values, device):
    import numpy as np
    a = np.ascontiguousarray(np.asarray(values, dtype=np.float32))
    key = (a.tobytes(), a.shape, str(device))
    t = _const_cache.get(key)
    if t is None:
        if len(_const_cache) > 4096:
            _const_cache.clear()
        t = _const_cache[key] = torch.tensor(a, device=device)
    return t


def size_query(fn, ints=(), outputs=1):
    out = [_sz(0) for _ in range(outputs)]
    check(fn(*ints, *[ctypes.byref(n) for n in out]))
    return out[0].value if outputs == 1 else tuple(n.value for n in out)


def c_ints(values):
    return (_ci * len(values))(*values)


def c_ptrs(tensors):
    return (_vp * len(tensors))(*[ptr(t) for t in tensors])


def c_floats(values):
    return (ctypes.c_float * len(values))(*values)


def raster_workspace(bs, nf, S, device):
    return torch.empty(size_query(lib().sdn_raster_workspace_bytes, (bs, nf, S)), dtype=torch.uint8, device=device)


def perspective_transform_scratch(n, V):
    return size_query(lib().sdn_perspective_transform_scratch, (n, V), 2)


def train_losses_scratch(B, R, nffd):
    return size_query(lib().sdn_train_losses_scratch, (B, R, nffd))


def raster_bwd_workspace(bs, nf, S, device):
    return torch.empty(size_query(lib().sdn_raster_bwd_workspace_bytes, (bs, nf, S)), dtype=torch.uint8, device=device)


def scene_id_workspace(device):
    return torch.empty(size_query(lib().sdn_scene_id_workspace_bytes), dtype=torch.uint8, device=device)


def train_id_workspace(B, device):
    return torch.empty(size_query(lib().sdn_train_id_stats_workspace_bytes, (int(B),)), dtype=torch.uint8, device=device)


def timing_enable(on=True):
    check(lib().sdn_timing_enable(int(bool(on))))


def timing_read():
    ms, n = _cd(0), _cl(0)
    check(lib().sdn_timing_read(ctypes.byref(ms), ctypes.byref(n)))
    return ms.value, n.value


SLOT_RASTER_TILES, SLOT_EDGE_SCAN, SLOT_CONV_GEMM, SLOT_CONV_WGRAD, SLOT_CONV_NARROW, SLOT_RASTER_TILES_K1 = 0, 1, 2, 3, 4, 5
SLOT_SCENE_MASKS = 6


def timing_read_slot(slot):
    ms, n, w = _cd(0), _cl(0), _cd(0)
    check(lib().sdn_timing_read_slot(slot, ctypes.byref(ms), ctypes.byref(n), ctypes.byref(w)))
    return ms.value, n.value, w.value
# ... 1 lines not shown
```

### include/sdn_hip.h

```cpp
#ifndef SDN_HIP_H
#define SDN_HIP_H

#include <stddef.h>
#include <stdint.h>

#ifdef __cplusplus
extern "C" {
#endif

typedef void* sdnStream;

#define SDN_OK 0
#define SDN_EINVAL (-1)
#define SDN_ELAUNCH (-2)
#define SDN_ENOMEM (-3)

#define SDN_RGB 1
#define SDN_ALPHA 2
#define SDN_DEPTH 4
#define SDN_AA 8
#define SDN_FACE_COLOR 16
#define SDN_SAVE_MAPS 32
#define SDN_ACCUMULATE 64
#define SDN_STREAM_FACES 256
#define SDN_COUNT_WORK 512
#define SDN_SPARSE_GRAD 1024
#define SDN_LAZY_MAPS 2048
#define SDN_K1_COVERAGE 4096
#define SDN_SERIAL_EDGES 128

const char* sdn_last_error(void);
#define SDN_ABI_VERSION 20
int sdn_version(void);

int sdn_project_vertices(const float* verts, int bs, int nv, int camera_mode, const float* eye,
                         const float* dir, const float* up, const float* width, int flip_x,
                         float* out, sdnStream stream);
int sdn_project_vertices_bwd(const float* verts, int bs, int nv, int camera_mode, const float* eye,
                             const float* dir, const float* up, const float* width, int flip_x,
                             const float* grad_out, float* grad_verts, sdnStream stream);

int sdn_gather_faces(const float* verts, const int32_t* faces_idx, int bs, int nv, int nf0,
                     long faces_batch_stride, int fill_back, float* faces_out, sdnStream stream);
int sdn_gather_faces_bwd(const float* grad_faces, const int32_t* faces_idx, int bs, int nv, int nf0,
                         long faces_batch_stride, int fill_back, float* grad_verts, sdnStream stream);

int sdn_face_normals(const float* faces, long n_faces_total, float* normals, sdnStream stream);
int sdn_face_normals_bwd(const float* faces, const float* grad_normals, long n_faces_total,
                         float* grad_faces, sdnStream stream);

int sdn_raster_workspace_bytes(int bs, int nf, int S, size_t* out);

int sdn_rasterize_fwd(const float* faces, const float* textures, int ts, int bs, int nf, int S,
                      double near, double far, double eps, const float* bg, int bg_per_batch, int flags,
                      float* face_inv, int32_t* face_index_map, float* weight_map, float* depth_map,
                      float* rgb_map, float* rgb_out, float* alpha_out, float* depth_out,
                      void* workspace, size_t workspace_bytes, sdnStream stream);

int sdn_raster_work_counters(const void* workspace, int bs, int nf, int S, unsigned long long* out3, sdnStream stream);

int sdn_raster_phase_clocks(const void* workspace, int bs, int nf, int S, unsigned long long* out8, sdnStream stream);

int sdn_raster_bwd_workspace_bytes(int bs, int nf, int S, size_t* out);
int sdn_rasterize_bwd(const float* faces, const float* textures, int ts, int bs, int nf, int S,
                      double eps, int flags, const float* face_inv, const int32_t* face_index_map,
                      const float* weight_map, const float* depth_map, const float* rgb_map,
                      const float* g_rgb_out, const float* g_alpha_out, const float* g_depth_out,
                      float* grad_faces, float* grad_textures, void* workspace, size_t workspace_bytes,
                      sdnStream stream);

int sdn_render_maps_bytes(int bs, int nv, int nf0, int fill_back, int image_size, int flags, size_t* state_bytes,
                          size_t* bwd_workspace_bytes, size_t* fwd_scratch_bytes);
int sdn_render_maps_fwd(const float* verts, int bs, int nv, const int32_t* faces_idx, int nf0, long faces_batch_stride,
                        int fill_back, int camera_mode, const float* eye, const float* dir, const float* up,
                        const float* width, int flip_x, int image_size, int flags, double near, double far, double eps,
                        const float* bg, float* alpha_out, float* normal_out, float* depth_out, void* state,
                        size_t state_bytes, void* scratch, size_t scratch_bytes, sdnStream stream);
int sdn_render_maps_bwd(const float* verts, int bs, int nv, const int32_t* faces_idx, int nf0, long faces_batch_stride,
                        int fill_back, int camera_mode, const float* eye, const float* dir, const float* up,
                        const float* width, int flip_x, int image_size, int flags, double eps, double eps_alpha,
                        const float* bg, const float* g_alpha, const float* g_normal, const float* g_depth, float* grad_verts,
                        const void* state, size_t state_bytes, void* workspace, size_t workspace_bytes, sdnStream stream);

int sdn_ffd_decode(const float* Bt, const float* P, const int32_t* cls, int n, int vmax, int ncoef,
                   float* out, sdnStream stream);
int sdn_ffd_decode_bwd(const float* Bt, const int32_t* cls, const float* grad_out, int n, int vmax,
                       int ncoef, float* grad_P, sdnStream stream);
int sdn_ffd_coefficients(const float* x, const float* M, const float* base, int n, int m, int transpose, float* out,
                         sdnStream stream);


#define SDN_STAT_SLOTS 8
int sdn_conv_gemm_workspace_bytes(int N, int OH, int OW, int Cop, size_t* out);
int sdn_conv_gemm(const float* in, int N, int IH, int IW, int Cip, float* out, int OH, int OW, int Cop, int QH, int QW,
                  int istride, int ostride, int py, int px, int ntaps, const int8_t* dy, const int8_t* dx, int pad_mode,
                  int in_relu, const void* w_packed, int Kp, int w_rows, const float* bias, int act,
                  double* stats, int accumulate, int precision, void* workspace, size_t workspace_bytes,
                  sdnStream stream);

int sdn_conv_gemm_phases(const float* in, int N, int IH, int IW, int Cip, float* out, int OH, int OW, int Cop, int istride,
                         int ostride, int nphase, const int32_t* QH, const int32_t* QW, const int32_t* py, const int32_t* px,
                         const int32_t* ntaps, const int8_t* taps, int pad_mode, int in_relu, const void* const* w_packed,
                         const int32_t* Kp, int w_rows, const float* bias, int act, double* stats, int accumulate,
                         int precision, sdnStream stream);

int sdn_conv_wgrad(const float* rows, const float* gath, float* dw, int N, int QH, int QW, int Cr, int GH, int GW, int Cc,
                   int istride, int ntaps, const int8_t* dy, const int8_t* dx, int pad_mode, int relu_rows,
                   int relu_gath, int splits, int precision, void* workspace, size_t workspace_bytes, sdnStream stream);
int sdn_conv_wgrad_narrow(const float* rows, const float* gath, float* dw, int N, int QH, int QW, int Cr, int rows_used,
                          int GH, int GW, int Cc, int ntaps, const int8_t* dy, const int8_t* dx, int pad_mode,
                          int relu_rows, int relu_gath, sdnStream stream);

int sdn_conv_wgrad_head_mfma(const float* rows, const float* gath, float* dw, int N, int QH, int QW, int Cr, int rows_used,
                             int GH, int GW, int Cc, int ntaps, const int8_t* dy, const int8_t* dx, int pad_mode,
                             int relu_rows, int relu_gath, sdnStream stream);

int sdn_conv_narrow_fwd(const float* in, int N, int IH, int IW, int Cip, float* out, int QH, int QW, int Cop,
                        int rows_used, const float* w_dense, int KH, int KW, int dy_min, int dx_min, int pad_mode,
                        int in_relu, const float* bias, int act, sdnStream stream);

int sdn_conv_head_steps(int Cip, int KH, int KW, int* steps);
int sdn_conv_head_mfma(const float* in, int N, int IH, int IW, int Cip, float* out, int QH, int QW, int Cop, int rows_used,
                       const void* w_frag, int KH, int KW, int dy_min, int dx_min, int pad_mode, int in_relu,
                       const float* bias, int act, double* stats, sdnStream stream);

int sdn_in_apply(float* z, const double* stats, float* mr, const float* res, float* out2, int N, int HW, int C, int Cp,
                 float eps, int act, int res_relu, float momentum, float* running_mean, float* running_var, void* planes,
                 long plane_stride, int planes_relu, sdnStream stream);
#define SDN_IN_BWD_SUMS_ZEROED 8
int sdn_in_bwd(float* g, const float* stored, const float* mr, double* sums, int N, int HW, int Cp, int mode, void* planes,
               long plane_stride, sdnStream stream);
int sdn_act_bwd(float* g, const float* y, float* bias_grad, long npos, int Cp, int act, void* planes, long plane_stride,
                sdnStream stream);
int sdn_reflect_fold(const float* gp, float* out, int N, int H, int W, int Cp, int pad, int accumulate, sdnStream stream);
int sdn_conv_pack_weights(const float* w, int R, int C, long sr, long sc, const int32_t* tapidx, int ntaps, int Ccp,
                          int Kp, int rows, void* packed, sdnStream stream);
int sdn_split_planes(const float* x, long n, int relu, void* planes, long plane_stride, sdnStream stream);
int sdn_assemble_nhwc(const float* const* parts, const int32_t* channels, int nparts, int N, int H, int W, int Cp, float* out,
                      sdnStream stream);
int sdn_conv_pack_weights_kmajor(const float* w, int R, int C, long sr, long sc, const int32_t* tapidx, int ntaps, int Ccp,
                                 int rows, void* packed, sdnStream stream);
int sdn_conv_tile(const void* in_planes, long plane_stride, int N, int IH, int IW, int Cip, float* out, void* out_planes,
                  long out_plane_stride, int planes_relu, int OH, int OW, int Cop, int QH, int QW, int istride, int ostride,
                  int py, int px, int ntaps, const int8_t* dy, const int8_t* dx, int pad_mode, const void* w_kmajor,
                  int w_rows, const float* bias, int act, double* stats, int accumulate, int ksplit, sdnStream stream);
int sdn_conv_halo_blocks(int N, int OH, int OW, int Cop, int kh, int kw, int* TH, int* TW, long* blocks);
int sdn_conv_halo(const void* in_planes, long plane_stride, int N, int IH, int IW, int Cip, float* out, int OH, int OW, int Cop,
                  int ntaps, const int8_t* dy, const int8_t* dx, int pad_mode, const void* w_kmajor, int w_rows,
                  const float* bias, int act, double* stats, int accumulate, sdnStream stream);
int sdn_conv_wgrad_tile(const void* rows_planes, long rows_stride, const void* gath_planes, long gath_stride, float* dw,
                        int N, int QH, int QW, int Cr, int GH, int GW, int Cc, int istride, int ntaps, const int8_t* dy,
                        const int8_t* dx, int pad_mode, sdnStream stream);
int sdn_conv_unpack_grad(const float* dw, int R, int C, long sr, long sc, const int32_t* tapidx, int ntaps, int Ccp,
                         float* grad_w, int accumulate, sdnStream stream);

int sdn_bn_forward(const float* x, long rows, int C, const float* gamma, const float* beta, float* running_mean,
                   float* running_var, float momentum, float eps, int training, const float* res, int relu, float* out,
                   float* mr, float* ss, double* sums, sdnStream stream);
int sdn_bn_backward(const float* g, const float* out, const float* x, const float* mr, const float* gamma, long rows, int C,
                    int training, int relu, float* gm, float* dx, double* sums, sdnStream stream);
int sdn_maxpool3x3s2_fwd(const float* x, int N, int H, int W, int C, float* out, int8_t* idx, sdnStream stream);
int sdn_maxpool3x3s2_bwd(const float* g, const int8_t* idx, int N, int H, int W, int C, float* gin, sdnStream stream);
int sdn_avgpool_global(const float* x, int N, int HW, int C, float* out, int backward, sdnStream stream);

int sdn_segment_mean(const float* x, const int32_t* seg, int N, int C, int HW, int K, float* sums, float* counts,
                     float* out, sdnStream stream);

int sdn_avgpool3x3s2_fwd(const float* in, int N, int C, int H, int W, const long* in_strides, float* out,
                         const long* out_strides, int inner_c, sdnStream stream);
int sdn_avgpool3x3s2_bwd(const float* g, int N, int C, int H, int W, const long* g_strides, float* gin,
                         const long* gin_strides, int inner_c, sdnStream stream);

int sdn_l1_loss_fwd(const float* a, const float* b, long n, double* sum, float* out, sdnStream stream);
int sdn_l1_loss_bwd(const float* a, const float* b, long n, const float* grad_out, float* grad_a, float* grad_b,
                    sdnStream stream);
#define SDN_SIL_LOSS_BLOCKS 512
#define SDN_SIL_LOSS_SUMS (3 + 3 * SDN_SIL_LOSS_BLOCKS)
int sdn_silhouette_loss_fwd(const float* masks, const float* target, const float* ignore, long n, const float* ffd, long nffd,
                            double* sums, float* out, sdnStream stream);
int sdn_silhouette_loss_bwd(const float* masks, const float* target, const float* ignore, long n, const float* ffd, long nffd,
                            const double* sums, const float* grad_out, float* grad_masks, float* grad_ffd, sdnStream stream);
int sdn_train_losses_scratch(int B, int R, long nffd, size_t* bytes);
int sdn_train_losses_fwd(const float* p_theta_deltas, const float* p_translation2ds, const float* p_log_scales,
                         const float* p_log_depths, const float* p_class_log_probs, const float* p_masks, const float* p_ffd,
                         long nffd, const float* thetas, const float* translation2ds, const float* log_scales,
                         const float* log_depths, const float* masks, const float* ignores, const int64_t* targets, int B, int R,
                         int S, int mode, double mask_weight, double ffd_coeff_reg, void* scratch, float* out, sdnStream stream);
int sdn_train_losses_bwd(const float* p_theta_deltas, const float* p_translation2ds, const float* p_log_scales,
                         const float* p_log_depths, const float* p_masks, const float* p_ffd, long nffd, const float* thetas,
                         const float* translation2ds, const float* log_scales, const float* log_depths, const float* masks,
                         const float* ignores, const int64_t* targets, int B, int R, int S, int mode, double mask_weight,
                         double ffd_coeff_reg, const void* scratch, const float* grad_out, float* grad_theta_deltas,
                         float* grad_translation2ds, float* grad_log_scales, float* grad_log_depths, float* grad_class_log_probs,
                         float* grad_masks, float* grad_ffd, sdnStream stream);
int sdn_pose_params(const float* theta, const float* log_scales, int n, float* quat, float* scales, sdnStream stream);
int sdn_pose_algebra(const float* centre, const float* extent, const float* focals, const float* theta_deltas,
                     const float* log_scales, const float* log_depths, const float* translation2ds, int n, int training,
                     float image_size, float render_size, float* thetas, float* alphas, float* rotations, float* scales,
                     float* depths, float* center2ds, float* translations, float* persp, float* zooms, sdnStream stream);
int sdn_pose_algebra_bwd(const float* centre, const float* extent, const float* theta_deltas, const float* thetas,
                         const float* scales, const float* depths, const float* center2ds, const float* translations, int n,
                         int training, const float* g_thetas, const float* g_alphas, const float* g_rotations,
                         const float* g_scales, const float* g_depths, const float* g_center2ds, const float* g_translations,
                         const float* g_persp, float* g_theta_deltas, float* g_log_scales, float* g_log_depths,
                         float* g_translation2ds, sdnStream stream);
int sdn_pose_params_bwd(const float* theta, const float* scales, const float* g_quat, const float* g_scales, int n,
                        float* g_theta, float* g_log_scales, sdnStream stream);

int sdn_composite_frame(const float* masks, const float* normals, const float* depth_maps, const float* zooms, int n,
                        int R, const int32_t* objs, int m, const int32_t* bounds, const int32_t* kk8, const double* kkf,
                        int H, int W, float* inst, float* nrm, float* dep, sdnStream stream);

int sdn_edit_assemble(const float* base_segm, long base_stride, const uint8_t* edit_inst, const int32_t* obj_label,
                      const int32_t* obj_pose, const int32_t* code_ids, const float* codes, int K, int C, int F, int HW,
                      int pose_channels, float* segm_out, float* inst_out, float* pose_out, float* feat_out,
                      int32_t* missing, sdnStream stream);

int sdn_scene_cover(const float* masks, int N, int H, int W, uint32_t* cover, sdnStream stream);
int sdn_scene_crops(const uint8_t* frame, const uint32_t* cover, const uint32_t* ignore_cover, const int64_t* nearer,
                    const int32_t* rois_host, const int32_t* objs, const int32_t* bounds, const int32_t* kk8, int N, int H, int W,
                    int image_size, int mask_size, int kinds, float mean0, float mean1, float mean2, float std0, float std1,
                    float std2, float* rgbs, float* masks, float* ignores, sdnStream stream);
int sdn_scene_edit(const float* theta_deltas, const float* translation2ds, const float* log_depths, const float* mroi_norms,
                   const float* droi_norms, const uint8_t* interests, const int32_t* records, int F, int N, int P,
                   float* theta_out, float* translation_out, float* log_depth_out, uint8_t* interests_out, sdnStream stream);

int sdn_unmold_masks(const float* mrcnn_mask, int D, int C, int Mh, int Mw, const int32_t* objs_host, const int32_t* objs, int n,
                     const int32_t* bounds, int n_bounds, const int32_t* kk8, int n_kk8, int H, int W, float* masks,
                     int32_t* areas, sdnStream stream);
int sdn_scene_gt_masks(const uint8_t* scene, const uint8_t* codes, int K, int H, int W, float* masks, int32_t* rois,
                       int32_t* areas, sdnStream stream);

int sdn_scene_id_workspace_bytes(size_t* out);
int sdn_scene_id_stats(const int32_t* scene, const int32_t* disparity, int category, int H, int W, int32_t* table,
                       void* workspace, sdnStream stream);
// ... 207 lines not shown
```

Before: 25170.

## Emit coverage bitmaps and visible flags in forward raster epilogue for backward reuse

The forward tile epilogue now writes the row and transposed coverage bitmasks and the per-face visibility flags into the saved render state. The backward pass then reads them instead of rebuilding them with k_cover_bits or k_mark_visible, and a smaller k_transpose_grad transposes the alpha gradient and zeroes the counters, which replaces most of a memset. This trades backward work for extra ballots, shared-memory exchange and global writes in the forward epilogue, plus extra state memory.

New measurement: 25680, median of 6. 2.0% higher.

```diff
diff --git a/3d-sdn_amd/csrc/raster_bwd.hip b/3d-sdn_amd/csrc/raster_bwd.hip
--- a/3d-sdn_amd/csrc/raster_bwd.hip
+++ b/3d-sdn_amd/csrc/raster_bwd.hip
@@ -278,6 +278,35 @@
         if (lx == 0 && xt < S) covT[((size_t)b * S + xt) * W + blockIdx.y] = (uint32_t)(m >> half);
         const int xo = blockIdx.x * n + lc, yo = blockIdx.y * n + lx;
         if (lx < n && lc < n && xo < R && yo < R) gT[((size_t)b * R + xo) * R + yo] = gt[lx][lc];
+    }
+}
+
+__global__ __launch_bounds__(256) void k_transpose_grad(const float* __restrict__ g, int R, float* __restrict__ gT,
+                                                        uint32_t* __restrict__ counter, uint32_t* __restrict__ row_cnt, long n_row_cnt)
+{
+    __shared__ float gt[32][33];
+    const int b = blockIdx.z;
+    const int lx = threadIdx.x & 31, l8 = threadIdx.x >> 5;
+    const long wg = ((long)blockIdx.z * gridDim.y + blockIdx.y) * gridDim.x + blockIdx.x;
+    const long nthreads = (long)gridDim.x * gridDim.y * gridDim.z * 256;
+    for (long i = wg * 256 + threadIdx.x; i < 64 + n_row_cnt; i += nthreads) {
+        if (i < 64)
+            counter[i] = 0u;
+        else
+            row_cnt[i - 64] = 0u;
+    }
+#pragma unroll
+    for (int r = 0; r < 4; r++) {
+        const int ly = l8 + 8 * r;
+        const int xo = blockIdx.x * 32 + lx, yo = blockIdx.y * 32 + ly;
+        gt[ly][lx] = (xo < R && yo < R) ? g[((size_t)b * R + yo) * R + xo] : 0.0f;
+    }
+    __syncthreads();
+#pragma unroll
+    for (int r = 0; r < 4; r++) {
+        const int lc = l8 + 8 * r;
+        const int xo = blockIdx.x * 32 + lc, yo = blockIdx.y * 32 + lx;
+        if (xo < R && yo < R) gT[((size_t)b * R + xo) * R + yo] = gt[lx][lc];
     }
 }
 
@@ -1079,10 +1108,6 @@
     total = off[13] + align256((size_t)cap);
 }
 
-namespace sdn {
-const uint32_t* raster_bwd_visible_flags(const void* workspace) { return (const uint32_t*)((const char*)workspace + 256); }
-}
-
 SDN_API int sdn_raster_bwd_workspace_bytes(int bs, int nf, int S, size_t* out)
 {
     if (bs <= 0 || nf <= 0 || S <= 0 || !out) return fail(SDN_EINVAL, "sdn_raster_bwd_workspace_bytes: bad sizes");
@@ -1109,8 +1134,9 @@
                             double eps, int flags, const float* face_inv, const int32_t* face_index_map, const float* weight_map,
                             const float* depth_map, const float* rgb_map, const float* g_rgb_out, const float* g_alpha_out,
                             const float* g_depth_out, float* grad_faces, float* grad_textures, void* workspace,
-                            size_t workspace_bytes, sdnStream stream)
-{
+                            size_t workspace_bytes, sdnStream stream, const CoverMaps* given)
+{
+    if (given && (!given->cov || !given->covT || !given->visible)) given = nullptr;
     if (!faces || !face_inv || !face_index_map || !weight_map || !depth_map || (!grad_faces && !sink) || bs <= 0 || nf <= 0 ||
         S <= 0)
         return fail(SDN_EINVAL, "sdn_rasterize_bwd: missing state (was the forward run with SDN_SAVE_MAPS?)");
@@ -1141,7 +1167,7 @@
     P.grad_textures = grad_textures;
     char* ws = (char*)workspace;
     P.counter = (uint32_t*)(ws + off[0]);
-    P.visible = (uint32_t*)(ws + off[1]);
+    P.visible = given ? given->visible : (uint32_t*)(ws + off[1]);
     P.chunk_base = (int32_t*)(ws + off[2]);
     P.chunk_desc = (uint4*)(ws + off[3]);
     P.chunk_out = (float2*)(ws + off[4]);
@@ -1168,13 +1194,17 @@
     if (!edges) P.flags &= ~SDN_SPARSE_GRAD;
     int rc;
     if (edges) {
-        hipError_t e = hipMemsetAsync(ws, 0, off[2], st);
-        if (e != hipSuccess) return fail(SDN_ELAUNCH, "hipMemsetAsync(plan): %s", hipGetErrorString(e));
         const size_t cov_words = (size_t)(S + 31) / 32;
         const bool setup_fits = 2 * (size_t)bs * S * cov_words * sizeof(uint32_t) <= off[7] - off[6] &&
                                 (size_t)bs * S * S * sizeof(float) <= off[12] - off[11];
         const bool sil_path = (P.flags & SDN_ALPHA) && !(P.flags & SDN_RGB) && !(flags & SDN_SERIAL_EDGES) && setup_fits;
-        if (!sil_path) {
+        hipError_t e = hipSuccess;
+        if (!given)
+            e = hipMemsetAsync(ws, 0, off[2], st);
+        else if (!sil_path)
+            e = hipMemsetAsync(ws, 0, 256, st);
+        if (e != hipSuccess) return fail(SDN_ELAUNCH, "hipMemsetAsync(plan): %s", hipGetErrorString(e));
+        if (!sil_path && !given) {
             hipLaunchKernelGGL(k_mark_visible, dim3(cdiv(npx, 256)), dim3(256), 0, st, face_index_map, npx, S, nf,
                                P.visible);
             if ((rc = check_launch("k_mark_visible"))) return rc;
@@ -1183,14 +1213,22 @@
             if (S > 65535) return fail(SDN_EINVAL, "sdn_rasterize_bwd: internal size %d exceeds the 16-bit row index", S);
             const bool aa = (P.flags & SDN_AA) != 0;
             const size_t rows = (size_t)bs * S;
-            uint32_t* cov = (uint32_t*)(ws + off[6]);
-            uint32_t* covT = cov + rows * cov_words;
+            const uint32_t* cov = given ? given->cov : (uint32_t*)(ws + off[6]);
+            const uint32_t* covT = given ? given->covT : cov + rows * cov_words;
             float* gT = (float*)(ws + off[11]);
             uint16_t* cnt = (uint16_t*)(ws + off[7]);
             uint16_t* pos = (uint16_t*)(ws + off[8]);
             float* val = (float*)(ws + off[9]);
-            hipLaunchKernelGGL(k_cover_bits, dim3(cdiv(S, 32), cdiv(S, 32), bs), dim3(256), 0, st, P, cov, covT, gT);
-            if ((rc = check_launch("k_cover_bits"))) return rc;
+            if (given) {
+                const int R = aa ? S / 2 : S;
+                hipLaunchKernelGGL(k_transpose_grad, dim3(cdiv(R, 32), cdiv(R, 32), bs), dim3(256), 0, st, P.g_alpha_out, R, gT,
+                                   P.counter, (uint32_t*)(ws + off[10]), (long)4 * bs * S);
+                if ((rc = check_launch("k_transpose_grad"))) return rc;
+            } else {
+                hipLaunchKernelGGL(k_cover_bits, dim3(cdiv(S, 32), cdiv(S, 32), bs), dim3(256), 0, st, P, (uint32_t*)(ws + off[6]),
+                                   (uint32_t*)(ws + off[6]) + rows * cov_words, gT);
+                if ((rc = check_launch("k_cover_bits"))) return rc;
+            }
             const dim3 grid((unsigned)cdiv((long)(2 * rows), 4));
             if (aa)
                 hipLaunchKernelGGL(k_compact_rows<true>, grid, dim3(256), 0, st, P, cov, covT, gT, rows, S, cnt, pos, val);
diff --git a/3d-sdn_amd/csrc/raster_fwd.hip b/3d-sdn_amd/csrc/raster_fwd.hip
--- a/3d-sdn_amd/csrc/raster_fwd.hip
+++ b/3d-sdn_amd/csrc/raster_fwd.hip
@@ -49,6 +49,9 @@
     const uint32_t* thin_count;
     const float4* thin_list;
     unsigned long long* counters;
+    uint32_t* cov;
+    uint32_t* covT;
+    uint32_t* visible;
     uint32_t list_cap;
     double eps;
     int ts, bs, nf, S, ntx, flags, bg_per_batch;
@@ -86,7 +89,7 @@
                                                      float* __restrict__ face_inv, uint32_t* __restrict__ tilebox,
                                                      uint4* __restrict__ pixbox, uint32_t* __restrict__ tile_count,
                                                      uint32_t* __restrict__ thin_count, float4* __restrict__ thin_list,
-                                                     const FaceSource G)
+                                                     uint32_t* __restrict__ visible, const FaceSource G)
 {
     __shared__ uint32_t hist[HIST_MAX];
     const int ntiles = ntx * ntx;
@@ -277,6 +280,7 @@
         }
     }
     tilebox[i] = tb;
+    if (visible) visible[i] = 0u;
     if (!GATHER || tb != TB_CULLED || thin) {
 #pragma unroll
         for (int k = 0; k < 9; k++) face_inv[i * 9 + k] = inv[k];
@@ -517,7 +521,7 @@
 }
 
 __device__ __forceinline__ void tile_epilogue(const FwdParams& P, const int b, const int X0, const int Y0,
-                                              const unsigned long long* zbuf, const int tid)
+                                              const unsigned long long* zbuf, const int tid, uint32_t* xch)
 {
     const int S = P.S;
     const bool aa = (P.flags & SDN_AA) != 0;
@@ -528,8 +532,33 @@
     const bool want_depth = (P.flags & SDN_DEPTH) != 0;
     const int qx = tid % (TS / 2), qy = tid / (TS / 2);
     const int R = aa ? S / 2 : S;
+    if (P.cov) {
+        const int lane = tid & 63, wave = tid >> 6;
+        const int W = (S + 31) >> 5;
+        const int lx = lane & 31;
+        const unsigned half = lane & 32;
+#pragma unroll
+        for (int r = 0; r < 4; r++) {
+            const int ly = 8 * wave + 2 * r + (lane >> 5);
+            const bool covered = zbuf[ly * TS + lx] != ~0ull && X0 + lx < S && Y0 + ly < S;
+            const uint32_t word = (uint32_t)(__ballot(covered) >> half);
+            if (lx == 0) {
+                xch[ly] = word;
+                if (Y0 + ly < S) P.cov[((size_t)b * S + Y0 + ly) * W + (X0 >> 5)] = word;
+            }
+        }
+        __syncthreads();
+        const uint32_t row_word = xch[lx];
+#pragma unroll
+        for (int c = 0; c < 4; c++) {
+            const int col = 8 * wave + c + (lane >> 5) * 4;
+            const uint32_t word = (uint32_t)(__ballot(((row_word >> col) & 1u) != 0u) >> half);
+            if (lx == 0 && X0 + col < S) P.covT[((size_t)b * S + X0 + col) * W + (Y0 >> 5)] = word;
+        }
+    }
     float s_alpha = 0.f, s_depth = 0.f, s_rgb[3] = {0.f, 0.f, 0.f};
     bool any_valid = false;
+    int qf[2][2] = {{-1, -1}, {-1, -1}};
 #pragma unroll
     for (int dyi = 0; dyi < 2; dyi++) {
 #pragma unroll
@@ -541,6 +570,7 @@
             any_valid = true;
             const PixelResult r = shade_pixel(P, b, zbuf[py * TS + px], gx, gy);
             const size_t q = ((size_t)b * S + gy) * S + gx;
+            qf[dy][dx] = r.fn;
             if (save) {
                 P.face_index_map[q] = r.fn;
                 P.depth_map[q] = r.zp;
@@ -582,6 +612,14 @@
 #pragma unroll
             for (int k = 0; k < 3; k++) P.rgb_out[(((size_t)b * 3 + k) * R + orow) * R + oc] = s_rgb[k] * 0.25f;
         }
+    }
+    if (P.cov) {
+        uint32_t* vis = P.visible + (size_t)b * P.nf;
+        const int left = __shfl_up(qf[0][1], 1);
+        if (qf[0][0] >= 0 && (qx == 0 || left != qf[0][0])) vis[qf[0][0]] = 1u;
+        if (qf[0][1] >= 0 && qf[0][1] != qf[0][0]) vis[qf[0][1]] = 1u;
+        if (qf[1][0] >= 0 && qf[1][0] != qf[0][0] && qf[1][0] != qf[0][1]) vis[qf[1][0]] = 1u;
+        if (qf[1][1] >= 0 && qf[1][1] != qf[1][0] && qf[1][1] != qf[0][1] && qf[1][1] != qf[0][0]) vis[qf[1][1]] = 1u;
     }
 }
 
@@ -1007,7 +1045,7 @@
     tick(c_fetch);
 
 
-    tile_epilogue(P, b, X0, Y0, zbuf, tid);
+    tile_epilogue(P, b, X0, Y0, zbuf, tid, q_fn);
     if constexpr (COUNT) {
         tick(c_epi);
         __shared__ unsigned long long cnt[3];
@@ -1229,13 +1267,14 @@
         }
     }
     __syncthreads();
-    tile_epilogue(P, b, X0, Y0, zbuf, tid);
+    tile_epilogue(P, b, X0, Y0, zbuf, tid, hit_queue[0]);
 }
 
 __global__ __launch_bounds__(NTHR) void k_raster_tiles_k1_plain(const FwdParams P)
 {
     __shared__ unsigned long long zbuf[TS * TS];
     __shared__ uint32_t next_batch;
+    __shared__ uint32_t row_words[TS];
     const int tid = threadIdx.x;
     const int lane = tid & 63;
     const int ntiles = P.ntx * P.ntx;
@@ -1351,7 +1390,7 @@
         }
     }
     __syncthreads();
-    tile_epilogue(P, b, X0, Y0, zbuf, tid);
+    tile_epilogue(P, b, X0, Y0, zbuf, tid, row_words);
 }
 
 }
@@ -1417,7 +1456,7 @@
                        double far, double eps, const float* bg, int bg_per_batch, int flags, float* face_inv,
                        int32_t* face_index_map, float* weight_map, float* depth_map, float* rgb_map,
                        float* rgb_out, float* alpha_out, float* depth_out, void* workspace,
-                       size_t workspace_bytes, sdnStream stream)
+                       size_t workspace_bytes, sdnStream stream, const CoverMaps* emit)
 {
     if (!(flags & (SDN_RGB | SDN_ALPHA | SDN_DEPTH)))
         return fail(SDN_EINVAL, "sdn_rasterize_fwd: nothing to draw (rasterize.py:25-27)");
@@ -1450,6 +1489,8 @@
     uint32_t* thin_count = (uint32_t*)(ws + W.thin_count);
     float4* thin_list = (float4*)(ws + W.thin_list);
     const int ntx = W.ntx;
+    if (emit && (!(flags & SDN_SAVE_MAPS) || !emit->cov || !emit->covT || !emit->visible)) emit = nullptr;
+    uint32_t* visible = emit ? emit->visible : nullptr;
     hipError_t me = hipMemsetAsync(ws + W.zeroed, 0, W.zeroed_bytes, st);
     if (me != hipSuccess) return fail(SDN_ELAUNCH, "hipMemsetAsync(tile counters): %s", hipGetErrorString(me));
     const dim3 face_grid(cdiv(nf, 256), bs);
@@ -1460,7 +1501,7 @@
     if (src) G = *src;
 #define SDN_FACE_SETUP(K1_, GATHER_)                                                                                          \
     hipLaunchKernelGGL((k_face_setup<K1_, GATHER_>), setup_grid, dim3(256), 0, st, faces, nf, S, ntx, face_inv, tilebox, pixbox, \
-                       tile_count, thin_count, thin_list, G)
+                       tile_count, thin_count, thin_list, visible, G)
     if (k1 && src) SDN_FACE_SETUP(true, true);
     else if (k1) SDN_FACE_SETUP(true, false);
     else if (src) SDN_FACE_SETUP(false, true);
@@ -1502,6 +1543,9 @@
     P.thin_count = thin_count;
     P.thin_list = thin_list;
     P.counters = (unsigned long long*)(ws + W.counters);
+    P.cov = emit ? emit->cov : nullptr;
+    P.covT = emit ? emit->covT : nullptr;
+    P.visible = visible;
     P.list_cap = W.list_cap;
     P.eps = eps;
     P.ts = ts;
diff --git a/3d-sdn_amd/csrc/raster_maps.hip b/3d-sdn_amd/csrc/raster_maps.hip
--- a/3d-sdn_amd/csrc/raster_maps.hip
+++ b/3d-sdn_amd/csrc/raster_maps.hip
@@ -11,6 +11,7 @@
 
 struct MapsLayout {
     size_t pv, faces9, face_inv, faces_n, colors, fim, wmap, dmap, rgbmap, bgcopy, raster_ws, raster_ws_bytes, total;
+    size_t cov, covT, visible;
     size_t b_raster, b_raster_bytes, g_faces9, g_colors, g_pv, g_faces_n, g_v2, b_total;
     int nf, S;
 };
@@ -36,6 +37,10 @@
     L.wmap = take(px * 12);
     L.dmap = take(px * 4);
     L.rgbmap = take(normal ? px * 12 : 0);
+    const size_t bits = (size_t)bs * L.S * ((L.S + 31) / 32) * sizeof(uint32_t);
+    L.cov = take(bits);
+    L.covT = take(bits);
+    L.visible = take(n * sizeof(uint32_t));
     L.bgcopy = take(0);
     int rc = sdn_raster_workspace_bytes(bs, L.nf, L.S, &L.raster_ws_bytes);
     if (rc) return rc;
@@ -78,6 +83,19 @@
     if (state_bytes) *state_bytes = L.total;
     if (bwd_bytes) *bwd_bytes = L.b_total;
     if (fwd_scratch_bytes) *fwd_scratch_bytes = L.raster_ws_bytes;
+    return SDN_OK;
+}
+
+SDN_API int sdn_render_maps_state_layout(int bs, int nv, int nf0, int fill_back, int image_size, int flags, size_t out[4])
+{
+    MapsLayout L;
+    int rc = maps_layout(bs, nv, nf0, fill_back, image_size, flags, L);
+    if (rc) return rc;
+    if (!out) return fail(SDN_EINVAL, "sdn_render_maps_state_layout: out is NULL");
+    out[0] = L.fim;
+    out[1] = L.cov;
+    out[2] = L.covT;
+    out[3] = L.visible;
     return SDN_OK;
 }
 
@@ -123,10 +141,11 @@
     }
     const int rflags = (flags & (SDN_RGB | SDN_DEPTH | SDN_AA | SDN_SAVE_MAPS | SDN_STREAM_FACES | SDN_COUNT_WORK | SDN_K1_COVERAGE)) | SDN_ALPHA |
                        (normal ? SDN_FACE_COLOR : 0) | SDN_LAZY_MAPS;
+    const CoverMaps emit = {(uint32_t*)(s + L.cov), (uint32_t*)(s + L.covT), (uint32_t*)(s + L.visible)};
     return rasterize_fwd_core(fused_setup ? &G : nullptr, (const float*)(s + L.faces9), colors, normal ? 2 : 0, bs, L.nf, L.S, near,
                               far, eps, bg, 0, rflags, (float*)(s + L.face_inv), (int32_t*)(s + L.fim), (float*)(s + L.wmap),
                               (float*)(s + L.dmap), normal ? (float*)(s + L.rgbmap) : nullptr, normal_out, alpha_out, depth_out,
-                              scratch, L.raster_ws_bytes, stream);
+                              scratch, L.raster_ws_bytes, stream, &emit);
 }
 
 SDN_API int sdn_render_maps_bwd(const float* verts, int bs, int nv, const int32_t* faces_idx, int nf0,
@@ -157,15 +176,16 @@
     float* g_faces9 = (float*)(w + L.g_faces9);
     float* g_colors = g_normal ? (float*)(w + L.g_colors) : nullptr;
     const int base = (flags & (SDN_AA | SDN_SERIAL_EDGES)) | (normal ? SDN_FACE_COLOR : 0) | SDN_SPARSE_GRAD;
-    const uint32_t* visible = (g_alpha || g_normal) ? raster_bwd_visible_flags(w + L.b_raster) : nullptr;
+    char* sw = const_cast<char*>(s);
+    const CoverMaps given = {(uint32_t*)(sw + L.cov), (uint32_t*)(sw + L.covT), (uint32_t*)(sw + L.visible)};
+    const uint32_t* visible = (g_alpha || g_normal) ? given.visible : nullptr;
     auto raster_bwd = [&](int fl, double e, const float* gr, const float* ga, const float* gd, float* gt) {
-        return sdn_rasterize_bwd(faces9, colors, normal ? 2 : 0, bs, L.nf, L.S, e, fl, (const float*)(s + L.face_inv),
-                                 (const int32_t*)(s + L.fim), (const float*)(s + L.wmap), (const float*)(s + L.dmap),
-                                 normal ? (const float*)(s + L.rgbmap) : nullptr, gr, ga, gd, g_faces9, gt, w + L.b_raster,
-                                 L.b_raster_bytes, stream);
+        return rasterize_bwd_core(nullptr, faces9, colors, normal ? 2 : 0, bs, L.nf, L.S, e, fl, (const float*)(s + L.face_inv),
+                                  (const int32_t*)(s + L.fim), (const float*)(s + L.wmap), (const float*)(s + L.dmap),
+                                  normal ? (const float*)(s + L.rgbmap) : nullptr, gr, ga, gd, g_faces9, gt, w + L.b_raster,
+                                  L.b_raster_bytes, stream, &given);
     };
     if ((normal && (g_normal || g_depth)) || (!normal && g_depth)) {
-        char* sw = const_cast<char*>(s);
         if ((rc = launch_reshade_maps(faces9, colors, normal ? 2 : 0, bs, L.nf, L.S, 0.0, eps,
                                       normal ? bg : nullptr, 0,
                                       (flags & (SDN_AA | SDN_K1_COVERAGE)) | (normal ? (SDN_RGB | SDN_FACE_COLOR) : 0), (const float*)(s + L.face_inv),
@@ -179,7 +199,7 @@
         if ((rc = rasterize_bwd_core(&sink, faces9, colors, normal ? 2 : 0, bs, L.nf, L.S, eps_alpha, base | SDN_ALPHA,
                                      (const float*)(s + L.face_inv), (const int32_t*)(s + L.fim), (const float*)(s + L.wmap),
                                      (const float*)(s + L.dmap), nullptr, nullptr, g_alpha, nullptr, nullptr, nullptr,
-                                     w + L.b_raster, L.b_raster_bytes, stream)))
+                                     w + L.b_raster, L.b_raster_bytes, stream, &given)))
             return rc;
         return sdn_project_vertices_bwd(verts, bs, nv, camera_mode, eye, dir, up, width, flip_x, g_pv, grad_verts, stream);
     }
diff --git a/3d-sdn_amd/csrc/sdn_common.h b/3d-sdn_amd/csrc/sdn_common.h
--- a/3d-sdn_amd/csrc/sdn_common.h
+++ b/3d-sdn_amd/csrc/sdn_common.h
@@ -69,7 +69,6 @@
 int launch_gather_faces_bwd(const float* grad_faces, const int32_t* faces_idx, int bs, int nv, int nf0, long fstride,
                             int fill_back, int flip_x, int zero_first, float* grad_verts, hipStream_t st,
                             const uint32_t* visible = nullptr);
-const uint32_t* raster_bwd_visible_flags(const void* raster_bwd_workspace);
 int launch_face_normals_gather(const float* verts, const int32_t* faces_idx, int bs, int nv, int nf0, long fstride,
                                int fill_back, int flip_x, float sx, float* normals, hipStream_t st);
 int launch_face_normals(const float* faces, long total, float sx, float* normals, hipStream_t st);
@@ -78,11 +77,17 @@
                         const float* depth_map, float* weight_map, float* rgb_map, hipStream_t st);
 int launch_face_normals_bwd(const float* faces, const float* grad_normals, long total, float sx, float* grad_faces,
                             hipStream_t st);
+struct CoverMaps {
+    uint32_t* cov;
+    uint32_t* covT;
+    uint32_t* visible;
+};
 struct FaceSource;
 int rasterize_fwd_core(const FaceSource* src, const float* faces, const float* textures, int ts, int bs, int nf, int S, double near,
                        double far, double eps, const float* bg, int bg_per_batch, int flags, float* face_inv,
                        int32_t* face_index_map, float* weight_map, float* depth_map, float* rgb_map, float* rgb_out,
-                       float* alpha_out, float* depth_out, void* workspace, size_t workspace_bytes, sdnStream stream);
+                       float* alpha_out, float* depth_out, void* workspace, size_t workspace_bytes, sdnStream stream,
+                       const CoverMaps* emit = nullptr);
 
 struct VertexSink {
     const int32_t* faces_idx;
@@ -94,6 +99,6 @@
                        int flags, const float* face_inv, const int32_t* face_index_map, const float* weight_map,
                        const float* depth_map, const float* rgb_map, const float* g_rgb_out, const float* g_alpha_out,
                        const float* g_depth_out, float* grad_faces, float* grad_textures, void* workspace, size_t workspace_bytes,
-                       sdnStream stream);
+                       sdnStream stream, const CoverMaps* given = nullptr);
 
 }
diff --git a/3d-sdn_amd/sdn_hip/__init__.py b/3d-sdn_amd/sdn_hip/__init__.py
--- a/3d-sdn_amd/sdn_hip/__init__.py
+++ b/3d-sdn_amd/sdn_hip/__init__.py
@@ -171,6 +171,7 @@
                                   _vp, _vp, _vp, _vp, _sz, _vp, _sz, _vp]
     sig['sdn_render_maps_bwd'] = [_vp, _ci, _ci, _vp, _ci, _cl, _ci, _ci, _vp, _vp, _vp, _vp, _ci, _ci, _ci, _cd, _cd, _vp, _vp, _vp,
                                   _vp, _vp, _vp, _sz, _vp, _sz, _vp]
+    sig['sdn_render_maps_state_layout'] = [_ci, _ci, _ci, _ci, _ci, _ci, ctypes.POINTER(_sz)]
     _lp = ctypes.POINTER(_cl)
     sig['sdn_avgpool3x3s2_fwd'] = [_vp, _ci, _ci, _ci, _ci, _lp, _vp, _lp, _ci, _vp]
     sig['sdn_avgpool3x3s2_bwd'] = [_vp, _ci, _ci, _ci, _ci, _lp, _vp, _lp, _ci, _vp]
diff --git a/include/sdn_hip.h b/include/sdn_hip.h
--- a/include/sdn_hip.h
+++ b/include/sdn_hip.h
@@ -81,6 +81,7 @@
                         const float* width, int flip_x, int image_size, int flags, double eps, double eps_alpha,
                         const float* bg, const float* g_alpha, const float* g_normal, const float* g_depth, float* grad_verts,
                         const void* state, size_t state_bytes, void* workspace, size_t workspace_bytes, sdnStream stream);
+int sdn_render_maps_state_layout(int bs, int nv, int nf0, int fill_back, int image_size, int flags, size_t out[4]);
 
 int sdn_ffd_decode(const float* Bt, const float* P, const int32_t* cls, int n, int vmax, int ncoef,
                    float* out, sdnStream stream);
```
